# lixiny/ArtiBoost

Measured on AMD Instinct MI355X. Metric: synth samples/sec (render+fwd+bwd) 256x256 bs=64, higher is better.
Workload: dtype bf16x3; 1 GPU; train_artiboost HO3Dv2-clasbased (HybridBaseline/ResNet-34, 22x28x32x32 heat-map) + online CCV render 512->256, per-GPU batch 64, HO3D-like objects; global_batch=64, image=256, parallelism=dp1, graph=True, render_overlap=False

## Files before the change

artiboost_amd/csrc/optim.hip:

```cpp
#include "common.h"

#define OPT_THREADS 256
#define OPT_MAX_PARTS 1024

__global__ __launch_bounds__(OPT_THREADS) void sqnorm_kernel(const float* __restrict__ g, long n, float* __restrict__ part) {
    double s = 0.0;
    long nvec = n / 4;
    for (long i = (long)blockIdx.x * OPT_THREADS + threadIdx.x; i < nvec; i += (long)gridDim.x * OPT_THREADS) {
        float4 v = ((const float4*)g)[i];
        s += (double)v.x * v.x + (double)v.y * v.y + (double)v.z * v.z + (double)v.w * v.w;
    }
    __shared__ double sm[OPT_THREADS];
    sm[threadIdx.x] = s;
    __syncthreads();
    for (int o = OPT_THREADS / 2; o > 0; o >>= 1) {
        if (threadIdx.x < o) sm[threadIdx.x] += sm[threadIdx.x + o];
        __syncthreads();
    }
    if (threadIdx.x == 0) part[blockIdx.x] = (float)sm[0];
}

__global__ void norm_finalize_kernel(const float* __restrict__ part, int nparts, float* __restrict__ out) {
    double s = 0.0;
    for (int i = threadIdx.x; i < nparts; i += 64) s += part[i];
#pragma unroll
    for (int o = 32; o > 0; o >>= 1) s += __shfl_xor(s, o, 64);
    if (threadIdx.x == 0) out[0] = (float)sqrt(s);
}

__global__ __launch_bounds__(OPT_THREADS) void clip_adam_kernel(float* __restrict__ p, const float* __restrict__ g,
                                                                float* __restrict__ m, float* __restrict__ v, long n,
                                                                const float* __restrict__ total_norm, float max_norm,
                                                                float lr, float b1, float b2, float eps, float bc1,
                                                                float bc2_sqrt, const float* __restrict__ hyper,
                                                                bf16_t* __restrict__ lp, bf16_t* __restrict__ lp_lo = nullptr) {
    if (hyper) { lr = hyper[0]; bc1 = hyper[1]; bc2_sqrt = hyper[2]; }
    float coef = 1.f;
    if (max_norm > 0.f) { coef = max_norm / (total_norm[0] + 1e-6f); coef = coef > 1.f ? 1.f : coef; }
    const float step = lr / bc1;
    long nvec = n / 4;
    for (long i = (long)blockIdx.x * OPT_THREADS + threadIdx.x; i < nvec; i += (long)gridDim.x * OPT_THREADS) {
        float4 pv = ((float4*)p)[i], gv = ((const float4*)g)[i], mv = ((float4*)m)[i], vv = ((float4*)v)[i];
        float pp[4] = {pv.x, pv.y, pv.z, pv.w}, gg[4] = {gv.x, gv.y, gv.z, gv.w};
        float mm[4] = {mv.x, mv.y, mv.z, mv.w}, vvv[4] = {vv.x, vv.y, vv.z, vv.w};
#pragma unroll
        for (int k = 0; k < 4; ++k) {
            float gk = gg[k] * coef;
            mm[k] = mm[k] * b1 + (1.f - b1) * gk;
            vvv[k] = vvv[k] * b2 + (1.f - b2) * gk * gk;
            float denom = sqrtf(vvv[k]) / bc2_sqrt + eps;
            pp[k] = pp[k] - step * (mm[k] / denom);
        }
        ((float4*)p)[i] = make_float4(pp[0], pp[1], pp[2], pp[3]);
        ((float4*)m)[i] = make_float4(mm[0], mm[1], mm[2], mm[3]);
        ((float4*)v)[i] = make_float4(vvv[0], vvv[1], vvv[2], vvv[3]);
        if (lp) {
            uint2 o;
            o.x = pack_bf16x2(pp[0], pp[1]);
            o.y = pack_bf16x2(pp[2], pp[3]);
            ((uint2*)lp)[i] = o;
            if (lp_lo) {
                uint2 l;
                l.x = pack_bf16x2(pp[0] - __uint_as_float(o.x << 16), pp[1] - __uint_as_float(o.x & 0xffff0000u));
                l.y = pack_bf16x2(pp[2] - __uint_as_float(o.y << 16), pp[3] - __uint_as_float(o.y & 0xffff0000u));
                ((uint2*)lp_lo)[i] = l;
            }
        }
    }
}

extern "C" int ab_grad_norm(const float* grad, long n, float* part, float* total_norm, void* stream) {
    if (!grad || !part || !total_norm) return AB_EINVAL;
    if (n % 4) return AB_ESHAPE;
    long b = (n / 4 + OPT_THREADS - 1) / OPT_THREADS;
    int nb = (int)(b > OPT_MAX_PARTS ? OPT_MAX_PARTS : (b < 1 ? 1 : b));
    sqnorm_kernel<<<nb, OPT_THREADS, 0, as_stream(stream)>>>(grad, n, part);
    AB_LAUNCH_CHECK();
    norm_finalize_kernel<<<1, 64, 0, as_stream(stream)>>>(part, nb, total_norm);
    AB_LAUNCH_CHECK();
    return 0;
}

__global__ __launch_bounds__(OPT_THREADS) void scale_kernel(float* __restrict__ x, long n, float s, int head) {
    long nvec = (n - head) / 4;
    float4* xv = (float4*)(x + head);
    for (long i = (long)blockIdx.x * OPT_THREADS + threadIdx.x; i < nvec; i += (long)gridDim.x * OPT_THREADS) {
        float4 v = xv[i];
        v.x *= s; v.y *= s; v.z *= s; v.w *= s;
        xv[i] = v;
    }
    if (blockIdx.x == 0) {
        if ((int)threadIdx.x < head) x[threadIdx.x] *= s;
        long t = head + nvec * 4 + threadIdx.x;
        if (threadIdx.x < 4 && t < n) x[t] *= s;
    }
}

extern "C" int ab_scale_f32(float* x, long n, float s, void* stream) {
    if (!x || n < 0 || (uintptr_t)x % 4) return AB_EINVAL;
    if (n == 0) return 0;
    int head = (int)(((16 - (uintptr_t)x % 16) % 16) / 4);
    if (head > n) head = (int)n;
    long b = ((n - head) / 4 + OPT_THREADS - 1) / OPT_THREADS;
    int nb = (int)(b > 2048 ? 2048 : (b < 1 ? 1 : b));
    scale_kernel<<<nb, OPT_THREADS, 0, as_stream(stream)>>>(x, n, s, head);
    AB_LAUNCH_CHECK();
    return 0;
}

static int clip_adam_impl(float* param, const float* grad, float* m, float* v, long n, const float* total_norm, float max_norm, float lr,
                          float beta1, float beta2, float eps, int step, const float* hyper, void* lp, void* lp_lo, void* stream);

extern "C" int ab_clip_adam(float* param, const float* grad, float* m, float* v, long n, const float* total_norm,
                            float max_norm, float lr, float beta1, float beta2, float eps, int step,
                            const float* hyper, void* lp, void* stream) {
    return clip_adam_impl(param, grad, m, v, n, total_norm, max_norm, lr, beta1, beta2, eps, step, hyper, lp, nullptr, stream);
}

extern "C" int ab_clip_adam_x3(float* param, const float* grad, float* m, float* v, long n, const float* total_norm,
                               float max_norm, float lr, float beta1, float beta2, float eps, int step,
                               const float* hyper, void* lp_hi, void* lp_lo, void* stream) {
    if (!lp_hi || !lp_lo) return AB_EINVAL;
    return clip_adam_impl(param, grad, m, v, n, total_norm, max_norm, lr, beta1, beta2, eps, step, hyper, lp_hi, lp_lo, stream);
}

static int clip_adam_impl(float* param, const float* grad, float* m, float* v, long n, const float* total_norm, float max_norm, float lr,
                          float beta1, float beta2, float eps, int step, const float* hyper, void* lp, void* lp_lo, void* stream) {
    if (!param || !grad || !m || !v || (max_norm > 0.f && !total_norm)) return AB_EINVAL;
    if (n % 4 || step < 1) return AB_ESHAPE;
    double bc1 = 1.0 - pow((double)beta1, (double)step), bc2 = 1.0 - pow((double)beta2, (double)step);
    long b = (n / 4 + OPT_THREADS - 1) / OPT_THREADS;
    int nb = (int)(b > 4096 ? 4096 : (b < 1 ? 1 : b));
    clip_adam_kernel<<<nb, OPT_THREADS, 0, as_stream(stream)>>>(param, grad, m, v, n, total_norm, max_norm, lr, beta1,
                                                                beta2, eps, (float)bc1, (float)sqrt(bc2), hyper, (bf16_t*)lp, (bf16_t*)lp_lo);
    AB_LAUNCH_CHECK();
    return 0;
}


__global__ void wall_stamp_kernel(int64_t* slot) { *slot = (int64_t)wall_clock64(); }
extern "C" int ab_wall_stamp(int64_t* slot, void* stream) {
    if (!slot) return AB_EINVAL;
    wall_stamp_kernel<<<1, 1, 0, as_stream(stream)>>>(slot);
    AB_LAUNCH_CHECK();
    return 0;
}
extern "C" int ab_wall_clock_khz(void) {
    int dev = 0, khz = 0;
    if (hipGetDevice(&dev) != hipSuccess || hipDeviceGetAttribute(&khz, hipDeviceAttributeWallClockRate, dev) != hipSuccess) return 0;
    return khz;
}
```

artiboost_amd/csrc/torch_ops_gen.cpp:

```cpp
#include <ATen/ATen.h>
#include <c10/hip/HIPStream.h>
#include <torch/library.h>
#include "../../include/artiboost_hip.h"

static inline void* p(const c10::optional<at::Tensor>& t) { return (t.has_value() && t->defined()) ? t->data_ptr() : nullptr; }
static inline void* cur_stream() { return (void*)c10::hip::getCurrentHIPStream().stream(); }

#include <c10/hip/HIPFunctions.h>
typedef c10::optional<at::Tensor> OptT;
static inline bool has(const OptT& t) { return t.has_value() && t->defined(); }
static inline void ck_contig(const char* op, const char* a, const OptT& t) {
    if (has(t)) TORCH_CHECK(t->is_contiguous(), op, ": argument '", a, "' must be contiguous (the kernels take raw buffers)");
}
static inline void ck_dev(const char* op, const char* a, const OptT& t, int dt, bool contiguous) {
    if (!has(t)) return;
    TORCH_CHECK(t->is_cuda(), op, ": argument '", a, "' must be a HIP tensor, got a ", t->device().str(), " tensor");
    TORCH_CHECK(t->get_device() == c10::hip::current_device(), op, ": argument '", a, "' lives on device ", t->get_device(), ", the current device is ", (int)c10::hip::current_device());
    if (contiguous) TORCH_CHECK(t->is_contiguous(), op, ": argument '", a, "' must be contiguous (the kernel takes it as a raw buffer without a pitch)");
    if (dt >= 0) TORCH_CHECK((int)t->scalar_type() == dt, op, ": argument '", a, "' must be ", c10::toString((at::ScalarType)dt), ", got ", c10::toString(t->scalar_type()));
}
static inline void ck_host(const char* op, const char* a, const OptT& t) {
    if (!has(t)) return;
    TORCH_CHECK(t->is_cpu(), op, ": argument '", a, "' is a HOST structure / array of the C ABI and must be a CPU tensor, got a ", t->device().str(), " tensor");
    TORCH_CHECK(t->is_contiguous(), op, ": argument '", a, "' must be contiguous");
// ... 74 lines not shown
static void w_col_stats(const c10::optional<at::Tensor>& x, int64_t dtype, int64_t M, int64_t C, const c10::optional<at::Tensor>& part) { static const char* const OP = "artiboost_hip::col_stats"; ck_dev(OP, "x", x, (int)-1, true); ck_dev(OP, "part", part, (int)at::kFloat, true); ck_dtcode(OP, "x", x, dtype); ck_numel(OP, "x", x, (int64_t)(M*C)); ck_numel(OP, "part", part, (int64_t)(ab_col_stats_nparts(M)*C*2)); const long rc = (long)ab_col_stats((const void*)p(x), (int)dtype, (long)M, (int)C, (float*)p(part), cur_stream()); TORCH_CHECK(rc == 0, "ab_col_stats failed with code ", rc, rc > 0 ? " (hipError)" : " (argument error)"); }
static void w_bn_finalize(const c10::optional<at::Tensor>& part, int64_t nparts, int64_t C, int64_t count, const c10::optional<at::Tensor>& gamma, const c10::optional<at::Tensor>& beta, double eps, double momentum, const c10::optional<at::Tensor>& running_mean, const c10::optional<at::Tensor>& running_var, const c10::optional<at::Tensor>& bnp) { static const char* const OP = "artiboost_hip::bn_finalize"; ck_dev(OP, "part", part, (int)at::kFloat, true); ck_dev(OP, "gamma", gamma, (int)at::kFloat, true); ck_dev(OP, "beta", beta, (int)at::kFloat, true); ck_dev(OP, "running_mean", running_mean, (int)at::kFloat, true); ck_dev(OP, "running_var", running_var, (int)at::kFloat, true); ck_dev(OP, "bnp", bnp, (int)at::kFloat, true); ck_numel(OP, "part", part, (int64_t)(nparts*C*2)); ck_numel(OP, "gamma", gamma, (int64_t)(C)); ck_numel(OP, "beta", beta, (int64_t)(C)); ck_numel(OP, "running_mean", running_mean, (int64_t)(C)); ck_numel(OP, "running_var", running_var, (int64_t)(C)); ck_numel(OP, "bnp", bnp, (int64_t)(4*C)); const long rc = (long)ab_bn_finalize((const float*)p(part), (int)nparts, (int)C, (long)count, (const float*)p(gamma), (const float*)p(beta), (float)eps, (float)momentum, (float*)p(running_mean), (float*)p(running_var), (float*)p(bnp), cur_stream()); TORCH_CHECK(rc == 0, "ab_bn_finalize failed with code ", rc, rc > 0 ? " (hipError)" : " (argument error)"); }
static void w_bn_eval_params(int64_t C, const c10::optional<at::Tensor>& gamma, const c10::optional<at::Tensor>& beta, const c10::optional<at::Tensor>& rm, const c10::optional<at::Tensor>& rv, double eps, const c10::optional<at::Tensor>& bnp) { static const char* const OP = "artiboost_hip::bn_eval_params"; ck_dev(OP, "gamma", gamma, (int)at::kFloat, true); ck_dev(OP, "beta", beta, (int)at::kFloat, true); ck_dev(OP, "rm", rm, (int)at::kFloat, true); ck_dev(OP, "rv", rv, (int)at::kFloat, true); ck_dev(OP, "bnp", bnp, (int)at::kFloat, true); ck_numel(OP, "gamma", gamma, (int64_t)(C)); ck_numel(OP, "beta", beta, (int64_t)(C)); ck_numel(OP, "rm", rm, (int64_t)(C)); ck_numel(OP, "rv", rv, (int64_t)(C)); ck_numel(OP, "bnp", bnp, (int64_t)(4*C)); const long rc = (long)ab_bn_eval_params((int)C, (const float*)p(gamma), (const float*)p(beta), (const float*)p(rm), (const float*)p(rv), (float)eps, (float*)p(bnp), cur_stream()); TORCH_CHECK(rc == 0, "ab_bn_eval_params failed with code ", rc, rc > 0 ? " (hipError)" : " (argument error)"); }
static void w_bn_eval_params_batch(const c10::optional<at::Tensor>& flat, const c10::optional<at::Tensor>& stats, const c10::optional<at::Tensor>& desc_dev, int64_t n, int64_t max_c, double eps, const c10::optional<at::Tensor>& out) { static const char* const OP = "artiboost_hip::bn_eval_params_batch"; ck_dev(OP, "flat", flat, (int)at::kFloat, true); ck_dev(OP, "stats", stats, (int)at::kFloat, true); ck_dev(OP, "desc_dev", desc_dev, (int)at::kInt, true); ck_dev(OP, "out", out, (int)at::kFloat, true); const long rc = (long)ab_bn_eval_params_batch((const float*)p(flat), (const float*)p(stats), (const int32_t*)p(desc_dev), (int)n, (int)max_c, (float)eps, (float*)p(out), cur_stream()); TORCH_CHECK(rc == 0, "ab_bn_eval_params_batch failed with code ", rc, rc > 0 ? " (hipError)" : " (argument error)"); }
static void w_bn_apply(const c10::optional<at::Tensor>& y, const c10::optional<at::Tensor>& res, const c10::optional<at::Tensor>& bnp, int64_t dtype, int64_t M, int64_t C, int64_t relu, const c10::optional<at::Tensor>& out) { static const char* const OP = "artiboost_hip::bn_apply"; ck_dev(OP, "y", y, (int)-1, true); ck_dev(OP, "res", res, (int)-1, true); ck_dev(OP, "bnp", bnp, (int)at::kFloat, true); ck_dev(OP, "out", out, (int)-1, true); const long rc = (long)ab_bn_apply((const void*)p(y), (const void*)p(res), (const float*)p(bnp), (int)dtype, (long)M, (int)C, (int)relu, (void*)p(out), cur_stream()); TORCH_CHECK(rc == 0, "ab_bn_apply failed with code ", rc, rc > 0 ? " (hipError)" : " (argument error)"); }
static void w_bn_bwd(const c10::optional<at::Tensor>& dout, const c10::optional<at::Tensor>& out, const c10::optional<at::Tensor>& y, const c10::optional<at::Tensor>& bnp, int64_t dtype, int64_t M, int64_t C, int64_t relu, const c10::optional<at::Tensor>& part, const c10::optional<at::Tensor>& bwdp, const c10::optional<at::Tensor>& dgamma, const c10::optional<at::Tensor>& dbeta, const c10::optional<at::Tensor>& dy, const c10::optional<at::Tensor>& dz_out) { static const char* const OP = "artiboost_hip::bn_bwd"; ck_dev(OP, "dout", dout, (int)-1, true); ck_dev(OP, "out", out, (int)-1, true); ck_dev(OP, "y", y, (int)-1, true); ck_dev(OP, "bnp", bnp, (int)at::kFloat, true); ck_dev(OP, "part", part, (int)at::kFloat, true); ck_dev(OP, "bwdp", bwdp, (int)at::kFloat, true); ck_dev(OP, "dgamma", dgamma, (int)at::kFloat, true); ck_dev(OP, "dbeta", dbeta, (int)at::kFloat, true); ck_dev(OP, "dy", dy, (int)-1, true); ck_dev(OP, "dz_out", dz_out, (int)-1, true); const long rc = (long)ab_bn_bwd((const void*)p(dout), (const void*)p(out), (const void*)p(y), (const float*)p(bnp), (int)dtype, (long)M, (int)C, (int)relu, (float*)p(part), (float*)p(bwdp), (float*)p(dgamma), (float*)p(dbeta), (void*)p(dy), (void*)p(dz_out), cur_stream()); TORCH_CHECK(rc == 0, "ab_bn_bwd failed with code ", rc, rc > 0 ? " (hipError)" : " (argument error)"); }
static void w_relu_bwd(const c10::optional<at::Tensor>& dout, const c10::optional<at::Tensor>& out, int64_t dtype, int64_t n, const c10::optional<at::Tensor>& dz) { static const char* const OP = "artiboost_hip::relu_bwd"; ck_dev(OP, "dout", dout, (int)-1, true); ck_dev(OP, "out", out, (int)-1, true); ck_dev(OP, "dz", dz, (int)-1, true); const long rc = (long)ab_relu_bwd((const void*)p(dout), (const void*)p(out), (int)dtype, (long)n, (void*)p(dz), cur_stream()); TORCH_CHECK(rc == 0, "ab_relu_bwd failed with code ", rc, rc > 0 ? " (hipError)" : " (argument error)"); }
static void w_col_sum(const c10::optional<at::Tensor>& x, int64_t dtype, int64_t M, int64_t C, const c10::optional<at::Tensor>& part, const c10::optional<at::Tensor>& out) { static const char* const OP = "artiboost_hip::col_sum"; ck_dev(OP, "x", x, (int)-1, true); ck_dev(OP, "part", part, (int)at::kFloat, true); ck_dev(OP, "out", out, (int)at::kFloat, true); const long rc = (long)ab_col_sum((const void*)p(x), (int)dtype, (long)M, (int)C, (float*)p(part), (float*)p(out), cur_stream()); TORCH_CHECK(rc == 0, "ab_col_sum failed with code ", rc, rc > 0 ? " (hipError)" : " (argument error)"); }
static void w_col_sum_x3(const c10::optional<at::Tensor>& hi, const c10::optional<at::Tensor>& lo, int64_t M, int64_t C, const c10::optional<at::Tensor>& part, const c10::optional<at::Tensor>& out) { static const char* const OP = "artiboost_hip::col_sum_x3"; ck_dev(OP, "hi", hi, (int)-1, true); ck_dev(OP, "lo", lo, (int)-1, true); ck_dev(OP, "part", part, (int)at::kFloat, true); ck_dev(OP, "out", out, (int)at::kFloat, true); const long rc = (long)ab_col_sum_x3((const void*)p(hi), (const void*)p(lo), (long)M, (int)C, (float*)p(part), (float*)p(out), cur_stream()); TORCH_CHECK(rc == 0, "ab_col_sum_x3 failed with code ", rc, rc > 0 ? " (hipError)" : " (argument error)"); }
static void w_add(const c10::optional<at::Tensor>& a, const c10::optional<at::Tensor>& b, int64_t dtype, int64_t n, const c10::optional<at::Tensor>& out) { static const char* const OP = "artiboost_hip::add"; ck_dev(OP, "a", a, (int)-1, true); ck_dev(OP, "b", b, (int)-1, true); ck_dev(OP, "out", out, (int)-1, true); const long rc = (long)ab_add((const void*)p(a), (const void*)p(b), (int)dtype, (long)n, (void*)p(out), cur_stream()); TORCH_CHECK(rc == 0, "ab_add failed with code ", rc, rc > 0 ? " (hipError)" : " (argument error)"); }
static void w_maxpool3x3s2_fwd(const c10::optional<at::Tensor>& x, int64_t dtype, int64_t N, int64_t H, int64_t W, int64_t C, const c10::optional<at::Tensor>& out, const c10::optional<at::Tensor>& idx) { static const char* const OP = "artiboost_hip::maxpool3x3s2_fwd"; ck_dev(OP, "x", x, (int)-1, true); ck_dev(OP, "out", out, (int)-1, true); ck_dev(OP, "idx", idx, (int)-1, true); const long rc = (long)ab_maxpool3x3s2_fwd((const void*)p(x), (int)dtype, (int)N, (int)H, (int)W, (int)C, (void*)p(out), (void*)p(idx), cur_stream()); TORCH_CHECK(rc == 0, "ab_maxpool3x3s2_fwd failed with code ", rc, rc > 0 ? " (hipError)" : " (argument error)"); }
static int64_t w_conv2d_dgrad_bnstats_rows(int64_t dtype, int64_t N, int64_t H, int64_t W, int64_t Cin, int64_t Cout, int64_t kh, int64_t kw, int64_t stride, int64_t pad) { return (int64_t)ab_conv2d_dgrad_bnstats_rows((int)dtype, (int)N, (int)H, (int)W, (int)Cin, (int)Cout, (int)kh, (int)kw, (int)stride, (int)pad); }
static void w_conv2d_dgrad_bnstats(const c10::optional<at::Tensor>& dy, const c10::optional<at::Tensor>& wt, const c10::optional<at::Tensor>& dx, int64_t dtype, int64_t N, int64_t H, int64_t W, int64_t Cin, int64_t Cout, int64_t kh, int64_t kw, int64_t stride, int64_t pad, const c10::optional<at::Tensor>& addend, const c10::optional<at::Tensor>& bn_y, const c10::optional<at::Tensor>& bn_out, const c10::optional<at::Tensor>& bnp, const c10::optional<at::Tensor>& bn_part) { static const char* const OP = "artiboost_hip::conv2d_dgrad_bnstats"; ck_dev(OP, "dy", dy, (int)-1, true); ck_dev(OP, "wt", wt, (int)-1, true); ck_dev(OP, "dx", dx, (int)-1, true); ck_dev(OP, "addend", addend, (int)-1, true); ck_dev(OP, "bn_y", bn_y, (int)-1, true); ck_dev(OP, "bn_out", bn_out, (int)-1, true); ck_dev(OP, "bnp", bnp, (int)at::kFloat, true); ck_dev(OP, "bn_part", bn_part, (int)at::kFloat, true); const long rc = (long)ab_conv2d_dgrad_bnstats((const void*)p(dy), (const void*)p(wt), (void*)p(dx), (int)dtype, (int)N, (int)H, (int)W, (int)Cin, (int)Cout, (int)kh, (int)kw, (int)stride, (int)pad, (const void*)p(addend), (const void*)p(bn_y), (const void*)p(bn_out), (const float*)p(bnp), (float*)p(bn_part), cur_stream()); TORCH_CHECK(rc == 0, "ab_conv2d_dgrad_bnstats failed with code ", rc, rc > 0 ? " (hipError)" : " (argument error)"); }
static void w_bn_bwd_apply(const c10::optional<at::Tensor>& dout, const c10::optional<at::Tensor>& out, const c10::optional<at::Tensor>& y, const c10::optional<at::Tensor>& bnp, int64_t dtype, int64_t M, int64_t C, int64_t relu, const c10::optional<at::Tensor>& part, int64_t nparts, const c10::optional<at::Tensor>& bwdp, const c10::optional<at::Tensor>& dgamma, const c10::optional<at::Tensor>& dbeta, const c10::optional<at::Tensor>& dy, const c10::optional<at::Tensor>& dz_out) { static const char* const OP = "artiboost_hip::bn_bwd_apply"; ck_dev(OP, "dout", dout, (int)-1, true); ck_dev(OP, "out", out, (int)-1, true); ck_dev(OP, "y", y, (int)-1, true); ck_dev(OP, "bnp", bnp, (int)at::kFloat, true); ck_dev(OP, "part", part, (int)at::kFloat, true); ck_dev(OP, "bwdp", bwdp, (int)at::kFloat, true); ck_dev(OP, "dgamma", dgamma, (int)at::kFloat, true); ck_dev(OP, "dbeta", dbeta, (int)at::kFloat, true); ck_dev(OP, "dy", dy, (int)-1, true); ck_dev(OP, "dz_out", dz_out, (int)-1, true); const long rc = (long)ab_bn_bwd_apply((const void*)p(dout), (const void*)p(out), (const void*)p(y), (const float*)p(bnp), (int)dtype, (long)M, (int)C, (int)relu, (const float*)p(part), (int)nparts, (float*)p(bwdp), (float*)p(dgamma), (float*)p(dbeta), (void*)p(dy), (void*)p(dz_out), cur_stream()); TORCH_CHECK(rc == 0, "ab_bn_bwd_apply failed with code ", rc, rc > 0 ? " (hipError)" : " (argument error)"); }
static void w_bn_relu_maxpool3x3s2_fwd(const c10::optional<at::Tensor>& y, const c10::optional<at::Tensor>& bnp, int64_t dtype, int64_t N, int64_t H, int64_t W, int64_t C, const c10::optional<at::Tensor>& out, const c10::optional<at::Tensor>& idx) { static const char* const OP = "artiboost_hip::bn_relu_maxpool3x3s2_fwd"; ck_dev(OP, "y", y, (int)-1, true); ck_dev(OP, "bnp", bnp, (int)at::kFloat, true); ck_dev(OP, "out", out, (int)-1, true); ck_dev(OP, "idx", idx, (int)-1, true); const long rc = (long)ab_bn_relu_maxpool3x3s2_fwd((const void*)p(y), (const float*)p(bnp), (int)dtype, (int)N, (int)H, (int)W, (int)C, (void*)p(out), (void*)p(idx), cur_stream()); TORCH_CHECK(rc == 0, "ab_bn_relu_maxpool3x3s2_fwd failed with code ", rc, rc > 0 ? " (hipError)" : " (argument error)"); }
static void w_bn_relu_maxpool3x3s2_fwd_x3(const c10::optional<at::Tensor>& y, const c10::optional<at::Tensor>& bnp, int64_t N, int64_t H, int64_t W, int64_t C, const c10::optional<at::Tensor>& out, const c10::optional<at::Tensor>& out_hi, const c10::optional<at::Tensor>& out_lo, const c10::optional<at::Tensor>& idx) { static const char* const OP = "artiboost_hip::bn_relu_maxpool3x3s2_fwd_x3"; ck_dev(OP, "y", y, (int)at::kFloat, true); ck_dev(OP, "bnp", bnp, (int)at::kFloat, true); ck_dev(OP, "out", out, (int)at::kFloat, true); ck_dev(OP, "out_hi", out_hi, (int)-1, true); ck_dev(OP, "out_lo", out_lo, (int)-1, true); ck_dev(OP, "idx", idx, (int)-1, true); const long rc = (long)ab_bn_relu_maxpool3x3s2_fwd_x3((const float*)p(y), (const float*)p(bnp), (int)N, (int)H, (int)W, (int)C, (float*)p(out), (void*)p(out_hi), (void*)p(out_lo), (void*)p(idx), cur_stream()); TORCH_CHECK(rc == 0, "ab_bn_relu_maxpool3x3s2_fwd_x3 failed with code ", rc, rc > 0 ? " (hipError)" : " (argument error)"); }
static void w_bn_relu_maxpool_bwd(const c10::optional<at::Tensor>& dpool, const c10::optional<at::Tensor>& idx, const c10::optional<at::Tensor>& y, const c10::optional<at::Tensor>& bnp, int64_t dtype, int64_t N, int64_t H, int64_t W, int64_t C, const c10::optional<at::Tensor>& part, const c10::optional<at::Tensor>& bwdp, const c10::optional<at::Tensor>& dgamma, const c10::optional<at::Tensor>& dbeta, const c10::optional<at::Tensor>& dy) { static const char* const OP = "artiboost_hip::bn_relu_maxpool_bwd"; ck_dev(OP, "dpool", dpool, (int)-1, true); ck_dev(OP, "idx", idx, (int)-1, true); ck_dev(OP, "y", y, (int)-1, true); ck_dev(OP, "bnp", bnp, (int)at::kFloat, true); ck_dev(OP, "part", part, (int)at::kFloat, true); ck_dev(OP, "bwdp", bwdp, (int)at::kFloat, true); ck_dev(OP, "dgamma", dgamma, (int)at::kFloat, true); ck_dev(OP, "dbeta", dbeta, (int)at::kFloat, true); ck_dev(OP, "dy", dy, (int)-1, true); const long rc = (long)ab_bn_relu_maxpool_bwd((const void*)p(dpool), (const void*)p(idx), (const void*)p(y), (const float*)p(bnp), (int)dtype, (int)N, (int)H, (int)W, (int)C, (float*)p(part), (float*)p(bwdp), (float*)p(dgamma), (float*)p(dbeta), (void*)p(dy), cur_stream()); TORCH_CHECK(rc == 0, "ab_bn_relu_maxpool_bwd failed with code ", rc, rc > 0 ? " (hipError)" : " (argument error)"); }
static int64_t w_bn_relu_maxpool_bwd_x3_nparts(int64_t N, int64_t H, int64_t W, int64_t C) { return (int64_t)ab_bn_relu_maxpool_bwd_x3_nparts((int)N, (int)H, (int)W, (int)C); }
static void w_bn_relu_maxpool_bwd_x3(const c10::optional<at::Tensor>& dpool, const c10::optional<at::Tensor>& idx, const c10::optional<at::Tensor>& y, const c10::optional<at::Tensor>& bnp, int64_t N, int64_t H, int64_t W, int64_t C, const c10::optional<at::Tensor>& part, const c10::optional<at::Tensor>& bwdp, const c10::optional<at::Tensor>& dgamma, const c10::optional<at::Tensor>& dbeta, const c10::optional<at::Tensor>& dz, const c10::optional<at::Tensor>& dy_hi, const c10::optional<at::Tensor>& dy_lo) { static const char* const OP = "artiboost_hip::bn_relu_maxpool_bwd_x3"; ck_dev(OP, "dpool", dpool, (int)at::kFloat, true); ck_dev(OP, "idx", idx, (int)-1, true); ck_dev(OP, "y", y, (int)at::kFloat, true); ck_dev(OP, "bnp", bnp, (int)at::kFloat, true); ck_dev(OP, "part", part, (int)at::kFloat, true); ck_dev(OP, "bwdp", bwdp, (int)at::kFloat, true); ck_dev(OP, "dgamma", dgamma, (int)at::kFloat, true); ck_dev(OP, "dbeta", dbeta, (int)at::kFloat, true); ck_dev(OP, "dz", dz, (int)at::kFloat, true); ck_dev(OP, "dy_hi", dy_hi, (int)-1, true); ck_dev(OP, "dy_lo", dy_lo, (int)-1, true); const long rc = (long)ab_bn_relu_maxpool_bwd_x3((const float*)p(dpool), (const void*)p(idx), (const float*)p(y), (const float*)p(bnp), (int)N, (int)H, (int)W, (int)C, (float*)p(part), (float*)p(bwdp), (float*)p(dgamma), (float*)p(dbeta), (float*)p(dz), (void*)p(dy_hi), (void*)p(dy_lo), cur_stream()); TORCH_CHECK(rc == 0, "ab_bn_relu_maxpool_bwd_x3 failed with code ", rc, rc > 0 ? " (hipError)" : " (argument error)"); }
static void w_bn_relu_maxpool3x3s2_fwd_x3w(const c10::optional<at::Tensor>& y, const c10::optional<at::Tensor>& bnp, int64_t N, int64_t H, int64_t W, int64_t C, const c10::optional<at::Tensor>& out, const c10::optional<at::Tensor>& out_hi, const c10::optional<at::Tensor>& out_lo, const c10::optional<at::Tensor>& idx, const c10::optional<at::Tensor>& ywin) { static const char* const OP = "artiboost_hip::bn_relu_maxpool3x3s2_fwd_x3w"; ck_dev(OP, "y", y, (int)at::kFloat, true); ck_dev(OP, "bnp", bnp, (int)at::kFloat, true); ck_dev(OP, "out", out, (int)at::kFloat, true); ck_dev(OP, "out_hi", out_hi, (int)-1, true); ck_dev(OP, "out_lo", out_lo, (int)-1, true); ck_dev(OP, "idx", idx, (int)-1, true); ck_dev(OP, "ywin", ywin, (int)at::kFloat, true); ck_dtype(OP, "out_hi", out_hi, at::kBFloat16); ck_dtype(OP, "out_lo", out_lo, at::kBFloat16); ck_numel(OP, "y", y, (int64_t)(N*H*W*C)); ck_numel(OP, "bnp", bnp, (int64_t)(2*C)); ck_numel(OP, "out", out, (int64_t)(N*(H/2)*(W/2)*C)); ck_numel(OP, "out_hi", out_hi, (int64_t)(N*(H/2)*(W/2)*C)); ck_numel(OP, "out_lo", out_lo, (int64_t)(N*(H/2)*(W/2)*C)); ck_numel(OP, "ywin", ywin, (int64_t)(N*(H/2)*(W/2)*C)); ck_bytes(OP, "idx", idx, (int64_t)(N*(H/2)*(W/2)*C)); const long rc = (long)ab_bn_relu_maxpool3x3s2_fwd_x3w((const float*)p(y), (const float*)p(bnp), (int)N, (int)H, (int)W, (int)C, (float*)p(out), (void*)p(out_hi), (void*)p(out_lo), (void*)p(idx), (float*)p(ywin), cur_stream()); TORCH_CHECK(rc == 0, "ab_bn_relu_maxpool3x3s2_fwd_x3w failed with code ", rc, rc > 0 ? " (hipError)" : " (argument error)"); }
static void w_bn_relu_maxpool_bwd_x3w(const c10::optional<at::Tensor>& dpool, const c10::optional<at::Tensor>& idx, const c10::optional<at::Tensor>& ywin, const c10::optional<at::Tensor>& y, const c10::optional<at::Tensor>& bnp, int64_t N, int64_t H, int64_t W, int64_t C, const c10::optional<at::Tensor>& part, const c10::optional<at::Tensor>& bwdp, const c10::optional<at::Tensor>& dgamma, const c10::optional<at::Tensor>& dbeta, const c10::optional<at::Tensor>& dy_hi, const c10::optional<at::Tensor>& dy_lo) { static const char* const OP = "artiboost_hip::bn_relu_maxpool_bwd_x3w"; ck_dev(OP, "dpool", dpool, (int)at::kFloat, true); ck_dev(OP, "idx", idx, (int)-1, true); ck_dev(OP, "ywin", ywin, (int)at::kFloat, true); ck_dev(OP, "y", y, (int)at::kFloat, true); ck_dev(OP, "bnp", bnp, (int)at::kFloat, true); ck_dev(OP, "part", part, (int)at::kFloat, true); ck_dev(OP, "bwdp", bwdp, (int)at::kFloat, true); ck_dev(OP, "dgamma", dgamma, (int)at::kFloat, true); ck_dev(OP, "dbeta", dbeta, (int)at::kFloat, true); ck_dev(OP, "dy_hi", dy_hi, (int)-1, true); ck_dev(OP, "dy_lo", dy_lo, (int)-1, true); const long rc = (long)ab_bn_relu_maxpool_bwd_x3w((const float*)p(dpool), (const void*)p(idx), (const float*)p(ywin), (const float*)p(y), (const float*)p(bnp), (int)N, (int)H, (int)W, (int)C, (float*)p(part), (float*)p(bwdp), (float*)p(dgamma), (float*)p(dbeta), (void*)p(dy_hi), (void*)p(dy_lo), cur_stream()); TORCH_CHECK(rc == 0, "ab_bn_relu_maxpool_bwd_x3w failed with code ", rc, rc > 0 ? " (hipError)" : " (argument error)"); }
static void w_maxpool3x3s2_bwd(const c10::optional<at::Tensor>& idx, const c10::optional<at::Tensor>& dout, int64_t dtype, int64_t N, int64_t H, int64_t W, int64_t C, const c10::optional<at::Tensor>& dx) { static const char* const OP = "artiboost_hip::maxpool3x3s2_bwd"; ck_dev(OP, "idx", idx, (int)-1, true); ck_dev(OP, "dout", dout, (int)-1, true); ck_dev(OP, "dx", dx, (int)-1, true); const long rc = (long)ab_maxpool3x3s2_bwd((const void*)p(idx), (const void*)p(dout), (int)dtype, (int)N, (int)H, (int)W, (int)C, (void*)p(dx), cur_stream()); TORCH_CHECK(rc == 0, "ab_maxpool3x3s2_bwd failed with code ", rc, rc > 0 ? " (hipError)" : " (argument error)"); }
static void w_avgpool_fwd(const c10::optional<at::Tensor>& x, int64_t dtype, int64_t N, int64_t HW, int64_t C, const c10::optional<at::Tensor>& out) { static const char* const OP = "artiboost_hip::avgpool_fwd"; ck_dev(OP, "x", x, (int)-1, true); ck_dev(OP, "out", out, (int)at::kFloat, true); ck_dtcode(OP, "x", x, dtype); ck_numel(OP, "x", x, (int64_t)(N*HW*C)); ck_numel(OP, "out", out, (int64_t)(N*C)); const long rc = (long)ab_avgpool_fwd((const void*)p(x), (int)dtype, (int)N, (int)HW, (int)C, (float*)p(out), cur_stream()); TORCH_CHECK(rc == 0, "ab_avgpool_fwd failed with code ", rc, rc > 0 ? " (hipError)" : " (argument error)"); }
static void w_avgpool_bwd(const c10::optional<at::Tensor>& g, int64_t dtype, int64_t N, int64_t HW, int64_t C, const c10::optional<at::Tensor>& dx, int64_t accumulate) { static const char* const OP = "artiboost_hip::avgpool_bwd"; ck_dev(OP, "g", g, (int)at::kFloat, true); ck_dev(OP, "dx", dx, (int)-1, true); const long rc = (long)ab_avgpool_bwd((const float*)p(g), (int)dtype, (int)N, (int)HW, (int)C, (void*)p(dx), (int)accumulate, cur_stream()); TORCH_CHECK(rc == 0, "ab_avgpool_bwd failed with code ", rc, rc > 0 ? " (hipError)" : " (argument error)"); }
static void w_cast_f32_bf16(const c10::optional<at::Tensor>& src, int64_t n, const c10::optional<at::Tensor>& dst) { static const char* const OP = "artiboost_hip::cast_f32_bf16"; ck_dev(OP, "src", src, (int)at::kFloat, true); ck_dev(OP, "dst", dst, (int)-1, true); ck_dtype(OP, "dst", dst, at::kBFloat16); ck_numel(OP, "src", src, (int64_t)(n)); ck_numel(OP, "dst", dst, (int64_t)(n)); const long rc = (long)ab_cast_f32_bf16((const float*)p(src), (long)n, (void*)p(dst), cur_stream()); TORCH_CHECK(rc == 0, "ab_cast_f32_bf16 failed with code ", rc, rc > 0 ? " (hipError)" : " (argument error)"); }
static void w_transpose_oki(const c10::optional<at::Tensor>& src, int64_t O, int64_t K, int64_t I, int64_t dtype, const c10::optional<at::Tensor>& dst) { static const char* const OP = "artiboost_hip::transpose_oki"; ck_dev(OP, "src", src, (int)at::kFloat, true); ck_dev(OP, "dst", dst, (int)-1, true); const long rc = (long)ab_transpose_oki((const float*)p(src), (int)O, (int)K, (int)I, (int)dtype, (void*)p(dst), cur_stream()); TORCH_CHECK(rc == 0, "ab_transpose_oki failed with code ", rc, rc > 0 ? " (hipError)" : " (argument error)"); }
static void w_transpose_oki_batch(const c10::optional<at::Tensor>& desc_dev, int64_t ntensors, int64_t total_tiles, int64_t dtype) { static const char* const OP = "artiboost_hip::transpose_oki_batch"; ck_dev(OP, "desc_dev", desc_dev, (int)-1, true); const long rc = (long)ab_transpose_oki_batch((const ab_transpose_desc*)p(desc_dev), (int)ntensors, (long)total_tiles, (int)dtype, cur_stream()); TORCH_CHECK(rc == 0, "ab_transpose_oki_batch failed with code ", rc, rc > 0 ? " (hipError)" : " (argument error)"); }
static void w_transpose_oki_batch_x3(const c10::optional<at::Tensor>& desc_dev, int64_t ntensors, int64_t total_tiles, int64_t lo_offset_elems) { static const char* const OP = "artiboost_hip::transpose_oki_batch_x3"; ck_dev(OP, "desc_dev", desc_dev, (int)-1, true); const long rc = (long)ab_transpose_oki_batch_x3((const ab_transpose_desc*)p(desc_dev), (int)ntensors, (long)total_tiles, (long)lo_offset_elems, cur_stream()); TORCH_CHECK(rc == 0, "ab_transpose_oki_batch_x3 failed with code ", rc, rc > 0 ? " (hipError)" : " (argument error)"); }
static void w_image_pad_nhwc4(const c10::optional<at::Tensor>& img_nchw, int64_t dtype, int64_t N, int64_t H, int64_t W, const c10::optional<at::Tensor>& out) { static const char* const OP = "artiboost_hip::image_pad_nhwc4"; ck_dev(OP, "img_nchw", img_nchw, (int)at::kFloat, true); ck_dev(OP, "out", out, (int)-1, true); ck_dtcode(OP, "out", out, dtype); ck_numel(OP, "img_nchw", img_nchw, (int64_t)(N*3*H*W)); ck_numel(OP, "out", out, (int64_t)(N*(H+6)*(W+8)*4)); const long rc = (long)ab_image_pad_nhwc4((const float*)p(img_nchw), (int)dtype, (int)N, (int)H, (int)W, (void*)p(out), cur_stream()); TORCH_CHECK(rc == 0, "ab_image_pad_nhwc4 failed with code ", rc, rc > 0 ? " (hipError)" : " (argument error)"); }
static void w_grad_norm(const c10::optional<at::Tensor>& grad, int64_t n, const c10::optional<at::Tensor>& part, const c10::optional<at::Tensor>& total_norm) { static const char* const OP = "artiboost_hip::grad_norm"; ck_dev(OP, "grad", grad, (int)at::kFloat, true); ck_dev(OP, "part", part, (int)at::kFloat, true); ck_dev(OP, "total_norm", total_norm, (int)at::kFloat, true); ck_numel(OP, "grad", grad, (int64_t)(n)); ck_numel(OP, "total_norm", total_norm, (int64_t)(1)); const long rc = (long)ab_grad_norm((const float*)p(grad), (long)n, (float*)p(part), (float*)p(total_norm), cur_stream()); TORCH_CHECK(rc == 0, "ab_grad_norm failed with code ", rc, rc > 0 ? " (hipError)" : " (argument error)"); }
static void w_scale_f32(const c10::optional<at::Tensor>& x, int64_t n, double s) { static const char* const OP = "artiboost_hip::scale_f32"; ck_dev(OP, "x", x, (int)at::kFloat, true); ck_numel(OP, "x", x, (int64_t)(n)); const long rc = (long)ab_scale_f32((float*)p(x), (long)n, (float)s, cur_stream()); TORCH_CHECK(rc == 0, "ab_scale_f32 failed with code ", rc, rc > 0 ? " (hipError)" : " (argument error)"); }
static void w_clip_adam(const c10::optional<at::Tensor>& param, const c10::optional<at::Tensor>& grad, const c10::optional<at::Tensor>& m, const c10::optional<at::Tensor>& v, int64_t n, const c10::optional<at::Tensor>& total_norm, double max_norm, double lr, double beta1, double beta2, double eps, int64_t step, const c10::optional<at::Tensor>& hyper, const c10::optional<at::Tensor>& lp) { static const char* const OP = "artiboost_hip::clip_adam"; ck_dev(OP, "param", param, (int)at::kFloat, true); ck_dev(OP, "grad", grad, (int)at::kFloat, true); ck_dev(OP, "m", m, (int)at::kFloat, true); ck_dev(OP, "v", v, (int)at::kFloat, true); ck_dev(OP, "total_norm", total_norm, (int)at::kFloat, true); ck_dev(OP, "hyper", hyper, (int)at::kFloat, true); ck_dev(OP, "lp", lp, (int)-1, true); ck_dtype(OP, "lp", lp, at::kBFloat16); ck_numel(OP, "param", param, (int64_t)(n)); ck_numel(OP, "grad", grad, (int64_t)(n)); ck_numel(OP, "m", m, (int64_t)(n)); ck_numel(OP, "v", v, (int64_t)(n)); ck_numel(OP, "lp", lp, (int64_t)(n)); ck_numel(OP, "total_norm", total_norm, (int64_t)(1)); const long rc = (long)ab_clip_adam((float*)p(param), (const float*)p(grad), (float*)p(m), (float*)p(v), (long)n, (const float*)p(total_norm), (float)max_norm, (float)lr, (float)beta1, (float)beta2, (float)eps, (int)step, (const float*)p(hyper), (void*)p(lp), cur_stream()); TORCH_CHECK(rc == 0, "ab_clip_adam failed with code ", rc, rc > 0 ? " (hipError)" : " (argument error)"); }
static void w_clip_adam_x3(const c10::optional<at::Tensor>& param, const c10::optional<at::Tensor>& grad, const c10::optional<at::Tensor>& m, const c10::optional<at::Tensor>& v, int64_t n, const c10::optional<at::Tensor>& total_norm, double max_norm, double lr, double beta1, double beta2, double eps, int64_t step, const c10::optional<at::Tensor>& hyper, const c10::optional<at::Tensor>& lp_hi, const c10::optional<at::Tensor>& lp_lo) { static const char* const OP = "artiboost_hip::clip_adam_x3"; ck_dev(OP, "param", param, (int)at::kFloat, true); ck_dev(OP, "grad", grad, (int)at::kFloat, true); ck_dev(OP, "m", m, (int)at::kFloat, true); ck_dev(OP, "v", v, (int)at::kFloat, true); ck_dev(OP, "total_norm", total_norm, (int)at::kFloat, true); ck_dev(OP, "hyper", hyper, (int)at::kFloat, true); ck_dev(OP, "lp_hi", lp_hi, (int)-1, true); ck_dev(OP, "lp_lo", lp_lo, (int)-1, true); ck_dtype(OP, "lp_hi", lp_hi, at::kBFloat16); ck_dtype(OP, "lp_lo", lp_lo, at::kBFloat16); ck_numel(OP, "param", param, (int64_t)(n)); ck_numel(OP, "grad", grad, (int64_t)(n)); ck_numel(OP, "m", m, (int64_t)(n)); ck_numel(OP, "v", v, (int64_t)(n)); ck_numel(OP, "lp_hi", lp_hi, (int64_t)(n)); ck_numel(OP, "lp_lo", lp_lo, (int64_t)(n)); ck_numel(OP, "total_norm", total_norm, (int64_t)(1)); const long rc = (long)ab_clip_adam_x3((float*)p(param), (const float*)p(grad), (float*)p(m), (float*)p(v), (long)n, (const float*)p(total_norm), (float)max_norm, (float)lr, (float)beta1, (float)beta2, (float)eps, (int)step, (const float*)p(hyper), (void*)p(lp_hi), (void*)p(lp_lo), cur_stream()); TORCH_CHECK(rc == 0, "ab_clip_adam_x3 failed with code ", rc, rc > 0 ? " (hipError)" : " (argument error)"); }
static void w_pose_assemble(const c10::optional<at::Tensor>& kp3d, const c10::optional<at::Tensor>& box6d, int64_t box_stride, const c10::optional<at::Tensor>& root_joint, const c10::optional<at::Tensor>& cam_intr, const c10::optional<at::Tensor>& corners_can, int64_t B, int64_t center_idx, double res_w, double res_h, const c10::optional<at::Tensor>& joints_abs, const c10::optional<at::Tensor>& corners_abs, const c10::optional<at::Tensor>& rotmat, const c10::optional<at::Tensor>& uvd2d, const c10::optional<at::Tensor>& joints_rel, const c10::optional<at::Tensor>& corners_rel, const c10::optional<at::Tensor>& boxroot) { static const char* const OP = "artiboost_hip::pose_assemble"; ck_dev(OP, "kp3d", kp3d, (int)at::kFloat, true); ck_dev(OP, "box6d", box6d, (int)at::kFloat, false); ck_dev(OP, "root_joint", root_joint, (int)at::kFloat, true); ck_dev(OP, "cam_intr", cam_intr, (int)at::kFloat, true); ck_dev(OP, "corners_can", corners_can, (int)at::kFloat, true); ck_dev(OP, "joints_abs", joints_abs, (int)at::kFloat, true); ck_dev(OP, "corners_abs", corners_abs, (int)at::kFloat, true); ck_dev(OP, "rotmat", rotmat, (int)at::kFloat, true); ck_dev(OP, "uvd2d", uvd2d, (int)at::kFloat, true); ck_dev(OP, "joints_rel", joints_rel, (int)at::kFloat, true); ck_dev(OP, "corners_rel", corners_rel, (int)at::kFloat, true); ck_dev(OP, "boxroot", boxroot, (int)at::kFloat, true); ck_numel(OP, "kp3d", kp3d, (int64_t)(B*22*3)); ck_numel(OP, "root_joint", root_joint, (int64_t)(B*3)); ck_numel(OP, "cam_intr", cam_intr, (int64_t)(B*9)); ck_numel(OP, "corners_can", corners_can, (int64_t)(B*24)); ck_numel(OP, "joints_abs", joints_abs, (int64_t)(B*63)); ck_numel(OP, "joints_rel", joints_rel, (int64_t)(B*63)); ck_numel(OP, "corners_abs", corners_abs, (int64_t)(B*24)); ck_numel(OP, "corners_rel", corners_rel, (int64_t)(B*24)); ck_numel(OP, "rotmat", rotmat, (int64_t)(B*9)); ck_numel(OP, "uvd2d", uvd2d, (int64_t)(B*90)); const long rc = (long)ab_pose_assemble((const float*)p(kp3d), (const float*)p(box6d), (int)box_stride, (const float*)p(root_joint), (const float*)p(cam_intr), (const float*)p(corners_can), (int)B, (int)center_idx, (float)res_w, (float)res_h, (float*)p(joints_abs), (float*)p(corners_abs), (float*)p(rotmat), (float*)p(uvd2d), (float*)p(joints_rel), (float*)p(corners_rel), (float*)p(boxroot), cur_stream()); TORCH_CHECK(rc == 0, "ab_pose_assemble failed with code ", rc, rc > 0 ? " (hipError)" : " (argument error)"); }
static void w_pose_loss(const c10::optional<at::Tensor>& kp3d, const c10::optional<at::Tensor>& box6d, int64_t box_stride, const c10::optional<at::Tensor>& root_joint, const c10::optional<at::Tensor>& cam_intr, const c10::optional<at::Tensor>& corners_can, const c10::optional<at::Tensor>& joints_3d, const c10::optional<at::Tensor>& corners_3d, const c10::optional<at::Tensor>& joints_vis, const c10::optional<at::Tensor>& corners_vis, const c10::optional<at::Tensor>& hand_views, int64_t nvh, const c10::optional<at::Tensor>& j0, const c10::optional<at::Tensor>& j1, int64_t njp, const c10::optional<at::Tensor>& p0, const c10::optional<at::Tensor>& p1, int64_t npp, const c10::optional<at::Tensor>& scene_views, int64_t nvs, const c10::optional<at::Tensor>& s0, const c10::optional<at::Tensor>& s1, int64_t nsp, int64_t B, int64_t center_idx, double res_w, double res_h, const c10::optional<at::Tensor>& weights8_host, const c10::optional<at::Tensor>& joints_abs, const c10::optional<at::Tensor>& corners_abs, const c10::optional<at::Tensor>& rotmat, const c10::optional<at::Tensor>& uvd2d, const c10::optional<at::Tensor>& sample_part, const c10::optional<at::Tensor>& losses, const c10::optional<at::Tensor>& g_kp3d, const c10::optional<at::Tensor>& g_box6d) { static const char* const OP = "artiboost_hip::pose_loss"; ck_dev(OP, "kp3d", kp3d, (int)at::kFloat, true); ck_dev(OP, "box6d", box6d, (int)at::kFloat, false); ck_dev(OP, "root_joint", root_joint, (int)at::kFloat, true); ck_dev(OP, "cam_intr", cam_intr, (int)at::kFloat, true); ck_dev(OP, "corners_can", corners_can, (int)at::kFloat, true); ck_dev(OP, "joints_3d", joints_3d, (int)at::kFloat, true); ck_dev(OP, "corners_3d", corners_3d, (int)at::kFloat, true); ck_dev(OP, "joints_vis", joints_vis, (int)at::kFloat, true); ck_dev(OP, "corners_vis", corners_vis, (int)at::kFloat, true); ck_dev(OP, "hand_views", hand_views, (int)at::kFloat, true); ck_dev(OP, "j0", j0, (int)at::kLong, true); ck_dev(OP, "j1", j1, (int)at::kLong, true); ck_dev(OP, "p0", p0, (int)at::kLong, true); ck_dev(OP, "p1", p1, (int)at::kLong, true); ck_dev(OP, "scene_views", scene_views, (int)at::kFloat, true); ck_dev(OP, "s0", s0, (int)at::kLong, true); ck_dev(OP, "s1", s1, (int)at::kLong, true); ck_host(OP, "weights8_host", weights8_host); ck_dev(OP, "joints_abs", joints_abs, (int)at::kFloat, true); ck_dev(OP, "corners_abs", corners_abs, (int)at::kFloat, true); ck_dev(OP, "rotmat", rotmat, (int)at::kFloat, true); ck_dev(OP, "uvd2d", uvd2d, (int)at::kFloat, true); ck_dev(OP, "sample_part", sample_part, (int)at::kFloat, true); ck_dev(OP, "losses", losses, (int)at::kFloat, true); ck_dev(OP, "g_kp3d", g_kp3d, (int)at::kFloat, true); ck_dev(OP, "g_box6d", g_box6d, (int)at::kFloat, false); ck_numel(OP, "kp3d", kp3d, (int64_t)(B*22*3)); ck_numel(OP, "g_kp3d", g_kp3d, (int64_t)(B*22*3)); ck_numel(OP, "root_joint", root_joint, (int64_t)(B*3)); ck_numel(OP, "cam_intr", cam_intr, (int64_t)(B*9)); ck_numel(OP, "corners_can", corners_can, (int64_t)(B*24)); ck_numel(OP, "corners_3d", corners_3d, (int64_t)(B*24)); ck_numel(OP, "joints_3d", joints_3d, (int64_t)(B*63)); ck_numel(OP, "joints_vis", joints_vis, (int64_t)(B*21)); ck_numel(OP, "corners_vis", corners_vis, (int64_t)(B*8)); ck_numel(OP, "hand_views", hand_views, (int64_t)(nvh*3)); ck_numel(OP, "scene_views", scene_views, (int64_t)(nvs*3)); ck_numel(OP, "j0", j0, (int64_t)(njp)); ck_numel(OP, "j1", j1, (int64_t)(njp)); ck_numel(OP, "p0", p0, (int64_t)(npp)); ck_numel(OP, "p1", p1, (int64_t)(npp)); ck_numel(OP, "s0", s0, (int64_t)(nsp)); ck_numel(OP, "s1", s1, (int64_t)(nsp)); ck_numel(OP, "weights8_host", weights8_host, (int64_t)(8)); const long rc = (long)ab_pose_loss((const float*)p(kp3d), (const float*)p(box6d), (int)box_stride, (const float*)p(root_joint), (const float*)p(cam_intr), (const float*)p(corners_can), (const float*)p(joints_3d), (const float*)p(corners_3d), (const float*)p(joints_vis), (const float*)p(corners_vis), (const float*)p(hand_views), (int)nvh, (const int64_t*)p(j0), (const int64_t*)p(j1), (int)njp, (const int64_t*)p(p0), (const int64_t*)p(p1), (int)npp, (const float*)p(scene_views), (int)nvs, (const int64_t*)p(s0), (const int64_t*)p(s1), (int)nsp, (int)B, (int)center_idx, (float)res_w, (float)res_h, (const float*)p(weights8_host), (float*)p(joints_abs), (float*)p(corners_abs), (float*)p(rotmat), (float*)p(uvd2d), (float*)p(sample_part), (float*)p(losses), (float*)p(g_kp3d), (float*)p(g_box6d), cur_stream()); TORCH_CHECK(rc == 0, "ab_pose_loss failed with code ", rc, rc > 0 ? " (hipError)" : " (argument error)"); }
static void w_pose_loss_sym(const c10::optional<at::Tensor>& kp3d, const c10::optional<at::Tensor>& box6d, int64_t box_stride, const c10::optional<at::Tensor>& root_joint, const c10::optional<at::Tensor>& cam_intr, const c10::optional<at::Tensor>& corners_can, const c10::optional<at::Tensor>& joints_3d, const c10::optional<at::Tensor>& corners_3d, const c10::optional<at::Tensor>& joints_vis, const c10::optional<at::Tensor>& corners_vis, const c10::optional<at::Tensor>& hand_views, int64_t nvh, const c10::optional<at::Tensor>& j0, const c10::optional<at::Tensor>& j1, int64_t njp, const c10::optional<at::Tensor>& p0, const c10::optional<at::Tensor>& p1, int64_t npp, const c10::optional<at::Tensor>& scene_views, int64_t nvs, const c10::optional<at::Tensor>& s0, const c10::optional<at::Tensor>& s1, int64_t nsp, int64_t B, int64_t center_idx, double res_w, double res_h, const c10::optional<at::Tensor>& weights8_host, const c10::optional<at::Tensor>& sym, const c10::optional<at::Tensor>& joints_abs, const c10::optional<at::Tensor>& corners_abs, const c10::optional<at::Tensor>& rotmat, const c10::optional<at::Tensor>& uvd2d, const c10::optional<at::Tensor>& sample_part, const c10::optional<at::Tensor>& losses, const c10::optional<at::Tensor>& g_kp3d, const c10::optional<at::Tensor>& g_box6d) { static const char* const OP = "artiboost_hip::pose_loss_sym"; ck_dev(OP, "kp3d", kp3d, (int)at::kFloat, true); ck_dev(OP, "box6d", box6d, (int)at::kFloat, false); ck_dev(OP, "root_joint", root_joint, (int)at::kFloat, true); ck_dev(OP, "cam_intr", cam_intr, (int)at::kFloat, true); ck_dev(OP, "corners_can", corners_can, (int)at::kFloat, true); ck_dev(OP, "joints_3d", joints_3d, (int)at::kFloat, true); ck_dev(OP, "corners_3d", corners_3d, (int)at::kFloat, true); ck_dev(OP, "joints_vis", joints_vis, (int)at::kFloat, true); ck_dev(OP, "corners_vis", corners_vis, (int)at::kFloat, true); ck_dev(OP, "hand_views", hand_views, (int)at::kFloat, true); ck_dev(OP, "j0", j0, (int)at::kLong, true); ck_dev(OP, "j1", j1, (int)at::kLong, true); ck_dev(OP, "p0", p0, (int)at::kLong, true); ck_dev(OP, "p1", p1, (int)at::kLong, true); ck_dev(OP, "scene_views", scene_views, (int)at::kFloat, true); ck_dev(OP, "s0", s0, (int)at::kLong, true); ck_dev(OP, "s1", s1, (int)at::kLong, true); ck_host(OP, "weights8_host", weights8_host); ck_contig(OP, "sym", sym); ck_dev(OP, "joints_abs", joints_abs, (int)at::kFloat, true); ck_dev(OP, "corners_abs", corners_abs, (int)at::kFloat, true); ck_dev(OP, "rotmat", rotmat, (int)at::kFloat, true); ck_dev(OP, "uvd2d", uvd2d, (int)at::kFloat, true); ck_dev(OP, "sample_part", sample_part, (int)at::kFloat, true); ck_dev(OP, "losses", losses, (int)at::kFloat, true); ck_dev(OP, "g_kp3d", g_kp3d, (int)at::kFloat, true); ck_dev(OP, "g_box6d", g_box6d, (int)at::kFloat, false); ck_numel(OP, "kp3d", kp3d, (int64_t)(B*22*3)); ck_numel(OP, "g_kp3d", g_kp3d, (int64_t)(B*22*3)); ck_numel(OP, "root_joint", root_joint, (int64_t)(B*3)); ck_numel(OP, "cam_intr", cam_intr, (int64_t)(B*9)); const long rc = (long)ab_pose_loss_sym((const float*)p(kp3d), (const float*)p(box6d), (int)box_stride, (const float*)p(root_joint), (const float*)p(cam_intr), (const float*)p(corners_can), (const float*)p(joints_3d), (const float*)p(corners_3d), (const float*)p(joints_vis), (const float*)p(corners_vis), (const float*)p(hand_views), (int)nvh, (const int64_t*)p(j0), (const int64_t*)p(j1), (int)njp, (const int64_t*)p(p0), (const int64_t*)p(p1), (int)npp, (const float*)p(scene_views), (int)nvs, (const int64_t*)p(s0), (const int64_t*)p(s1), (int)nsp, (int)B, (int)center_idx, (float)res_w, (float)res_h, (const float*)p(weights8_host), (const ab_symcorner*)p(sym), (float*)p(joints_abs), (float*)p(corners_abs), (float*)p(rotmat), (float*)p(uvd2d), (float*)p(sample_part), (float*)p(losses), (float*)p(g_kp3d), (float*)p(g_box6d), cur_stream()); TORCH_CHECK(rc == 0, "ab_pose_loss_sym failed with code ", rc, rc > 0 ? " (hipError)" : " (argument error)"); }
static void w_reg_pose_loss(const c10::optional<at::Tensor>& joints_pred, const c10::optional<at::Tensor>& mano_pca_pose, const c10::optional<at::Tensor>& mano_shape, const c10::optional<at::Tensor>& transf, int64_t transf_stride, const c10::optional<at::Tensor>& root_joint, const c10::optional<at::Tensor>& cam_intr, const c10::optional<at::Tensor>& corners_can, const c10::optional<at::Tensor>& joints_3d, const c10::optional<at::Tensor>& corners_3d, const c10::optional<at::Tensor>& joints_vis, const c10::optional<at::Tensor>& corners_vis, const c10::optional<at::Tensor>& hand_views, int64_t nvh, const c10::optional<at::Tensor>& j0, const c10::optional<at::Tensor>& j1, int64_t njp, const c10::optional<at::Tensor>& p0, const c10::optional<at::Tensor>& p1, int64_t npp, const c10::optional<at::Tensor>& scene_views, int64_t nvs, const c10::optional<at::Tensor>& s0, const c10::optional<at::Tensor>& s1, int64_t nsp, int64_t B, int64_t ncomps, const c10::optional<at::Tensor>& weights12_host, const c10::optional<at::Tensor>& joints_abs, const c10::optional<at::Tensor>& corners_abs, const c10::optional<at::Tensor>& rotmat, const c10::optional<at::Tensor>& sample_part, const c10::optional<at::Tensor>& losses, const c10::optional<at::Tensor>& g_joints, const c10::optional<at::Tensor>& g_pose, const c10::optional<at::Tensor>& g_shape, const c10::optional<at::Tensor>& g_transf) { static const char* const OP = "artiboost_hip::reg_pose_loss"; ck_dev(OP, "joints_pred", joints_pred, (int)at::kFloat, true); ck_dev(OP, "mano_pca_pose", mano_pca_pose, (int)at::kFloat, true); ck_dev(OP, "mano_shape", mano_shape, (int)at::kFloat, true); ck_dev(OP, "transf", transf, (int)at::kFloat, false); ck_dev(OP, "root_joint", root_joint, (int)at::kFloat, true); ck_dev(OP, "cam_intr", cam_intr, (int)at::kFloat, true); ck_dev(OP, "corners_can", corners_can, (int)at::kFloat, true); ck_dev(OP, "joints_3d", joints_3d, (int)at::kFloat, true); ck_dev(OP, "corners_3d", corners_3d, (int)at::kFloat, true); ck_dev(OP, "joints_vis", joints_vis, (int)at::kFloat, true); ck_dev(OP, "corners_vis", corners_vis, (int)at::kFloat, true); ck_dev(OP, "hand_views", hand_views, (int)at::kFloat, true); ck_dev(OP, "j0", j0, (int)at::kLong, true); ck_dev(OP, "j1", j1, (int)at::kLong, true); ck_dev(OP, "p0", p0, (int)at::kLong, true); ck_dev(OP, "p1", p1, (int)at::kLong, true); ck_dev(OP, "scene_views", scene_views, (int)at::kFloat, true); ck_dev(OP, "s0", s0, (int)at::kLong, true); ck_dev(OP, "s1", s1, (int)at::kLong, true); ck_host(OP, "weights12_host", weights12_host); ck_dev(OP, "joints_abs", joints_abs, (int)at::kFloat, true); ck_dev(OP, "corners_abs", corners_abs, (int)at::kFloat, true); ck_dev(OP, "rotmat", rotmat, (int)at::kFloat, true); ck_dev(OP, "sample_part", sample_part, (int)at::kFloat, true); ck_dev(OP, "losses", losses, (int)at::kFloat, true); ck_dev(OP, "g_joints", g_joints, (int)at::kFloat, true); ck_dev(OP, "g_pose", g_pose, (int)at::kFloat, true); ck_dev(OP, "g_shape", g_shape, (int)at::kFloat, true); ck_dev(OP, "g_transf", g_transf, (int)at::kFloat, false); ck_numel(OP, "joints_pred", joints_pred, (int64_t)(B*63)); ck_numel(OP, "joints_3d", joints_3d, (int64_t)(B*63)); ck_numel(OP, "joints_abs", joints_abs, (int64_t)(B*63)); ck_numel(OP, "g_joints", g_joints, (int64_t)(B*63)); ck_numel(OP, "mano_pca_pose", mano_pca_pose, (int64_t)(B*(3+ncomps))); ck_numel(OP, "g_pose", g_pose, (int64_t)(B*(3+ncomps))); ck_numel(OP, "mano_shape", mano_shape, (int64_t)(B*10)); ck_numel(OP, "g_shape", g_shape, (int64_t)(B*10)); ck_numel(OP, "root_joint", root_joint, (int64_t)(B*3)); ck_numel(OP, "cam_intr", cam_intr, (int64_t)(B*9)); ck_numel(OP, "corners_can", corners_can, (int64_t)(B*24)); ck_numel(OP, "corners_3d", corners_3d, (int64_t)(B*24)); ck_numel(OP, "corners_abs", corners_abs, (int64_t)(B*24)); ck_numel(OP, "joints_vis", joints_vis, (int64_t)(B*21)); ck_numel(OP, "corners_vis", corners_vis, (int64_t)(B*8)); ck_numel(OP, "rotmat", rotmat, (int64_t)(B*9)); ck_numel(OP, "sample_part", sample_part, (int64_t)(B*8)); ck_numel(OP, "losses", losses, (int64_t)(16)); ck_numel(OP, "hand_views", hand_views, (int64_t)(nvh*3)); ck_numel(OP, "scene_views", scene_views, (int64_t)(nvs*3)); ck_numel(OP, "j0", j0, (int64_t)(njp)); ck_numel(OP, "j1", j1, (int64_t)(njp)); ck_numel(OP, "p0", p0, (int64_t)(npp)); ck_numel(OP, "p1", p1, (int64_t)(npp)); ck_numel(OP, "s0", s0, (int64_t)(nsp)); ck_numel(OP, "s1", s1, (int64_t)(nsp)); ck_numel(OP, "weights12_host", weights12_host, (int64_t)(12)); const long rc = (long)ab_reg_pose_loss((const float*)p(joints_pred), (const float*)p(mano_pca_pose), (const float*)p(mano_shape), (const float*)p(transf), (int)transf_stride, (const float*)p(root_joint), (const float*)p(cam_intr), (const float*)p(corners_can), (const float*)p(joints_3d), (const float*)p(corners_3d), (const float*)p(joints_vis), (const float*)p(corners_vis), (const float*)p(hand_views), (int)nvh, (const int64_t*)p(j0), (const int64_t*)p(j1), (int)njp, (const int64_t*)p(p0), (const int64_t*)p(p1), (int)npp, (const float*)p(scene_views), (int)nvs, (const int64_t*)p(s0), (const int64_t*)p(s1), (int)nsp, (int)B, (int)ncomps, (const float*)p(weights12_host), (float*)p(joints_abs), (float*)p(corners_abs), (float*)p(rotmat), (float*)p(sample_part), (float*)p(losses), (float*)p(g_joints), (float*)p(g_pose), (float*)p(g_shape), (float*)p(g_transf), cur_stream()); TORCH_CHECK(rc == 0, "ab_reg_pose_loss failed with code ", rc, rc > 0 ? " (hipError)" : " (argument error)"); }
static int64_t w_render_workspace_bytes(int64_t B, int64_t W, int64_t H, int64_t max_faces) { return (int64_t)ab_render_workspace_bytes((int)B, (int)W, (int)H, (int)max_faces); }
static void w_render_batch(const c10::optional<at::Tensor>& scene_host, const c10::optional<at::Tensor>& samples, const c10::optional<at::Tensor>& hand_verts, const c10::optional<at::Tensor>& order, const c10::optional<at::Tensor>& factor, const c10::optional<at::Tensor>& inv_affine, const c10::optional<at::Tensor>& blur_radius, int64_t B, int64_t max_faces, int64_t ow, int64_t oh, int64_t out_dtype, const c10::optional<at::Tensor>& out_pad, const c10::optional<at::Tensor>& out_chw, const c10::optional<at::Tensor>& workspace, const c10::optional<at::Tensor>& keys_out, const c10::optional<at::Tensor>& rgbx_out) { static const char* const OP = "artiboost_hip::render_batch"; ck_host(OP, "scene_host", scene_host); ck_dev(OP, "samples", samples, (int)-1, true); ck_dev(OP, "hand_verts", hand_verts, (int)at::kFloat, true); ck_dev(OP, "order", order, (int)at::kInt, true); ck_dev(OP, "factor", factor, (int)at::kFloat, true); ck_dev(OP, "inv_affine", inv_affine, (int)at::kFloat, true); ck_dev(OP, "blur_radius", blur_radius, (int)at::kFloat, true); ck_dev(OP, "out_pad", out_pad, (int)-1, true); ck_dev(OP, "out_chw", out_chw, (int)at::kFloat, true); ck_dev(OP, "workspace", workspace, (int)-1, true); ck_dev(OP, "keys_out", keys_out, (int)-1, true); ck_dev(OP, "rgbx_out", rgbx_out, (int)-1, true); ck_bytes(OP, "samples", samples, (int64_t)(B*96)); ck_numel(OP, "hand_verts", hand_verts, (int64_t)(B*778*3)); ck_numel(OP, "order", order, (int64_t)(B*4)); ck_numel(OP, "factor", factor, (int64_t)(B*4)); ck_numel(OP, "inv_affine", inv_affine, (int64_t)(B*6)); ck_numel(OP, "blur_radius", blur_radius, (int64_t)(B)); ck_dtcode(OP, "out_pad", out_pad, out_dtype); ck_numel(OP, "out_pad", out_pad, (int64_t)(B*(oh+6)*(ow+8)*4)); ck_numel(OP, "out_chw", out_chw, (int64_t)(B*3*oh*ow)); const long rc = (long)ab_render_batch((const ab_scene*)p(scene_host), (const void*)p(samples), (const float*)p(hand_verts), (const int32_t*)p(order), (const float*)p(factor), (const float*)p(inv_affine), (const float*)p(blur_radius), (int)B, (int)max_faces, (int)ow, (int)oh, (int)out_dtype, (void*)p(out_pad), (float*)p(out_chw), (void*)p(workspace), (void*)p(keys_out), (void*)p(rgbx_out), cur_stream()); TORCH_CHECK(rc == 0, "ab_render_batch failed with code ", rc, rc > 0 ? " (hipError)" : " (argument error)"); }
static void w_gaussian_blur(const c10::optional<at::Tensor>& rgbx, int64_t B, int64_t W, int64_t H, const c10::optional<at::Tensor>& radius, const c10::optional<at::Tensor>& out) { static const char* const OP = "artiboost_hip::gaussian_blur"; ck_dev(OP, "rgbx", rgbx, (int)-1, true); ck_dev(OP, "radius", radius, (int)at::kFloat, true); ck_dev(OP, "out", out, (int)-1, true); ck_dtype(OP, "rgbx", rgbx, at::kByte); ck_dtype(OP, "out", out, at::kByte); ck_numel(OP, "rgbx", rgbx, (int64_t)(B*W*H*4)); ck_numel(OP, "out", out, (int64_t)(B*W*H*4)); ck_numel(OP, "radius", radius, (int64_t)(B)); const long rc = (long)ab_gaussian_blur((const void*)p(rgbx), (int)B, (int)W, (int)H, (const float*)p(radius), (void*)p(out), cur_stream()); TORCH_CHECK(rc == 0, "ab_gaussian_blur failed with code ", rc, rc > 0 ? " (hipError)" : " (argument error)"); }
static int64_t w_augment_workspace_bytes(int64_t B, int64_t W, int64_t H) { return (int64_t)ab_augment_workspace_bytes((int)B, (int)W, (int)H); }
static void w_augment_batch(const c10::optional<at::Tensor>& rgbx, int64_t B, int64_t W, int64_t H, const c10::optional<at::Tensor>& order, const c10::optional<at::Tensor>& factor, const c10::optional<at::Tensor>& inv_affine, const c10::optional<at::Tensor>& blur_radius, const c10::optional<at::Tensor>& flip, int64_t ow, int64_t oh, int64_t out_dtype, const c10::optional<at::Tensor>& out_pad, const c10::optional<at::Tensor>& out_chw, const c10::optional<at::Tensor>& workspace) { static const char* const OP = "artiboost_hip::augment_batch"; ck_dev(OP, "rgbx", rgbx, (int)-1, true); ck_dev(OP, "order", order, (int)at::kInt, true); ck_dev(OP, "factor", factor, (int)at::kFloat, true); ck_dev(OP, "inv_affine", inv_affine, (int)at::kFloat, true); ck_dev(OP, "blur_radius", blur_radius, (int)at::kFloat, true); ck_dev(OP, "flip", flip, (int)at::kByte, true); ck_dev(OP, "out_pad", out_pad, (int)-1, true); ck_dev(OP, "out_chw", out_chw, (int)at::kFloat, true); ck_dev(OP, "workspace", workspace, (int)-1, true); ck_dtype(OP, "rgbx", rgbx, at::kByte); ck_numel(OP, "rgbx", rgbx, (int64_t)(B*W*H*4)); ck_numel(OP, "order", order, (int64_t)(B*4)); ck_numel(OP, "factor", factor, (int64_t)(B*4)); ck_numel(OP, "inv_affine", inv_affine, (int64_t)(B*6)); ck_numel(OP, "blur_radius", blur_radius, (int64_t)(B)); ck_numel(OP, "flip", flip, (int64_t)(B)); ck_dtcode(OP, "out_pad", out_pad, out_dtype); ck_numel(OP, "out_pad", out_pad, (int64_t)(B*(oh+6)*(ow+8)*4)); ck_numel(OP, "out_chw", out_chw, (int64_t)(B*3*oh*ow)); ck_bytes(OP, "workspace", workspace, (int64_t)(ab_augment_workspace_bytes(B,W,H))); const long rc = (long)ab_augment_batch((const void*)p(rgbx), (int)B, (int)W, (int)H, (const int32_t*)p(order), (const float*)p(factor), (const float*)p(inv_affine), (const float*)p(blur_radius), (const uint8_t*)p(flip), (int)ow, (int)oh, (int)out_dtype, (void*)p(out_pad), (float*)p(out_chw), (void*)p(workspace), cur_stream()); TORCH_CHECK(rc == 0, "ab_augment_batch failed with code ", rc, rc > 0 ? " (hipError)" : " (argument error)"); }
static int64_t w_jpeg_workspace_bytes(int64_t total_blocks, int64_t total_subseq, int64_t plane_bytes, int64_t data_bytes, int64_t total_segs, int64_t n, int64_t n_tables) { return (int64_t)ab_jpeg_workspace_bytes((long)total_blocks, (long)total_subseq, (long)plane_bytes, (long)data_bytes, (long)total_segs, (int)n, (int)n_tables); }
static void w_jpeg_decode_batch(const c10::optional<at::Tensor>& data, const c10::optional<at::Tensor>& desc, const c10::optional<at::Tensor>& segs, const c10::optional<at::Tensor>& qtabs, const c10::optional<at::Tensor>& htabs, int64_t n, int64_t n_tables, int64_t sub_bytes, int64_t total_blocks, int64_t total_subseq, int64_t plane_bytes, int64_t data_bytes, int64_t total_segs, int64_t max_blocks, int64_t max_width, int64_t max_height, int64_t max_subseq, int64_t out_channels, const c10::optional<at::Tensor>& out, const c10::optional<at::Tensor>& workspace) { static const char* const OP = "artiboost_hip::jpeg_decode_batch"; ck_dev(OP, "data", data, (int)-1, true); ck_dev(OP, "desc", desc, (int)at::kInt, true); ck_dev(OP, "segs", segs, (int)at::kInt, true); ck_dev(OP, "qtabs", qtabs, (int)-1, true); ck_dev(OP, "htabs", htabs, (int)-1, true); ck_dev(OP, "out", out, (int)-1, true); ck_dev(OP, "workspace", workspace, (int)-1, true); ck_dtype(OP, "data", data, at::kByte); ck_dtype(OP, "out", out, at::kByte); ck_bytes(OP, "data", data, (int64_t)(data_bytes)); ck_numel(OP, "desc", desc, (int64_t)(n*AB_JPEG_DESC_INTS)); ck_numel(OP, "segs", segs, (int64_t)(total_segs*4)); ck_bytes(OP, "qtabs", qtabs, (int64_t)(n*4*64*2)); ck_bytes(OP, "htabs", htabs, (int64_t)(n_tables*8*272)); ck_bytes(OP, "workspace", workspace, (int64_t)(ab_jpeg_workspace_bytes(total_blocks,total_subseq,plane_bytes,data_bytes,total_segs,n,n_tables))); const long rc = (long)ab_jpeg_decode_batch((const void*)p(data), (const int32_t*)p(desc), (const int32_t*)p(segs), (const void*)p(qtabs), (const void*)p(htabs), (int)n, (int)n_tables, (int)sub_bytes, (long)total_blocks, (long)total_subseq, (long)plane_bytes, (long)data_bytes, (long)total_segs, (int)max_blocks, (int)max_width, (int)max_height, (int)max_subseq, (int)out_channels, (void*)p(out), (void*)p(workspace), cur_stream()); TORCH_CHECK(rc == 0, "ab_jpeg_decode_batch failed with code ", rc, rc > 0 ? " (hipError)" : " (argument error)"); }
static void w_png_unfilter_batch(const c10::optional<at::Tensor>& raw, const c10::optional<at::Tensor>& desc, int64_t n, int64_t max_width, int64_t max_bpp, int64_t out_channels, const c10::optional<at::Tensor>& out, const c10::optional<at::Tensor>& status) { static const char* const OP = "artiboost_hip::png_unfilter_batch"; ck_dev(OP, "raw", raw, (int)-1, true); ck_dev(OP, "desc", desc, (int)at::kInt, true); ck_dev(OP, "out", out, (int)-1, true); ck_dev(OP, "status", status, (int)at::kInt, true); ck_dtype(OP, "raw", raw, at::kByte); ck_dtype(OP, "out", out, at::kByte); ck_numel(OP, "desc", desc, (int64_t)(n*AB_PNG_DESC_INTS)); ck_numel(OP, "status", status, (int64_t)(1)); const long rc = (long)ab_png_unfilter_batch((const void*)p(raw), (const int32_t*)p(desc), (int)n, (int)max_width, (int)max_bpp, (int)out_channels, (void*)p(out), (int*)p(status), cur_stream()); TORCH_CHECK(rc == 0, "ab_png_unfilter_batch failed with code ", rc, rc > 0 ? " (hipError)" : " (argument error)"); }
static void w_linear_fwd(const c10::optional<at::Tensor>& x, const c10::optional<at::Tensor>& w, const c10::optional<at::Tensor>& bias, int64_t M, int64_t N, int64_t K, int64_t relu, const c10::optional<at::Tensor>& y) { static const char* const OP = "artiboost_hip::linear_fwd"; ck_dev(OP, "x", x, (int)at::kFloat, true); ck_dev(OP, "w", w, (int)at::kFloat, true); ck_dev(OP, "bias", bias, (int)at::kFloat, true); ck_dev(OP, "y", y, (int)at::kFloat, true); ck_numel(OP, "x", x, (int64_t)(M*K)); ck_numel(OP, "w", w, (int64_t)(N*K)); ck_numel(OP, "bias", bias, (int64_t)(N)); ck_numel(OP, "y", y, (int64_t)(M*N)); const long rc = (long)ab_linear_fwd((const float*)p(x), (const float*)p(w), (const float*)p(bias), (int)M, (int)N, (int)K, (int)relu, (float*)p(y), cur_stream()); TORCH_CHECK(rc == 0, "ab_linear_fwd failed with code ", rc, rc > 0 ? " (hipError)" : " (argument error)"); }
static void w_linear_dgrad(const c10::optional<at::Tensor>& g, const c10::optional<at::Tensor>& wt, const c10::optional<at::Tensor>& act_out, int64_t M, int64_t N, int64_t K, const c10::optional<at::Tensor>& gx) { static const char* const OP = "artiboost_hip::linear_dgrad"; ck_dev(OP, "g", g, (int)at::kFloat, true); ck_dev(OP, "wt", wt, (int)at::kFloat, true); ck_dev(OP, "act_out", act_out, (int)at::kFloat, true); ck_dev(OP, "gx", gx, (int)at::kFloat, true); ck_numel(OP, "g", g, (int64_t)(M*N)); ck_numel(OP, "act_out", act_out, (int64_t)(M*N)); ck_numel(OP, "wt", wt, (int64_t)(K*N)); ck_numel(OP, "gx", gx, (int64_t)(M*K)); const long rc = (long)ab_linear_dgrad((const float*)p(g), (const float*)p(wt), (const float*)p(act_out), (int)M, (int)N, (int)K, (float*)p(gx), cur_stream()); TORCH_CHECK(rc == 0, "ab_linear_dgrad failed with code ", rc, rc > 0 ? " (hipError)" : " (argument error)"); }
static void w_linear_wgrad(const c10::optional<at::Tensor>& g, const c10::optional<at::Tensor>& x, int64_t M, int64_t N, int64_t K, const c10::optional<at::Tensor>& dw, const c10::optional<at::Tensor>& db) { static const char* const OP = "artiboost_hip::linear_wgrad"; ck_dev(OP, "g", g, (int)at::kFloat, true); ck_dev(OP, "x", x, (int)at::kFloat, true); ck_dev(OP, "dw", dw, (int)at::kFloat, true); ck_dev(OP, "db", db, (int)at::kFloat, true); ck_numel(OP, "g", g, (int64_t)(M*N)); ck_numel(OP, "x", x, (int64_t)(M*K)); ck_numel(OP, "dw", dw, (int64_t)(N*K)); ck_numel(OP, "db", db, (int64_t)(N)); const long rc = (long)ab_linear_wgrad((const float*)p(g), (const float*)p(x), (int)M, (int)N, (int)K, (float*)p(dw), (float*)p(db), cur_stream()); TORCH_CHECK(rc == 0, "ab_linear_wgrad failed with code ", rc, rc > 0 ? " (hipError)" : " (argument error)"); }
static void w_nearest_dist(const c10::optional<at::Tensor>& x, const c10::optional<at::Tensor>& ypts, const c10::optional<at::Tensor>& obj_idx, const c10::optional<at::Tensor>& rot, int64_t B, int64_t P1, int64_t P2, const c10::optional<at::Tensor>& scale, const c10::optional<at::Tensor>& shift, const c10::optional<at::Tensor>& dist, int64_t ld, const c10::optional<at::Tensor>& idx_out) { static const char* const OP = "artiboost_hip::nearest_dist"; ck_dev(OP, "x", x, (int)at::kFloat, true); ck_dev(OP, "ypts", ypts, (int)at::kFloat, true); ck_dev(OP, "obj_idx", obj_idx, (int)at::kLong, true); ck_dev(OP, "rot", rot, (int)at::kFloat, true); ck_dev(OP, "scale", scale, (int)at::kFloat, true); ck_dev(OP, "shift", shift, (int)at::kFloat, true); ck_dev(OP, "dist", dist, (int)at::kFloat, false); ck_dev(OP, "idx_out", idx_out, (int)at::kInt, true); ck_numel(OP, "x", x, (int64_t)(B*P1*3)); ck_numel(OP, "rot", rot, (int64_t)(B*9)); ck_numel(OP, "obj_idx", obj_idx, (int64_t)(B)); ck_numel(OP, "scale", scale, (int64_t)(P1)); ck_numel(OP, "shift", shift, (int64_t)(P1)); ck_numel(OP, "idx_out", idx_out, (int64_t)(B*P1)); const long rc = (long)ab_nearest_dist((const float*)p(x), (const float*)p(ypts), (const int64_t*)p(obj_idx), (const float*)p(rot), (int)B, (int)P1, (int)P2, (const float*)p(scale), (const float*)p(shift), (float*)p(dist), (int)ld, (int32_t*)p(idx_out), cur_stream()); TORCH_CHECK(rc == 0, "ab_nearest_dist failed with code ", rc, rc > 0 ? " (hipError)" : " (argument error)"); }
static void w_linear_fused(const c10::optional<at::Tensor>& x, const c10::optional<at::Tensor>& w, const c10::optional<at::Tensor>& bias, const c10::optional<at::Tensor>& scale, const c10::optional<at::Tensor>& shift, const c10::optional<at::Tensor>& residual, int64_t ldr, int64_t M, int64_t N, int64_t K, int64_t act, double slope, const c10::optional<at::Tensor>& y, int64_t ldy) { static const char* const OP = "artiboost_hip::linear_fused"; ck_dev(OP, "x", x, (int)at::kFloat, true); ck_dev(OP, "w", w, (int)at::kFloat, true); ck_dev(OP, "bias", bias, (int)at::kFloat, true); ck_dev(OP, "scale", scale, (int)at::kFloat, true); ck_dev(OP, "shift", shift, (int)at::kFloat, true); ck_dev(OP, "residual", residual, (int)at::kFloat, false); ck_dev(OP, "y", y, (int)at::kFloat, false); ck_numel(OP, "x", x, (int64_t)(M*K)); ck_numel(OP, "w", w, (int64_t)(N*K)); ck_numel(OP, "bias", bias, (int64_t)(N)); ck_numel(OP, "scale", scale, (int64_t)(N)); ck_numel(OP, "shift", shift, (int64_t)(N)); const long rc = (long)ab_linear_fused((const float*)p(x), (const float*)p(w), (const float*)p(bias), (const float*)p(scale), (const float*)p(shift), (const float*)p(residual), (int)ldr, (int)M, (int)N, (int)K, (int)act, (float)slope, (float*)p(y), (int)ldy, cur_stream()); TORCH_CHECK(rc == 0, "ab_linear_fused failed with code ", rc, rc > 0 ? " (hipError)" : " (argument error)"); }
static void w_color_jitter(const c10::optional<at::Tensor>& rgbx, int64_t B, int64_t npix, const c10::optional<at::Tensor>& order, const c10::optional<at::Tensor>& factor, const c10::optional<at::Tensor>& out, const c10::optional<at::Tensor>& lsum_ws) { static const char* const OP = "artiboost_hip::color_jitter"; ck_dev(OP, "rgbx", rgbx, (int)-1, true); ck_dev(OP, "order", order, (int)at::kInt, true); ck_dev(OP, "factor", factor, (int)at::kFloat, true); ck_dev(OP, "out", out, (int)-1, true); ck_dev(OP, "lsum_ws", lsum_ws, (int)-1, true); ck_dtype(OP, "rgbx", rgbx, at::kByte); ck_dtype(OP, "out", out, at::kByte); ck_numel(OP, "rgbx", rgbx, (int64_t)(B*npix*4)); ck_numel(OP, "out", out, (int64_t)(B*npix*4)); ck_numel(OP, "order", order, (int64_t)(B*4)); ck_numel(OP, "factor", factor, (int64_t)(B*4)); ck_bytes(OP, "lsum_ws", lsum_ws, (int64_t)(B*8)); const long rc = (long)ab_color_jitter((const void*)p(rgbx), (int)B, (int)npix, (const int32_t*)p(order), (const float*)p(factor), (void*)p(out), (void*)p(lsum_ws), cur_stream()); TORCH_CHECK(rc == 0, "ab_color_jitter failed with code ", rc, rc > 0 ? " (hipError)" : " (argument error)"); }
static void w_mano_lbs(const c10::optional<at::Tensor>& pose, const c10::optional<at::Tensor>& betas, const c10::optional<at::Tensor>& v_template, const c10::optional<at::Tensor>& shapedirs, const c10::optional<at::Tensor>& posedirs, const c10::optional<at::Tensor>& J_regressor, const c10::optional<at::Tensor>& weights, const c10::optional<at::Tensor>& hands_mean, int64_t B, const c10::optional<at::Tensor>& verts, const c10::optional<at::Tensor>& joints, const c10::optional<at::Tensor>& T_abs) { static const char* const OP = "artiboost_hip::mano_lbs"; ck_dev(OP, "pose", pose, (int)at::kFloat, true); ck_dev(OP, "betas", betas, (int)at::kFloat, true); ck_dev(OP, "v_template", v_template, (int)at::kFloat, true); ck_dev(OP, "shapedirs", shapedirs, (int)at::kFloat, true); ck_dev(OP, "posedirs", posedirs, (int)at::kFloat, true); ck_dev(OP, "J_regressor", J_regressor, (int)at::kFloat, true); ck_dev(OP, "weights", weights, (int)at::kFloat, true); ck_dev(OP, "hands_mean", hands_mean, (int)at::kFloat, true); ck_dev(OP, "verts", verts, (int)at::kFloat, true); ck_dev(OP, "joints", joints, (int)at::kFloat, true); ck_dev(OP, "T_abs", T_abs, (int)at::kFloat, true); ck_numel(OP, "pose", pose, (int64_t)(B*48)); ck_numel(OP, "betas", betas, (int64_t)(B*10)); ck_numel(OP, "v_template", v_template, (int64_t)(778*3)); ck_numel(OP, "shapedirs", shapedirs, (int64_t)(778*3*10)); ck_numel(OP, "posedirs", posedirs, (int64_t)(778*3*135)); ck_numel(OP, "J_regressor", J_regressor, (int64_t)(16*778)); ck_numel(OP, "weights", weights, (int64_t)(778*16)); ck_numel(OP, "hands_mean", hands_mean, (int64_t)(45)); ck_numel(OP, "verts", verts, (int64_t)(B*778*3)); ck_numel(OP, "joints", joints, (int64_t)(B*21*3)); ck_numel(OP, "T_abs", T_abs, (int64_t)(B*16*16)); const long rc = (long)ab_mano_lbs((const float*)p(pose), (const float*)p(betas), (const float*)p(v_template), (const float*)p(shapedirs), (const float*)p(posedirs), (const float*)p(J_regressor), (const float*)p(weights), (const float*)p(hands_mean), (int)B, (float*)p(verts), (float*)p(joints), (float*)p(T_abs), cur_stream()); TORCH_CHECK(rc == 0, "ab_mano_lbs failed with code ", rc, rc > 0 ? " (hipError)" : " (argument error)"); }
static void w_mano_pca_fwd(const c10::optional<at::Tensor>& pose_coeffs, const c10::optional<at::Tensor>& betas, const c10::optional<at::Tensor>& comps, const c10::optional<at::Tensor>& hands_mean, const c10::optional<at::Tensor>& v_template, const c10::optional<at::Tensor>& shapedirs, const c10::optional<at::Tensor>& posedirs, const c10::optional<at::Tensor>& J_regressor, const c10::optional<at::Tensor>& weights, int64_t ncomps, int64_t center_idx, int64_t B, const c10::optional<at::Tensor>& verts, const c10::optional<at::Tensor>& joints, const c10::optional<at::Tensor>& full_pose) { static const char* const OP = "artiboost_hip::mano_pca_fwd"; ck_dev(OP, "pose_coeffs", pose_coeffs, (int)at::kFloat, true); ck_dev(OP, "betas", betas, (int)at::kFloat, true); ck_dev(OP, "comps", comps, (int)at::kFloat, true); ck_dev(OP, "hands_mean", hands_mean, (int)at::kFloat, true); ck_dev(OP, "v_template", v_template, (int)at::kFloat, true); ck_dev(OP, "shapedirs", shapedirs, (int)at::kFloat, true); ck_dev(OP, "posedirs", posedirs, (int)at::kFloat, true); ck_dev(OP, "J_regressor", J_regressor, (int)at::kFloat, true); ck_dev(OP, "weights", weights, (int)at::kFloat, true); ck_dev(OP, "verts", verts, (int)at::kFloat, true); ck_dev(OP, "joints", joints, (int)at::kFloat, true); ck_dev(OP, "full_pose", full_pose, (int)at::kFloat, true); ck_numel(OP, "pose_coeffs", pose_coeffs, (int64_t)(B*(3+ncomps))); ck_numel(OP, "betas", betas, (int64_t)(B*10)); ck_numel(OP, "comps", comps, (int64_t)(ncomps*45)); ck_numel(OP, "hands_mean", hands_mean, (int64_t)(45)); ck_numel(OP, "v_template", v_template, (int64_t)(778*3)); ck_numel(OP, "shapedirs", shapedirs, (int64_t)(778*3*10)); ck_numel(OP, "posedirs", posedirs, (int64_t)(778*3*135)); ck_numel(OP, "J_regressor", J_regressor, (int64_t)(16*778)); ck_numel(OP, "weights", weights, (int64_t)(778*16)); ck_numel(OP, "verts", verts, (int64_t)(B*778*3)); ck_numel(OP, "joints", joints, (int64_t)(B*21*3)); ck_numel(OP, "full_pose", full_pose, (int64_t)(B*48)); const long rc = (long)ab_mano_pca_fwd((const float*)p(pose_coeffs), (const float*)p(betas), (const float*)p(comps), (const float*)p(hands_mean), (const float*)p(v_template), (const float*)p(shapedirs), (const float*)p(posedirs), (const float*)p(J_regressor), (const float*)p(weights), (int)ncomps, (int)center_idx, (int)B, (float*)p(verts), (float*)p(joints), (float*)p(full_pose), cur_stream()); TORCH_CHECK(rc == 0, "ab_mano_pca_fwd failed with code ", rc, rc > 0 ? " (hipError)" : " (argument error)"); }
static void w_mano_pca_bwd(const c10::optional<at::Tensor>& pose_coeffs, const c10::optional<at::Tensor>& betas, const c10::optional<at::Tensor>& comps, const c10::optional<at::Tensor>& hands_mean, const c10::optional<at::Tensor>& v_template, const c10::optional<at::Tensor>& shapedirs, const c10::optional<at::Tensor>& posedirs, const c10::optional<at::Tensor>& J_regressor, const c10::optional<at::Tensor>& weights, int64_t ncomps, int64_t center_idx, int64_t B, const c10::optional<at::Tensor>& g_verts, const c10::optional<at::Tensor>& g_joints, const c10::optional<at::Tensor>& g_full_pose, const c10::optional<at::Tensor>& g_pose_coeffs, const c10::optional<at::Tensor>& g_betas) { static const char* const OP = "artiboost_hip::mano_pca_bwd"; ck_dev(OP, "pose_coeffs", pose_coeffs, (int)at::kFloat, true); ck_dev(OP, "betas", betas, (int)at::kFloat, true); ck_dev(OP, "comps", comps, (int)at::kFloat, true); ck_dev(OP, "hands_mean", hands_mean, (int)at::kFloat, true); ck_dev(OP, "v_template", v_template, (int)at::kFloat, true); ck_dev(OP, "shapedirs", shapedirs, (int)at::kFloat, true); ck_dev(OP, "posedirs", posedirs, (int)at::kFloat, true); ck_dev(OP, "J_regressor", J_regressor, (int)at::kFloat, true); ck_dev(OP, "weights", weights, (int)at::kFloat, true); ck_dev(OP, "g_verts", g_verts, (int)at::kFloat, true); ck_dev(OP, "g_joints", g_joints, (int)at::kFloat, true); ck_dev(OP, "g_full_pose", g_full_pose, (int)at::kFloat, true); ck_dev(OP, "g_pose_coeffs", g_pose_coeffs, (int)at::kFloat, true); ck_dev(OP, "g_betas", g_betas, (int)at::kFloat, true); ck_numel(OP, "pose_coeffs", pose_coeffs, (int64_t)(B*(3+ncomps))); ck_numel(OP, "g_pose_coeffs", g_pose_coeffs, (int64_t)(B*(3+ncomps))); ck_numel(OP, "betas", betas, (int64_t)(B*10)); ck_numel(OP, "g_betas", g_betas, (int64_t)(B*10)); ck_numel(OP, "comps", comps, (int64_t)(ncomps*45)); ck_numel(OP, "hands_mean", hands_mean, (int64_t)(45)); ck_numel(OP, "v_template", v_template, (int64_t)(778*3)); ck_numel(OP, "shapedirs", shapedirs, (int64_t)(778*3*10)); ck_numel(OP, "posedirs", posedirs, (int64_t)(778*3*135)); ck_numel(OP, "J_regressor", J_regressor, (int64_t)(16*778)); ck_numel(OP, "weights", weights, (int64_t)(778*16)); ck_numel(OP, "g_verts", g_verts, (int64_t)(B*778*3)); ck_numel(OP, "g_joints", g_joints, (int64_t)(B*21*3)); ck_numel(OP, "g_full_pose", g_full_pose, (int64_t)(B*48)); const long rc = (long)ab_mano_pca_bwd((const float*)p(pose_coeffs), (const float*)p(betas), (const float*)p(comps), (const float*)p(hands_mean), (const float*)p(v_template), (const float*)p(shapedirs), (const float*)p(posedirs), (const float*)p(J_regressor), (const float*)p(weights), (int)ncomps, (int)center_idx, (int)B, (const float*)p(g_verts), (const float*)p(g_joints), (const float*)p(g_full_pose), (float*)p(g_pose_coeffs), (float*)p(g_betas), cur_stream()); TORCH_CHECK(rc == 0, "ab_mano_pca_bwd failed with code ", rc, rc > 0 ? " (hipError)" : " (argument error)"); }
static int64_t w_honet_recover_chunks(int64_t N) { return (int64_t)ab_honet_recover_chunks((int)N); }
static int64_t w_honet_recover_workspace(int64_t B, int64_t N) { return (int64_t)ab_honet_recover_workspace((int)B, (int)N); }
static void w_honet_recover_fwd(const c10::optional<at::Tensor>& hand_st, int64_t hand_pitch, const c10::optional<at::Tensor>& obj_st, int64_t obj_pitch, const c10::optional<at::Tensor>& cam_intr, const c10::optional<at::Tensor>& joints_3d, const c10::optional<at::Tensor>& hand_verts_3d, const c10::optional<at::Tensor>& obj_verts_can, const c10::optional<at::Tensor>& corners_can, int64_t B, int64_t N, double trans_factor, double scale_factor, double img_w, double img_h, double off_z, const c10::optional<at::Tensor>& root_joint, const c10::optional<at::Tensor>& joints_3d_abs, const c10::optional<at::Tensor>& hand_verts_3d_abs, const c10::optional<at::Tensor>& joints_2d, const c10::optional<at::Tensor>& hand_verts_2d, const c10::optional<at::Tensor>& obj_center, const c10::optional<at::Tensor>& rotmat, const c10::optional<at::Tensor>& obj_verts_3d_abs, const c10::optional<at::Tensor>& obj_verts_2d, const c10::optional<at::Tensor>& corners_3d_abs, const c10::optional<at::Tensor>& corners_2d, const c10::optional<at::Tensor>& corners_3d, const c10::optional<at::Tensor>& obj_verts_3d) { static const char* const OP = "artiboost_hip::honet_recover_fwd"; ck_dev(OP, "hand_st", hand_st, (int)at::kFloat, false); ck_dev(OP, "obj_st", obj_st, (int)at::kFloat, false); ck_dev(OP, "cam_intr", cam_intr, (int)at::kFloat, true); ck_dev(OP, "joints_3d", joints_3d, (int)at::kFloat, true); ck_dev(OP, "hand_verts_3d", hand_verts_3d, (int)at::kFloat, true); ck_dev(OP, "obj_verts_can", obj_verts_can, (int)at::kFloat, true); ck_dev(OP, "corners_can", corners_can, (int)at::kFloat, true); ck_dev(OP, "root_joint", root_joint, (int)at::kFloat, true); ck_dev(OP, "joints_3d_abs", joints_3d_abs, (int)at::kFloat, true); ck_dev(OP, "hand_verts_3d_abs", hand_verts_3d_abs, (int)at::kFloat, true); ck_dev(OP, "joints_2d", joints_2d, (int)at::kFloat, true); ck_dev(OP, "hand_verts_2d", hand_verts_2d, (int)at::kFloat, true); ck_dev(OP, "obj_center", obj_center, (int)at::kFloat, true); ck_dev(OP, "rotmat", rotmat, (int)at::kFloat, true); ck_dev(OP, "obj_verts_3d_abs", obj_verts_3d_abs, (int)at::kFloat, true); ck_dev(OP, "obj_verts_2d", obj_verts_2d, (int)at::kFloat, true); ck_dev(OP, "corners_3d_abs", corners_3d_abs, (int)at::kFloat, true); ck_dev(OP, "corners_2d", corners_2d, (int)at::kFloat, true); ck_dev(OP, "corners_3d", corners_3d, (int)at::kFloat, true); ck_dev(OP, "obj_verts_3d", obj_verts_3d, (int)at::kFloat, true); ck_numel(OP, "cam_intr", cam_intr, (int64_t)(B*9)); ck_numel(OP, "rotmat", rotmat, (int64_t)(B*9)); ck_numel(OP, "joints_3d", joints_3d, (int64_t)(B*63)); ck_numel(OP, "joints_3d_abs", joints_3d_abs, (int64_t)(B*63)); ck_numel(OP, "hand_verts_3d", hand_verts_3d, (int64_t)(B*778*3)); ck_numel(OP, "hand_verts_3d_abs", hand_verts_3d_abs, (int64_t)(B*778*3)); ck_numel(OP, "obj_verts_can", obj_verts_can, (int64_t)(B*N*3)); ck_numel(OP, "obj_verts_3d_abs", obj_verts_3d_abs, (int64_t)(B*N*3)); ck_numel(OP, "obj_verts_3d", obj_verts_3d, (int64_t)(B*N*3)); ck_numel(OP, "corners_can", corners_can, (int64_t)(B*24)); ck_numel(OP, "corners_3d_abs", corners_3d_abs, (int64_t)(B*24)); ck_numel(OP, "corners_3d", corners_3d, (int64_t)(B*24)); ck_numel(OP, "root_joint", root_joint, (int64_t)(B*3)); ck_numel(OP, "obj_center", obj_center, (int64_t)(B*3)); ck_numel(OP, "joints_2d", joints_2d, (int64_t)(B*42)); ck_numel(OP, "hand_verts_2d", hand_verts_2d, (int64_t)(B*778*2)); ck_numel(OP, "obj_verts_2d", obj_verts_2d, (int64_t)(B*N*2)); ck_numel(OP, "corners_2d", corners_2d, (int64_t)(B*16)); const long rc = (long)ab_honet_recover_fwd((const float*)p(hand_st), (int)hand_pitch, (const float*)p(obj_st), (int)obj_pitch, (const float*)p(cam_intr), (const float*)p(joints_3d), (const float*)p(hand_verts_3d), (const float*)p(obj_verts_can), (const float*)p(corners_can), (int)B, (int)N, (float)trans_factor, (float)scale_factor, (float)img_w, (float)img_h, (float)off_z, (float*)p(root_joint), (float*)p(joints_3d_abs), (float*)p(hand_verts_3d_abs), (float*)p(joints_2d), (float*)p(hand_verts_2d), (float*)p(obj_center), (float*)p(rotmat), (float*)p(obj_verts_3d_abs), (float*)p(obj_verts_2d), (float*)p(corners_3d_abs), (float*)p(corners_2d), (float*)p(corners_3d), (float*)p(obj_verts_3d), cur_stream()); TORCH_CHECK(rc == 0, "ab_honet_recover_fwd failed with code ", rc, rc > 0 ? " (hipError)" : " (argument error)"); }
static void w_honet_recover_bwd(const c10::optional<at::Tensor>& hand_st, int64_t hand_pitch, const c10::optional<at::Tensor>& obj_st, int64_t obj_pitch, const c10::optional<at::Tensor>& cam_intr, const c10::optional<at::Tensor>& joints_3d, const c10::optional<at::Tensor>& hand_verts_3d, const c10::optional<at::Tensor>& obj_verts_can, const c10::optional<at::Tensor>& corners_can, int64_t B, int64_t N, double trans_factor, double scale_factor, double img_w, double img_h, double off_z, const c10::optional<at::Tensor>& g_root_joint, const c10::optional<at::Tensor>& g_joints_3d_abs, const c10::optional<at::Tensor>& g_hand_verts_3d_abs, const c10::optional<at::Tensor>& g_joints_2d, const c10::optional<at::Tensor>& g_hand_verts_2d, const c10::optional<at::Tensor>& g_obj_center, const c10::optional<at::Tensor>& g_rotmat, const c10::optional<at::Tensor>& g_obj_verts_3d_abs, const c10::optional<at::Tensor>& g_obj_verts_2d, const c10::optional<at::Tensor>& g_corners_3d_abs, const c10::optional<at::Tensor>& g_corners_2d, const c10::optional<at::Tensor>& g_corners_3d, const c10::optional<at::Tensor>& g_obj_verts_3d, const c10::optional<at::Tensor>& g_hand_st, int64_t g_hand_pitch, const c10::optional<at::Tensor>& g_obj_st, int64_t g_obj_pitch, const c10::optional<at::Tensor>& g_joints_3d, const c10::optional<at::Tensor>& g_hand_verts_3d, const c10::optional<at::Tensor>& workspace) { static const char* const OP = "artiboost_hip::honet_recover_bwd"; ck_dev(OP, "hand_st", hand_st, (int)at::kFloat, false); ck_dev(OP, "obj_st", obj_st, (int)at::kFloat, false); ck_dev(OP, "cam_intr", cam_intr, (int)at::kFloat, true); ck_dev(OP, "joints_3d", joints_3d, (int)at::kFloat, true); ck_dev(OP, "hand_verts_3d", hand_verts_3d, (int)at::kFloat, true); ck_dev(OP, "obj_verts_can", obj_verts_can, (int)at::kFloat, true); ck_dev(OP, "corners_can", corners_can, (int)at::kFloat, true); ck_dev(OP, "g_root_joint", g_root_joint, (int)at::kFloat, true); ck_dev(OP, "g_joints_3d_abs", g_joints_3d_abs, (int)at::kFloat, true); ck_dev(OP, "g_hand_verts_3d_abs", g_hand_verts_3d_abs, (int)at::kFloat, true); ck_dev(OP, "g_joints_2d", g_joints_2d, (int)at::kFloat, true); ck_dev(OP, "g_hand_verts_2d", g_hand_verts_2d, (int)at::kFloat, true); ck_dev(OP, "g_obj_center", g_obj_center, (int)at::kFloat, true); ck_dev(OP, "g_rotmat", g_rotmat, (int)at::kFloat, true); ck_dev(OP, "g_obj_verts_3d_abs", g_obj_verts_3d_abs, (int)at::kFloat, true); ck_dev(OP, "g_obj_verts_2d", g_obj_verts_2d, (int)at::kFloat, true); ck_dev(OP, "g_corners_3d_abs", g_corners_3d_abs, (int)at::kFloat, true); ck_dev(OP, "g_corners_2d", g_corners_2d, (int)at::kFloat, true); ck_dev(OP, "g_corners_3d", g_corners_3d, (int)at::kFloat, true); ck_dev(OP, "g_obj_verts_3d", g_obj_verts_3d, (int)at::kFloat, true); ck_dev(OP, "g_hand_st", g_hand_st, (int)at::kFloat, false); ck_dev(OP, "g_obj_st", g_obj_st, (int)at::kFloat, false); ck_dev(OP, "g_joints_3d", g_joints_3d, (int)at::kFloat, true); ck_dev(OP, "g_hand_verts_3d", g_hand_verts_3d, (int)at::kFloat, true); ck_dev(OP, "workspace", workspace, (int)-1, true); ck_numel(OP, "cam_intr", cam_intr, (int64_t)(B*9)); ck_numel(OP, "g_rotmat", g_rotmat, (int64_t)(B*9)); ck_numel(OP, "joints_3d", joints_3d, (int64_t)(B*63)); ck_numel(OP, "g_joints_3d_abs", g_joints_3d_abs, (int64_t)(B*63)); ck_numel(OP, "g_joints_3d", g_joints_3d, (int64_t)(B*63)); ck_numel(OP, "hand_verts_3d", hand_verts_3d, (int64_t)(B*778*3)); ck_numel(OP, "g_hand_verts_3d_abs", g_hand_verts_3d_abs, (int64_t)(B*778*3)); ck_numel(OP, "g_hand_verts_3d", g_hand_verts_3d, (int64_t)(B*778*3)); ck_numel(OP, "obj_verts_can", obj_verts_can, (int64_t)(B*N*3)); ck_numel(OP, "g_obj_verts_3d_abs", g_obj_verts_3d_abs, (int64_t)(B*N*3)); ck_numel(OP, "g_obj_verts_3d", g_obj_verts_3d, (int64_t)(B*N*3)); ck_numel(OP, "corners_can", corners_can, (int64_t)(B*24)); ck_numel(OP, "g_corners_3d_abs", g_corners_3d_abs, (int64_t)(B*24)); ck_numel(OP, "g_corners_3d", g_corners_3d, (int64_t)(B*24)); ck_numel(OP, "g_root_joint", g_root_joint, (int64_t)(B*3)); ck_numel(OP, "g_obj_center", g_obj_center, (int64_t)(B*3)); ck_numel(OP, "g_joints_2d", g_joints_2d, (int64_t)(B*42)); ck_numel(OP, "g_hand_verts_2d", g_hand_verts_2d, (int64_t)(B*778*2)); ck_numel(OP, "g_obj_verts_2d", g_obj_verts_2d, (int64_t)(B*N*2)); ck_numel(OP, "g_corners_2d", g_corners_2d, (int64_t)(B*16)); ck_bytes(OP, "workspace", workspace, (int64_t)(ab_honet_recover_workspace(B,N))); const long rc = (long)ab_honet_recover_bwd((const float*)p(hand_st), (int)hand_pitch, (const float*)p(obj_st), (int)obj_pitch, (const float*)p(cam_intr), (const float*)p(joints_3d), (const float*)p(hand_verts_3d), (const float*)p(obj_verts_can), (const float*)p(corners_can), (int)B, (int)N, (float)trans_factor, (float)scale_factor, (float)img_w, (float)img_h, (float)off_z, (const float*)p(g_root_joint), (const float*)p(g_joints_3d_abs), (const float*)p(g_hand_verts_3d_abs), (const float*)p(g_joints_2d), (const float*)p(g_hand_verts_2d), (const float*)p(g_obj_center), (const float*)p(g_rotmat), (const float*)p(g_obj_verts_3d_abs), (const float*)p(g_obj_verts_2d), (const float*)p(g_corners_3d_abs), (const float*)p(g_corners_2d), (const float*)p(g_corners_3d), (const float*)p(g_obj_verts_3d), (float*)p(g_hand_st), (int)g_hand_pitch, (float*)p(g_obj_st), (int)g_obj_pitch, (float*)p(g_joints_3d), (float*)p(g_hand_verts_3d), (void*)p(workspace), cur_stream()); TORCH_CHECK(rc == 0, "ab_honet_recover_bwd failed with code ", rc, rc > 0 ? " (hipError)" : " (argument error)"); }
static void w_mesh_queries(const c10::optional<at::Tensor>& table, int64_t n_obj, int64_t n, const c10::optional<at::Tensor>& obj_id, const c10::optional<at::Tensor>& obj_transf, const c10::optional<at::Tensor>& root_joint, const c10::optional<at::Tensor>& hand_verts, const c10::optional<at::Tensor>& samples, int64_t sample_pitch, int64_t pose_offset, int64_t B, const c10::optional<at::Tensor>& obj_verts_can, const c10::optional<at::Tensor>& obj_verts_3d, const c10::optional<at::Tensor>& hand_verts_3d) { static const char* const OP = "artiboost_hip::mesh_queries"; ck_dev(OP, "table", table, (int)at::kFloat, true); ck_dev(OP, "obj_id", obj_id, (int)at::kLong, true); ck_dev(OP, "obj_transf", obj_transf, (int)at::kFloat, true); ck_dev(OP, "root_joint", root_joint, (int)at::kFloat, true); ck_dev(OP, "hand_verts", hand_verts, (int)at::kFloat, true); ck_dev(OP, "samples", samples, (int)at::kByte, true); ck_dev(OP, "obj_verts_can", obj_verts_can, (int)at::kFloat, true); ck_dev(OP, "obj_verts_3d", obj_verts_3d, (int)at::kFloat, true); ck_dev(OP, "hand_verts_3d", hand_verts_3d, (int)at::kFloat, true); ck_numel(OP, "table", table, (int64_t)(n_obj*n*3)); ck_numel(OP, "obj_id", obj_id, (int64_t)(B)); ck_numel(OP, "obj_transf", obj_transf, (int64_t)(B*16)); ck_numel(OP, "root_joint", root_joint, (int64_t)(B*3)); ck_numel(OP, "hand_verts", hand_verts, (int64_t)(B*778*3)); ck_numel(OP, "hand_verts_3d", hand_verts_3d, (int64_t)(B*778*3)); ck_bytes(OP, "samples", samples, (int64_t)((B-1)*sample_pitch+pose_offset+64)); ck_numel(OP, "obj_verts_can", obj_verts_can, (int64_t)(B*n*3)); ck_numel(OP, "obj_verts_3d", obj_verts_3d, (int64_t)(B*n*3)); const long rc = (long)ab_mesh_queries((const float*)p(table), (int)n_obj, (int)n, (const int64_t*)p(obj_id), (const float*)p(obj_transf), (const float*)p(root_joint), (const float*)p(hand_verts), (const uint8_t*)p(samples), (long)sample_pitch, (long)pose_offset, (int)B, (float*)p(obj_verts_can), (float*)p(obj_verts_3d), (float*)p(hand_verts_3d), cur_stream()); TORCH_CHECK(rc == 0, "ab_mesh_queries failed with code ", rc, rc > 0 ? " (hipError)" : " (argument error)"); }
static void w_real_mesh_queries(const c10::optional<at::Tensor>& table, int64_t n_rows, int64_t n, const c10::optional<at::Tensor>& row, const c10::optional<at::Tensor>& obj_map, const c10::optional<at::Tensor>& hand_map, const c10::optional<at::Tensor>& mano_verts, int64_t B, const c10::optional<at::Tensor>& obj_verts_can, const c10::optional<at::Tensor>& obj_verts_3d, const c10::optional<at::Tensor>& hand_verts_3d) { static const char* const OP = "artiboost_hip::real_mesh_queries"; ck_dev(OP, "table", table, (int)at::kFloat, true); ck_dev(OP, "row", row, (int)at::kLong, true); ck_dev(OP, "obj_map", obj_map, (int)at::kFloat, true); ck_dev(OP, "hand_map", hand_map, (int)at::kFloat, true); ck_dev(OP, "mano_verts", mano_verts, (int)at::kFloat, true); ck_dev(OP, "obj_verts_can", obj_verts_can, (int)at::kFloat, true); ck_dev(OP, "obj_verts_3d", obj_verts_3d, (int)at::kFloat, true); ck_dev(OP, "hand_verts_3d", hand_verts_3d, (int)at::kFloat, true); ck_numel(OP, "table", table, (int64_t)(n_rows*n*3)); ck_numel(OP, "row", row, (int64_t)(B)); ck_numel(OP, "obj_map", obj_map, (int64_t)(B*12)); ck_numel(OP, "hand_map", hand_map, (int64_t)(B*12)); ck_numel(OP, "mano_verts", mano_verts, (int64_t)(B*778*3)); ck_numel(OP, "hand_verts_3d", hand_verts_3d, (int64_t)(B*778*3)); ck_numel(OP, "obj_verts_can", obj_verts_can, (int64_t)(B*n*3)); ck_numel(OP, "obj_verts_3d", obj_verts_3d, (int64_t)(B*n*3)); const long rc = (long)ab_real_mesh_queries((const float*)p(table), (int)n_rows, (int)n, (const int64_t*)p(row), (const float*)p(obj_map), (const float*)p(hand_map), (const float*)p(mano_verts), (int)B, (float*)p(obj_verts_can), (float*)p(obj_verts_3d), (float*)p(hand_verts_3d), cur_stream()); TORCH_CHECK(rc == 0, "ab_real_mesh_queries failed with code ", rc, rc > 0 ? " (hipError)" : " (argument error)"); }
static int64_t w_honet_loss_chunks(int64_t N) { return (int64_t)ab_honet_loss_chunks((int)N); }
static int64_t w_honet_loss_workspace(int64_t B, int64_t N) { return (int64_t)ab_honet_loss_workspace((int)B, (int)N); }
static void w_honet_loss(const c10::optional<at::Tensor>& joints_3d_abs, const c10::optional<at::Tensor>& hand_verts_3d_abs, const c10::optional<at::Tensor>& obj_verts_3d_abs, const c10::optional<at::Tensor>& corners_3d_abs, const c10::optional<at::Tensor>& mano_pca_pose, const c10::optional<at::Tensor>& mano_shape, const c10::optional<at::Tensor>& root_joint, const c10::optional<at::Tensor>& joints_3d, const c10::optional<at::Tensor>& hand_verts_3d, const c10::optional<at::Tensor>& obj_verts_3d, const c10::optional<at::Tensor>& corners_3d, int64_t B, int64_t N, int64_t ncomps, const c10::optional<at::Tensor>& weights7_host, const c10::optional<at::Tensor>& sample_part, const c10::optional<at::Tensor>& losses, const c10::optional<at::Tensor>& g_joints_3d_abs, const c10::optional<at::Tensor>& g_hand_verts_3d_abs, const c10::optional<at::Tensor>& g_obj_verts_3d_abs, const c10::optional<at::Tensor>& g_mano_pca_pose, const c10::optional<at::Tensor>& g_mano_shape, const c10::optional<at::Tensor>& workspace) { static const char* const OP = "artiboost_hip::honet_loss"; ck_dev(OP, "joints_3d_abs", joints_3d_abs, (int)at::kFloat, true); ck_dev(OP, "hand_verts_3d_abs", hand_verts_3d_abs, (int)at::kFloat, true); ck_dev(OP, "obj_verts_3d_abs", obj_verts_3d_abs, (int)at::kFloat, true); ck_dev(OP, "corners_3d_abs", corners_3d_abs, (int)at::kFloat, true); ck_dev(OP, "mano_pca_pose", mano_pca_pose, (int)at::kFloat, true); ck_dev(OP, "mano_shape", mano_shape, (int)at::kFloat, true); ck_dev(OP, "root_joint", root_joint, (int)at::kFloat, true); ck_dev(OP, "joints_3d", joints_3d, (int)at::kFloat, true); ck_dev(OP, "hand_verts_3d", hand_verts_3d, (int)at::kFloat, true); ck_dev(OP, "obj_verts_3d", obj_verts_3d, (int)at::kFloat, true); ck_dev(OP, "corners_3d", corners_3d, (int)at::kFloat, true); ck_host(OP, "weights7_host", weights7_host); ck_dev(OP, "sample_part", sample_part, (int)at::kFloat, true); ck_dev(OP, "losses", losses, (int)at::kFloat, true); ck_dev(OP, "g_joints_3d_abs", g_joints_3d_abs, (int)at::kFloat, true); ck_dev(OP, "g_hand_verts_3d_abs", g_hand_verts_3d_abs, (int)at::kFloat, true); ck_dev(OP, "g_obj_verts_3d_abs", g_obj_verts_3d_abs, (int)at::kFloat, true); ck_dev(OP, "g_mano_pca_pose", g_mano_pca_pose, (int)at::kFloat, true); ck_dev(OP, "g_mano_shape", g_mano_shape, (int)at::kFloat, true); ck_dev(OP, "workspace", workspace, (int)-1, true); ck_numel(OP, "joints_3d_abs", joints_3d_abs, (int64_t)(B*63)); ck_numel(OP, "joints_3d", joints_3d, (int64_t)(B*63)); ck_numel(OP, "g_joints_3d_abs", g_joints_3d_abs, (int64_t)(B*63)); ck_numel(OP, "hand_verts_3d_abs", hand_verts_3d_abs, (int64_t)(B*778*3)); ck_numel(OP, "hand_verts_3d", hand_verts_3d, (int64_t)(B*778*3)); ck_numel(OP, "g_hand_verts_3d_abs", g_hand_verts_3d_abs, (int64_t)(B*778*3)); ck_numel(OP, "obj_verts_3d_abs", obj_verts_3d_abs, (int64_t)(B*N*3)); ck_numel(OP, "obj_verts_3d", obj_verts_3d, (int64_t)(B*N*3)); ck_numel(OP, "g_obj_verts_3d_abs", g_obj_verts_3d_abs, (int64_t)(B*N*3)); ck_numel(OP, "corners_3d_abs", corners_3d_abs, (int64_t)(B*24)); ck_numel(OP, "corners_3d", corners_3d, (int64_t)(B*24)); ck_numel(OP, "mano_pca_pose", mano_pca_pose, (int64_t)(B*(3+ncomps))); ck_numel(OP, "g_mano_pca_pose", g_mano_pca_pose, (int64_t)(B*(3+ncomps))); ck_numel(OP, "mano_shape", mano_shape, (int64_t)(B*10)); ck_numel(OP, "g_mano_shape", g_mano_shape, (int64_t)(B*10)); ck_numel(OP, "root_joint", root_joint, (int64_t)(B*3)); ck_numel(OP, "weights7_host", weights7_host, (int64_t)(7)); ck_numel(OP, "sample_part", sample_part, (int64_t)(B*8)); ck_numel(OP, "losses", losses, (int64_t)(8)); ck_bytes(OP, "workspace", workspace, (int64_t)(ab_honet_loss_workspace(B,N))); const long rc = (long)ab_honet_loss((const float*)p(joints_3d_abs), (const float*)p(hand_verts_3d_abs), (const float*)p(obj_verts_3d_abs), (const float*)p(corners_3d_abs), (const float*)p(mano_pca_pose), (const float*)p(mano_shape), (const float*)p(root_joint), (const float*)p(joints_3d), (const float*)p(hand_verts_3d), (const float*)p(obj_verts_3d), (const float*)p(corners_3d), (int)B, (int)N, (int)ncomps, (const float*)p(weights7_host), (float*)p(sample_part), (float*)p(losses), (float*)p(g_joints_3d_abs), (float*)p(g_hand_verts_3d_abs), (float*)p(g_obj_verts_3d_abs), (float*)p(g_mano_pca_pose), (float*)p(g_mano_shape), (void*)p(workspace), cur_stream()); TORCH_CHECK(rc == 0, "ab_honet_loss failed with code ", rc, rc > 0 ? " (hipError)" : " (argument error)"); }
static void w_mano_fit(const c10::optional<at::Tensor>& quat, const c10::optional<at::Tensor>& pred_joints, const c10::optional<at::Tensor>& v_template, const c10::optional<at::Tensor>& shapedirs, const c10::optional<at::Tensor>& posedirs, const c10::optional<at::Tensor>& J_regressor, const c10::optional<at::Tensor>& weights, const c10::optional<at::Tensor>& J_template, const c10::optional<at::Tensor>& J_shapedirs, int64_t B, int64_t n_iter, int64_t step0, int64_t init, const c10::optional<at::Tensor>& params, const c10::optional<at::Tensor>& adam_m, const c10::optional<at::Tensor>& adam_v, const c10::optional<at::Tensor>& verts, const c10::optional<at::Tensor>& joints, const c10::optional<at::Tensor>& loss, const c10::optional<at::Tensor>& grad) { static const char* const OP = "artiboost_hip::mano_fit"; ck_dev(OP, "quat", quat, (int)at::kFloat, true); ck_dev(OP, "pred_joints", pred_joints, (int)at::kFloat, true); ck_dev(OP, "v_template", v_template, (int)at::kFloat, true); ck_dev(OP, "shapedirs", shapedirs, (int)at::kFloat, true); ck_dev(OP, "posedirs", posedirs, (int)at::kFloat, true); ck_dev(OP, "J_regressor", J_regressor, (int)at::kFloat, true); ck_dev(OP, "weights", weights, (int)at::kFloat, true); ck_dev(OP, "J_template", J_template, (int)at::kFloat, true); ck_dev(OP, "J_shapedirs", J_shapedirs, (int)at::kFloat, true); ck_dev(OP, "params", params, (int)at::kFloat, true); ck_dev(OP, "adam_m", adam_m, (int)at::kFloat, true); ck_dev(OP, "adam_v", adam_v, (int)at::kFloat, true); ck_dev(OP, "verts", verts, (int)at::kFloat, true); ck_dev(OP, "joints", joints, (int)at::kFloat, true); ck_dev(OP, "loss", loss, (int)at::kFloat, true); ck_dev(OP, "grad", grad, (int)at::kFloat, true); ck_numel(OP, "quat", quat, (int64_t)(B*64)); ck_numel(OP, "pred_joints", pred_joints, (int64_t)(B*63)); ck_numel(OP, "v_template", v_template, (int64_t)(778*3)); ck_numel(OP, "shapedirs", shapedirs, (int64_t)(778*3*10)); ck_numel(OP, "posedirs", posedirs, (int64_t)(778*3*135)); ck_numel(OP, "J_regressor", J_regressor, (int64_t)(16*778)); ck_numel(OP, "weights", weights, (int64_t)(778*16)); ck_numel(OP, "J_template", J_template, (int64_t)(48)); ck_numel(OP, "J_shapedirs", J_shapedirs, (int64_t)(480)); ck_numel(OP, "params", params, (int64_t)(B*59)); ck_numel(OP, "adam_m", adam_m, (int64_t)(B*59)); ck_numel(OP, "adam_v", adam_v, (int64_t)(B*59)); ck_numel(OP, "grad", grad, (int64_t)(B*59)); ck_numel(OP, "verts", verts, (int64_t)(B*778*3)); ck_numel(OP, "joints", joints, (int64_t)(B*63)); ck_numel(OP, "loss", loss, (int64_t)(B*n_iter)); const long rc = (long)ab_mano_fit((const float*)p(quat), (const float*)p(pred_joints), (const float*)p(v_template), (const float*)p(shapedirs), (const float*)p(posedirs), (const float*)p(J_regressor), (const float*)p(weights), (const float*)p(J_template), (const float*)p(J_shapedirs), (int)B, (int)n_iter, (int)step0, (int)init, (float*)p(params), (float*)p(adam_m), (float*)p(adam_v), (float*)p(verts), (float*)p(joints), (float*)p(loss), (float*)p(grad), cur_stream()); TORCH_CHECK(rc == 0, "ab_mano_fit failed with code ", rc, rc > 0 ? " (hipError)" : " (argument error)"); }
static int64_t w_draw_workspace_bytes(int64_t B, int64_t W, int64_t H, int64_t max_obj_verts) { return (int64_t)ab_draw_workspace_bytes((int)B, (int)W, (int)H, (int)max_obj_verts); }
static int64_t w_draw_workspace_keys_offset(int64_t B, int64_t max_obj_verts) { return (int64_t)ab_draw_workspace_keys_offset((int)B, (int)max_obj_verts); }
// ... 111 lines not shown
    m.def("col_stats(Tensor? x, int dtype, int M, int C, Tensor(a!)? part) -> ()");
    m.def("bn_finalize(Tensor? part, int nparts, int C, int count, Tensor? gamma, Tensor? beta, float eps, float momentum, Tensor(a!)? running_mean, Tensor(b!)? running_var, Tensor(c!)? bnp) -> ()");
    m.def("bn_eval_params(int C, Tensor? gamma, Tensor? beta, Tensor? rm, Tensor? rv, float eps, Tensor(a!)? bnp) -> ()");
    m.def("bn_eval_params_batch(Tensor? flat, Tensor? stats, Tensor? desc_dev, int n, int max_c, float eps, Tensor(a!)? out) -> ()");
    m.def("bn_apply(Tensor? y, Tensor? res, Tensor? bnp, int dtype, int M, int C, int relu, Tensor(a!)? out) -> ()");
    m.def("bn_bwd(Tensor? dout, Tensor? out, Tensor? y, Tensor? bnp, int dtype, int M, int C, int relu, Tensor(a!)? part, Tensor(b!)? bwdp, Tensor(c!)? dgamma, Tensor(d!)? dbeta, Tensor(e!)? dy, Tensor(f!)? dz_out) -> ()");
    m.def("relu_bwd(Tensor? dout, Tensor? out, int dtype, int n, Tensor(a!)? dz) -> ()");
    m.def("col_sum(Tensor? x, int dtype, int M, int C, Tensor(a!)? part, Tensor(b!)? out) -> ()");
    m.def("col_sum_x3(Tensor? hi, Tensor? lo, int M, int C, Tensor(a!)? part, Tensor(b!)? out) -> ()");
    m.def("add(Tensor? a, Tensor? b, int dtype, int n, Tensor(a!)? out) -> ()");
    m.def("maxpool3x3s2_fwd(Tensor? x, int dtype, int N, int H, int W, int C, Tensor(a!)? out, Tensor(b!)? idx) -> ()");
    m.def("conv2d_dgrad_bnstats_rows(int dtype, int N, int H, int W, int Cin, int Cout, int kh, int kw, int stride, int pad) -> int");
    m.def("conv2d_dgrad_bnstats(Tensor? dy, Tensor? wt, Tensor(a!)? dx, int dtype, int N, int H, int W, int Cin, int Cout, int kh, int kw, int stride, int pad, Tensor? addend, Tensor? bn_y, Tensor? bn_out, Tensor? bnp, Tensor(b!)? bn_part) -> ()");
    m.def("bn_bwd_apply(Tensor? dout, Tensor? out, Tensor? y, Tensor? bnp, int dtype, int M, int C, int relu, Tensor? part, int nparts, Tensor(a!)? bwdp, Tensor(b!)? dgamma, Tensor(c!)? dbeta, Tensor(d!)? dy, Tensor(e!)? dz_out) -> ()");
    m.def("bn_relu_maxpool3x3s2_fwd(Tensor? y, Tensor? bnp, int dtype, int N, int H, int W, int C, Tensor(a!)? out, Tensor(b!)? idx) -> ()");
    m.def("bn_relu_maxpool3x3s2_fwd_x3(Tensor? y, Tensor? bnp, int N, int H, int W, int C, Tensor(a!)? out, Tensor(b!)? out_hi, Tensor(c!)? out_lo, Tensor(d!)? idx) -> ()");
    m.def("bn_relu_maxpool_bwd(Tensor? dpool, Tensor? idx, Tensor? y, Tensor? bnp, int dtype, int N, int H, int W, int C, Tensor(a!)? part, Tensor(b!)? bwdp, Tensor(c!)? dgamma, Tensor(d!)? dbeta, Tensor(e!)? dy) -> ()");
    m.def("bn_relu_maxpool_bwd_x3_nparts(int N, int H, int W, int C) -> int");
    m.def("bn_relu_maxpool_bwd_x3(Tensor? dpool, Tensor? idx, Tensor? y, Tensor? bnp, int N, int H, int W, int C, Tensor(a!)? part, Tensor(b!)? bwdp, Tensor(c!)? dgamma, Tensor(d!)? dbeta, Tensor(e!)? dz, Tensor(f!)? dy_hi, Tensor(g!)? dy_lo) -> ()");
    m.def("bn_relu_maxpool3x3s2_fwd_x3w(Tensor? y, Tensor? bnp, int N, int H, int W, int C, Tensor(a!)? out, Tensor(b!)? out_hi, Tensor(c!)? out_lo, Tensor(d!)? idx, Tensor(e!)? ywin) -> ()");
    m.def("bn_relu_maxpool_bwd_x3w(Tensor? dpool, Tensor? idx, Tensor? ywin, Tensor? y, Tensor? bnp, int N, int H, int W, int C, Tensor(a!)? part, Tensor(b!)? bwdp, Tensor(c!)? dgamma, Tensor(d!)? dbeta, Tensor(e!)? dy_hi, Tensor(f!)? dy_lo) -> ()");
    m.def("maxpool3x3s2_bwd(Tensor? idx, Tensor? dout, int dtype, int N, int H, int W, int C, Tensor(a!)? dx) -> ()");
    m.def("avgpool_fwd(Tensor? x, int dtype, int N, int HW, int C, Tensor(a!)? out) -> ()");
    m.def("avgpool_bwd(Tensor? g, int dtype, int N, int HW, int C, Tensor(a!)? dx, int accumulate) -> ()");
    m.def("cast_f32_bf16(Tensor? src, int n, Tensor(a!)? dst) -> ()");
    m.def("transpose_oki(Tensor? src, int O, int K, int I, int dtype, Tensor(a!)? dst) -> ()");
    m.def("transpose_oki_batch(Tensor? desc_dev, int ntensors, int total_tiles, int dtype) -> ()");
    m.def("transpose_oki_batch_x3(Tensor? desc_dev, int ntensors, int total_tiles, int lo_offset_elems) -> ()");
    m.def("image_pad_nhwc4(Tensor? img_nchw, int dtype, int N, int H, int W, Tensor(a!)? out) -> ()");
    m.def("grad_norm(Tensor? grad, int n, Tensor(a!)? part, Tensor(b!)? total_norm) -> ()");
    m.def("scale_f32(Tensor(a!)? x, int n, float s) -> ()");
    m.def("clip_adam(Tensor(a!)? param, Tensor? grad, Tensor(b!)? m, Tensor(c!)? v, int n, Tensor? total_norm, float max_norm, float lr, float beta1, float beta2, float eps, int step, Tensor? hyper, Tensor(d!)? lp) -> ()");
    m.def("clip_adam_x3(Tensor(a!)? param, Tensor? grad, Tensor(b!)? m, Tensor(c!)? v, int n, Tensor? total_norm, float max_norm, float lr, float beta1, float beta2, float eps, int step, Tensor? hyper, Tensor(d!)? lp_hi, Tensor(e!)? lp_lo) -> ()");
    m.def("pose_assemble(Tensor? kp3d, Tensor? box6d, int box_stride, Tensor? root_joint, Tensor? cam_intr, Tensor? corners_can, int B, int center_idx, float res_w, float res_h, Tensor(a!)? joints_abs, Tensor(b!)? corners_abs, Tensor(c!)? rotmat, Tensor(d!)? uvd2d, Tensor(e!)? joints_rel, Tensor(f!)? corners_rel, Tensor(g!)? boxroot) -> ()");
    m.def("pose_loss(Tensor? kp3d, Tensor? box6d, int box_stride, Tensor? root_joint, Tensor? cam_intr, Tensor? corners_can, Tensor? joints_3d, Tensor? corners_3d, Tensor? joints_vis, Tensor? corners_vis, Tensor? hand_views, int nvh, Tensor? j0, Tensor? j1, int njp, Tensor? p0, Tensor? p1, int npp, Tensor? scene_views, int nvs, Tensor? s0, Tensor? s1, int nsp, int B, int center_idx, float res_w, float res_h, Tensor? weights8_host, Tensor(a!)? joints_abs, Tensor(b!)? corners_abs, Tensor(c!)? rotmat, Tensor(d!)? uvd2d, Tensor(e!)? sample_part, Tensor(f!)? losses, Tensor(g!)? g_kp3d, Tensor(h!)? g_box6d) -> ()");
    m.def("pose_loss_sym(Tensor? kp3d, Tensor? box6d, int box_stride, Tensor? root_joint, Tensor? cam_intr, Tensor? corners_can, Tensor? joints_3d, Tensor? corners_3d, Tensor? joints_vis, Tensor? corners_vis, Tensor? hand_views, int nvh, Tensor? j0, Tensor? j1, int njp, Tensor? p0, Tensor? p1, int npp, Tensor? scene_views, int nvs, Tensor? s0, Tensor? s1, int nsp, int B, int center_idx, float res_w, float res_h, Tensor? weights8_host, Tensor? sym, Tensor(a!)? joints_abs, Tensor(b!)? corners_abs, Tensor(c!)? rotmat, Tensor(d!)? uvd2d, Tensor(e!)? sample_part, Tensor(f!)? losses, Tensor(g!)? g_kp3d, Tensor(h!)? g_box6d) -> ()");
    m.def("reg_pose_loss(Tensor? joints_pred, Tensor? mano_pca_pose, Tensor? mano_shape, Tensor? transf, int transf_stride, Tensor? root_joint, Tensor? cam_intr, Tensor? corners_can, Tensor? joints_3d, Tensor? corners_3d, Tensor? joints_vis, Tensor? corners_vis, Tensor? hand_views, int nvh, Tensor? j0, Tensor? j1, int njp, Tensor? p0, Tensor? p1, int npp, Tensor? scene_views, int nvs, Tensor? s0, Tensor? s1, int nsp, int B, int ncomps, Tensor? weights12_host, Tensor(a!)? joints_abs, Tensor(b!)? corners_abs, Tensor(c!)? rotmat, Tensor(d!)? sample_part, Tensor(e!)? losses, Tensor(f!)? g_joints, Tensor(g!)? g_pose, Tensor(h!)? g_shape, Tensor(i!)? g_transf) -> ()");
    m.def("render_workspace_bytes(int B, int W, int H, int max_faces) -> int");
    m.def("render_batch(Tensor? scene_host, Tensor? samples, Tensor? hand_verts, Tensor? order, Tensor? factor, Tensor? inv_affine, Tensor? blur_radius, int B, int max_faces, int ow, int oh, int out_dtype, Tensor(a!)? out_pad, Tensor(b!)? out_chw, Tensor(c!)? workspace, Tensor(d!)? keys_out, Tensor(e!)? rgbx_out) -> ()");
    m.def("gaussian_blur(Tensor? rgbx, int B, int W, int H, Tensor? radius, Tensor(a!)? out) -> ()");
    m.def("augment_workspace_bytes(int B, int W, int H) -> int");
    m.def("augment_batch(Tensor? rgbx, int B, int W, int H, Tensor? order, Tensor? factor, Tensor? inv_affine, Tensor? blur_radius, Tensor? flip, int ow, int oh, int out_dtype, Tensor(a!)? out_pad, Tensor(b!)? out_chw, Tensor(c!)? workspace) -> ()");
    m.def("jpeg_workspace_bytes(int total_blocks, int total_subseq, int plane_bytes, int data_bytes, int total_segs, int n, int n_tables) -> int");
    m.def("jpeg_decode_batch(Tensor? data, Tensor? desc, Tensor? segs, Tensor? qtabs, Tensor? htabs, int n, int n_tables, int sub_bytes, int total_blocks, int total_subseq, int plane_bytes, int data_bytes, int total_segs, int max_blocks, int max_width, int max_height, int max_subseq, int out_channels, Tensor(a!)? out, Tensor(b!)? workspace) -> ()");
    m.def("png_unfilter_batch(Tensor? raw, Tensor? desc, int n, int max_width, int max_bpp, int out_channels, Tensor(a!)? out, Tensor(b!)? status) -> ()");
    m.def("linear_fwd(Tensor? x, Tensor? w, Tensor? bias, int M, int N, int K, int relu, Tensor(a!)? y) -> ()");
    m.def("linear_dgrad(Tensor? g, Tensor? wt, Tensor? act_out, int M, int N, int K, Tensor(a!)? gx) -> ()");
    m.def("linear_wgrad(Tensor? g, Tensor? x, int M, int N, int K, Tensor(a!)? dw, Tensor(b!)? db) -> ()");
    m.def("nearest_dist(Tensor? x, Tensor? ypts, Tensor? obj_idx, Tensor? rot, int B, int P1, int P2, Tensor? scale, Tensor? shift, Tensor(a!)? dist, int ld, Tensor(b!)? idx_out) -> ()");
    m.def("linear_fused(Tensor? x, Tensor? w, Tensor? bias, Tensor? scale, Tensor? shift, Tensor? residual, int ldr, int M, int N, int K, int act, float slope, Tensor(a!)? y, int ldy) -> ()");
    m.def("color_jitter(Tensor? rgbx, int B, int npix, Tensor? order, Tensor? factor, Tensor(a!)? out, Tensor(b!)? lsum_ws) -> ()");
    m.def("mano_lbs(Tensor? pose, Tensor? betas, Tensor? v_template, Tensor? shapedirs, Tensor? posedirs, Tensor? J_regressor, Tensor? weights, Tensor? hands_mean, int B, Tensor(a!)? verts, Tensor(b!)? joints, Tensor(c!)? T_abs) -> ()");
    m.def("mano_pca_fwd(Tensor? pose_coeffs, Tensor? betas, Tensor? comps, Tensor? hands_mean, Tensor? v_template, Tensor? shapedirs, Tensor? posedirs, Tensor? J_regressor, Tensor? weights, int ncomps, int center_idx, int B, Tensor(a!)? verts, Tensor(b!)? joints, Tensor(c!)? full_pose) -> ()");
    m.def("mano_pca_bwd(Tensor? pose_coeffs, Tensor? betas, Tensor? comps, Tensor? hands_mean, Tensor? v_template, Tensor? shapedirs, Tensor? posedirs, Tensor? J_regressor, Tensor? weights, int ncomps, int center_idx, int B, Tensor? g_verts, Tensor? g_joints, Tensor? g_full_pose, Tensor(a!)? g_pose_coeffs, Tensor(b!)? g_betas) -> ()");
    m.def("honet_recover_chunks(int N) -> int");
    m.def("honet_recover_workspace(int B, int N) -> int");
    m.def("honet_recover_fwd(Tensor? hand_st, int hand_pitch, Tensor? obj_st, int obj_pitch, Tensor? cam_intr, Tensor? joints_3d, Tensor? hand_verts_3d, Tensor? obj_verts_can, Tensor? corners_can, int B, int N, float trans_factor, float scale_factor, float img_w, float img_h, float off_z, Tensor(a!)? root_joint, Tensor(b!)? joints_3d_abs, Tensor(c!)? hand_verts_3d_abs, Tensor(d!)? joints_2d, Tensor(e!)? hand_verts_2d, Tensor(f!)? obj_center, Tensor(g!)? rotmat, Tensor(h!)? obj_verts_3d_abs, Tensor(i!)? obj_verts_2d, Tensor(j!)? corners_3d_abs, Tensor(k!)? corners_2d, Tensor(l!)? corners_3d, Tensor(m!)? obj_verts_3d) -> ()");
    m.def("honet_recover_bwd(Tensor? hand_st, int hand_pitch, Tensor? obj_st, int obj_pitch, Tensor? cam_intr, Tensor? joints_3d, Tensor? hand_verts_3d, Tensor? obj_verts_can, Tensor? corners_can, int B, int N, float trans_factor, float scale_factor, float img_w, float img_h, float off_z, Tensor? g_root_joint, Tensor? g_joints_3d_abs, Tensor? g_hand_verts_3d_abs, Tensor? g_joints_2d, Tensor? g_hand_verts_2d, Tensor? g_obj_center, Tensor? g_rotmat, Tensor? g_obj_verts_3d_abs, Tensor? g_obj_verts_2d, Tensor? g_corners_3d_abs, Tensor? g_corners_2d, Tensor? g_corners_3d, Tensor? g_obj_verts_3d, Tensor(a!)? g_hand_st, int g_hand_pitch, Tensor(b!)? g_obj_st, int g_obj_pitch, Tensor(c!)? g_joints_3d, Tensor(d!)? g_hand_verts_3d, Tensor(e!)? workspace) -> ()");
    m.def("mesh_queries(Tensor? table, int n_obj, int n, Tensor? obj_id, Tensor? obj_transf, Tensor? root_joint, Tensor? hand_verts, Tensor? samples, int sample_pitch, int pose_offset, int B, Tensor(a!)? obj_verts_can, Tensor(b!)? obj_verts_3d, Tensor(c!)? hand_verts_3d) -> ()");
    m.def("real_mesh_queries(Tensor? table, int n_rows, int n, Tensor? row, Tensor? obj_map, Tensor? hand_map, Tensor? mano_verts, int B, Tensor(a!)? obj_verts_can, Tensor(b!)? obj_verts_3d, Tensor(c!)? hand_verts_3d) -> ()");
    m.def("honet_loss_chunks(int N) -> int");
    m.def("honet_loss_workspace(int B, int N) -> int");
    m.def("honet_loss(Tensor? joints_3d_abs, Tensor? hand_verts_3d_abs, Tensor? obj_verts_3d_abs, Tensor? corners_3d_abs, Tensor? mano_pca_pose, Tensor? mano_shape, Tensor? root_joint, Tensor? joints_3d, Tensor? hand_verts_3d, Tensor? obj_verts_3d, Tensor? corners_3d, int B, int N, int ncomps, Tensor? weights7_host, Tensor(a!)? sample_part, Tensor(b!)? losses, Tensor(c!)? g_joints_3d_abs, Tensor(d!)? g_hand_verts_3d_abs, Tensor(e!)? g_obj_verts_3d_abs, Tensor(f!)? g_mano_pca_pose, Tensor(g!)? g_mano_shape, Tensor(h!)? workspace) -> ()");
    m.def("mano_fit(Tensor? quat, Tensor? pred_joints, Tensor? v_template, Tensor? shapedirs, Tensor? posedirs, Tensor? J_regressor, Tensor? weights, Tensor? J_template, Tensor? J_shapedirs, int B, int n_iter, int step0, int init, Tensor(a!)? params, Tensor(b!)? adam_m, Tensor(c!)? adam_v, Tensor(d!)? verts, Tensor(e!)? joints, Tensor(f!)? loss, Tensor(g!)? grad) -> ()");
    m.def("draw_workspace_bytes(int B, int W, int H, int max_obj_verts) -> int");
    m.def("draw_workspace_keys_offset(int B, int max_obj_verts) -> int");
// ... 66 lines not shown
    m.impl("col_stats", &w_col_stats);
    m.impl("bn_finalize", &w_bn_finalize);
    m.impl("bn_eval_params", &w_bn_eval_params);
    m.impl("bn_eval_params_batch", &w_bn_eval_params_batch);
    m.impl("bn_apply", &w_bn_apply);
    m.impl("bn_bwd", &w_bn_bwd);
    m.impl("relu_bwd", &w_relu_bwd);
    m.impl("col_sum", &w_col_sum);
    m.impl("col_sum_x3", &w_col_sum_x3);
    m.impl("add", &w_add);
    m.impl("maxpool3x3s2_fwd", &w_maxpool3x3s2_fwd);
    m.impl("conv2d_dgrad_bnstats_rows", &w_conv2d_dgrad_bnstats_rows);
    m.impl("conv2d_dgrad_bnstats", &w_conv2d_dgrad_bnstats);
    m.impl("bn_bwd_apply", &w_bn_bwd_apply);
    m.impl("bn_relu_maxpool3x3s2_fwd", &w_bn_relu_maxpool3x3s2_fwd);
    m.impl("bn_relu_maxpool3x3s2_fwd_x3", &w_bn_relu_maxpool3x3s2_fwd_x3);
    m.impl("bn_relu_maxpool_bwd", &w_bn_relu_maxpool_bwd);
    m.impl("bn_relu_maxpool_bwd_x3_nparts", &w_bn_relu_maxpool_bwd_x3_nparts);
    m.impl("bn_relu_maxpool_bwd_x3", &w_bn_relu_maxpool_bwd_x3);
    m.impl("bn_relu_maxpool3x3s2_fwd_x3w", &w_bn_relu_maxpool3x3s2_fwd_x3w);
    m.impl("bn_relu_maxpool_bwd_x3w", &w_bn_relu_maxpool_bwd_x3w);
    m.impl("maxpool3x3s2_bwd", &w_maxpool3x3s2_bwd);
    m.impl("avgpool_fwd", &w_avgpool_fwd);
    m.impl("avgpool_bwd", &w_avgpool_bwd);
    m.impl("cast_f32_bf16", &w_cast_f32_bf16);
    m.impl("transpose_oki", &w_transpose_oki);
    m.impl("transpose_oki_batch", &w_transpose_oki_batch);
    m.impl("transpose_oki_batch_x3", &w_transpose_oki_batch_x3);
    m.impl("image_pad_nhwc4", &w_image_pad_nhwc4);
    m.impl("grad_norm", &w_grad_norm);
    m.impl("scale_f32", &w_scale_f32);
    m.impl("clip_adam", &w_clip_adam);
    m.impl("clip_adam_x3", &w_clip_adam_x3);
    m.impl("pose_assemble", &w_pose_assemble);
    m.impl("pose_loss", &w_pose_loss);
    m.impl("pose_loss_sym", &w_pose_loss_sym);
    m.impl("reg_pose_loss", &w_reg_pose_loss);
    m.impl("render_workspace_bytes", &w_render_workspace_bytes);
    m.impl("render_batch", &w_render_batch);
    m.impl("gaussian_blur", &w_gaussian_blur);
    m.impl("augment_workspace_bytes", &w_augment_workspace_bytes);
    m.impl("augment_batch", &w_augment_batch);
    m.impl("jpeg_workspace_bytes", &w_jpeg_workspace_bytes);
    m.impl("jpeg_decode_batch", &w_jpeg_decode_batch);
    m.impl("png_unfilter_batch", &w_png_unfilter_batch);
    m.impl("linear_fwd", &w_linear_fwd);
    m.impl("linear_dgrad", &w_linear_dgrad);
    m.impl("linear_wgrad", &w_linear_wgrad);
    m.impl("nearest_dist", &w_nearest_dist);
    m.impl("linear_fused", &w_linear_fused);
    m.impl("color_jitter", &w_color_jitter);
    m.impl("mano_lbs", &w_mano_lbs);
    m.impl("mano_pca_fwd", &w_mano_pca_fwd);
    m.impl("mano_pca_bwd", &w_mano_pca_bwd);
    m.impl("honet_recover_chunks", &w_honet_recover_chunks);
    m.impl("honet_recover_workspace", &w_honet_recover_workspace);
    m.impl("honet_recover_fwd", &w_honet_recover_fwd);
    m.impl("honet_recover_bwd", &w_honet_recover_bwd);
    m.impl("mesh_queries", &w_mesh_queries);
    m.impl("real_mesh_queries", &w_real_mesh_queries);
    m.impl("honet_loss_chunks", &w_honet_loss_chunks);
    m.impl("honet_loss_workspace", &w_honet_loss_workspace);
    m.impl("honet_loss", &w_honet_loss);
    m.impl("mano_fit", &w_mano_fit);
    m.impl("draw_workspace_bytes", &w_draw_workspace_bytes);
    m.impl("draw_workspace_keys_offset", &w_draw_workspace_keys_offset);
// ... 8 lines not shown
```

artiboost_amd/hybridnet.py:

```python
from collections import OrderedDict

import os

import torch

from . import kernels as K
from .head import softargmax3d_fwd, softargmax3d_bwd, softargmax3d_bwd_x3, softargmax3d_stage2

RESNET34_LAYERS = [3, 4, 6, 3]
DEPTH_PITCH = 32
BOX_OUT_PAD = 64


class _Entry:
    __slots__ = ("name", "kind", "ref_shape", "kshape", "offset", "numel", "bn")

    def __init__(self, name, kind, ref_shape, kshape):
        self.name, self.kind, self.ref_shape, self.kshape = name, kind, tuple(ref_shape), tuple(kshape)
        self.numel = 1
        for d in kshape:
            self.numel *= d
        self.offset = 0


# ... 241 lines not shown
            elif e.kind in ("linear", "linear_pad", "frozen") and len(shp) == 2:
                bound = 1.0 / math.sqrt(shp[1])
                sd[name] = (torch.rand(shp, generator=g) * 2 - 1) * bound
            elif name.endswith(".weight") and e.kind == "vec":
                sd[name] = torch.ones(shp)
            elif "box_head" in name or "fc.bias" in name or name.startswith(("mano_branch.", "obj_transfhead.", "mano_transhead.", "obj_transhead.")):
                fan_in = self.entries[name.replace(".bias", ".weight")].ref_shape[1]
                sd[name] = (torch.rand(shp, generator=g) * 2 - 1) / math.sqrt(fan_in)
            else:
                sd[name] = torch.zeros(shp)
        for name, (_, c) in self.buffers.items():
            sd[name] = torch.ones(c) if name.endswith("running_var") else torch.zeros(c)
        self.load_reference_state_dict(sd)


class HybridNet:

    def __init__(self, store: ParamStore, image_size=(256, 256), compute_dtype=torch.bfloat16):
        self.p = store
        self.W, self.H = int(image_size[0]), int(image_size[1])
        self.x3 = compute_dtype in ("bf16x3", "x3")
        self.dtype = torch.float32 if self.x3 else compute_dtype
        self.training = True
        self.image_plane = "f32"
        self.norm = 0
        self.frozen_bn = False
        self.lp = None
        self.tr = {}
        self._packed = False
        self.saved = None
        self.last = None
        self.eval_fold = True
        self._tr_plan = None
        self._eval_desc = None
        self._eval_bnp = None
        self._zparts = {}
        self._g3 = None
        self._head_full = None
        self._wgrp = []
        self._wgrp_key = None
        self._wgrp_max = {}

    def _dgrad_names(self):
        names = []
        for name, e in self.p.entries.items():
            if e.kind in ("conv", "deconv", "final_w"):
                names.append(name)
        return names

    def refresh_after_update(self, lp_fresh=False):
        self.pack_weights(skip_cast=lp_fresh)

    def pack_weights(self, skip_cast=False):
        p = self.p
        if self.x3:
            if self.lp is None or tuple(self.lp.shape) != (2, p.total):
                self.lp = torch.empty((2, p.total), dtype=torch.bfloat16, device=p.device)
                skip_cast = False
            if not skip_cast:
                K.split(p.flat, out=self.lp)
        elif self.dtype == torch.bfloat16:
            if self.lp is None or self.lp.dtype != torch.bfloat16:
                self.lp = torch.empty(p.total, dtype=torch.bfloat16, device=p.device)
                skip_cast = False
            if not skip_cast:
                K.cast_bf16(p.flat, self.lp)
        else:
            self.lp = p.flat
        if self._tr_plan is None:
            pairs = []
            if self.x3:
                tot = sum(_round_up(p.entries[n].numel, 64) for n in self._dgrad_names())
                self._tr_planes = torch.zeros((2, tot), dtype=torch.bfloat16, device=p.device)
                self._tr_lo_off = tot
                off = 0
            for name in self._dgrad_names():
                O, kh, kw, I = p.entries[name].kshape
                if self.x3:
                    n = p.entries[name].numel
                    dst = self._tr_planes[0, off:off + n].view(I, kh, kw, O)
                    self.tr[name] = self._tr_planes[:, off:off + n].view(2, I, kh, kw, O)
                    off += _round_up(n, 64)
                else:
                    dst = self.tr[name] = torch.empty((I, kh, kw, O), dtype=self.dtype, device=p.device)
                pairs.append((p.view(name).reshape(O, kh * kw, I), dst))
            self._tr_pairs = pairs
            self._tr_plan = K.transpose_plan(pairs) or False
            self.box_t, bpairs = {}, []
            lin = (("box_head.layers.0.weight", "box_head.layers.2.weight", "box_head.layers.4.weight") if p.box_head else
                   tuple(n for n, e in p.entries.items() if e.kind in ("linear", "linear_pad")) if p.trunk_only else ())
            for name in lin:
                O, _, _, I = p.entries[name].kshape
                dst = self.box_t[name] = torch.empty((I, O), dtype=torch.float32, device=p.device)
                bpairs.append((p.view(name).reshape(O, 1, I), dst.view(I, 1, O)))
            self._box_pairs = bpairs
            self._box_plan = (K.transpose_plan(bpairs) or False) if bpairs else False
        if self._box_plan:
            K.transpose_oki_batch(self._box_plan)
        else:
            for src, dst in self._box_pairs:
                dst.copy_(src.permute(2, 1, 0))
        if self.x3:
            if not self._tr_plan:
                raise RuntimeError("bf16x3 needs the batched transpose plan (channel counts multiples of 8 / 4)")
            K.transpose_oki_batch_x3(self._tr_plan, self._tr_lo_off)
        elif self._tr_plan:
            K.transpose_oki_batch(self._tr_plan)
        else:
            for src, dst in self._tr_pairs:
                K.transpose_oki(src, dst)
        self._packed = True

    def w(self, name):
        e = self.p.entries[name]
        if self.x3:
            return self.lp[:, e.offset:e.offset + e.numel].view((2,) + e.kshape)
        return self.lp[e.offset:e.offset + e.numel].view(e.kshape)

    def _conv_fwd(self, x, name, stride, pad, **kw):
        if kw.get("want_stats") and not self.training:
            kw = dict(kw, want_stats=False)
            fn = K.conv2d_fwd_x3 if self.x3 else K.conv2d_fwd
            return fn(x, self.w(name), stride, pad, **kw), None
        if self.x3:
            return K.conv2d_fwd_x3(x, self.w(name), stride, pad, **kw)
        return K.conv2d_fwd(x, self.w(name), stride, pad, **kw)

    def _conv_dgrad(self, dy, name, in_hw, stride, pad, addend=None, bn=None, want_stats=False):
        if self.x3:
# ... 439 lines not shown
```

artiboost_amd/kernels.py:

```python
import ctypes

import torch

from . import _lib as L


def _empty(shape, like, dtype=None):
    return torch.empty(shape, dtype=dtype or like.dtype, device=like.device)


def conv_out(h, k, s, p):
    return (h + 2 * p - k) // s + 1


def conv2d_fwd(x, w_ohwi, stride, pad, bias=None, want_stats=False, relu=False):
    N, H, W, Cin = x.shape
    Cout, kh, kw, _ = w_ohwi.shape
    Ho, Wo = conv_out(H, kh, stride, pad), conv_out(W, kw, stride, pad)
    y = _empty((N, Ho, Wo, Cout), x)
    lib = L.lib()
    stats = None
    if want_stats:
        nt = lib.ab_conv2d_stat_rows(L.i(L.dt(x)), L.i(N), L.i(H), L.i(W), L.i(Cin), L.i(Cout), L.i(kh), L.i(kw), L.i(stride), L.i(pad), L.i(0))
        stats = torch.empty((nt, Cout, 2), dtype=torch.float32, device=x.device)
# ... 318 lines not shown
def linear_wgrad(g, x, dw, db=None):
    M, N = g.shape
    Kd = x.shape[1]
    L.check(L.lib().ab_linear_wgrad(L.ptr(g), L.ptr(x), L.i(M), L.i(N), L.i(Kd), L.ptr(dw), L.ptr(db), L.stream()),
            "ab_linear_wgrad")


def transpose_plan(pairs):
    import numpy as np
    rec = np.zeros(len(pairs), dtype=np.dtype([("src", "<u8"), ("dst", "<u8"), ("O", "<i4"), ("K", "<i4"), ("I", "<i4"),
                                               ("tile_begin", "<i4")]))
    tiles = 0
    for n, (src, dst) in enumerate(pairs):
        O, Kk, I = src.shape
        if I % 4 or O % 8 or not src.is_contiguous() or not dst.is_contiguous() or dst.dtype != pairs[0][1].dtype:
            return None
        rec[n] = (src.data_ptr(), dst.data_ptr(), O, Kk, I, tiles)
        tiles += ((O + 63) // 64) * Kk * ((I + 63) // 64)
    dev = torch.from_numpy(rec.view(np.uint8).copy()).to(pairs[0][0].device)
    return dev, len(pairs), tiles, L.dt(pairs[0][1])


def transpose_oki_batch(plan):
    dev, n, tiles, dt = plan
    L.check(L.lib().ab_transpose_oki_batch(L.ptr(dev), L.i(n), L.l(tiles), L.i(dt), L.stream()), "ab_transpose_oki_batch")


def transpose_oki_batch_x3(plan, lo_offset_elems):
    dev, n, tiles, dt = plan
    assert dt == L.DT_BF16
    L.check(L.lib().ab_transpose_oki_batch_x3(L.ptr(dev), L.i(n), L.l(tiles), L.l(lo_offset_elems), L.stream()), "ab_transpose_oki_batch_x3")


def image_pad_nhwc4(img_nchw_f32, dtype):
    N, C, H, W = img_nchw_f32.shape
    assert C == 3
    out = torch.empty((N, H + 6, W + 8, 4), dtype=dtype, device=img_nchw_f32.device)
    L.check(L.lib().ab_image_pad_nhwc4(L.ptr(img_nchw_f32), L.i(L.dt(out)), L.i(N), L.i(H), L.i(W), L.ptr(out),
                                       L.stream()), "ab_image_pad_nhwc4")
    return out


def relu_bwd(dout, out):
    dz = torch.empty_like(dout)
    L.check(L.lib().ab_relu_bwd(L.ptr(dout), L.ptr(out), L.i(L.dt(dout)), L.l(dout.numel()), L.ptr(dz), L.stream()),
            "ab_relu_bwd")
    return dz


def col_sum(x, out):
    C = x.shape[-1]
    M = x.numel() // C
    lib = L.lib()
    part = torch.empty((lib.ab_col_stats_nparts(L.l(M)), C, 2), dtype=torch.float32, device=x.device)
    L.check(lib.ab_col_sum(L.ptr(x), L.i(L.dt(x)), L.l(M), L.i(C), L.ptr(part), L.ptr(out), L.stream()), "ab_col_sum")
    return out



def split(x_f32, out=None):
    if x_f32.dtype != torch.float32:
        raise TypeError("split() takes a float32 tensor")
    sp = out if out is not None else torch.empty((2,) + tuple(x_f32.shape), dtype=torch.bfloat16, device=x_f32.device)
    L.check(L.lib().ab_split_f32(L.ptr(x_f32), L.l(x_f32.numel()), L.ptr(sp[0]), L.ptr(sp[1]), L.stream()), "ab_split_f32")
    return sp

# ... 564 lines not shown
```

artiboost_amd/optim.py:

```python
import torch

from . import _lib as L


class FusedClipAdam(torch.optim.Optimizer):

    def __init__(self, params, lr=5e-5, betas=(0.9, 0.999), eps=1e-8, weight_decay=0.0, max_norm=None, model=None):
        if weight_decay:
            raise NotImplementedError("weight_decay (the reference trains with WEIGHT_DECAY: 0)")
        super().__init__(params, dict(lr=lr, betas=betas, eps=eps))
        self.max_norm = max_norm
        self.model = model
        self._part = None
        self.total_norm = None
        self.hyper = None
        self._hyper_host = None
        self.graph_steps = 0
        self._eager_hyper = None

    HYPER_SLOTS = 32

    def use_device_hyper(self, device):
        self.hyper = torch.zeros(3, dtype=torch.float32, device=device)
        self._hyper_host = torch.zeros((self.HYPER_SLOTS, 3), dtype=torch.float32).pin_memory()
        self._hyper_events = [None] * self.HYPER_SLOTS
        self._hyper_next = 0

    def advance_hyper(self):
        self.graph_steps += 1
        for st in self.state.values():
            st["step"] = self.graph_steps
        g = self.param_groups[0]
        b1, b2 = g["betas"]
        k = self._hyper_next
        self._hyper_next = (k + 1) % self.HYPER_SLOTS
        if self._hyper_events[k] is not None:
            self._hyper_events[k].synchronize()
        slot = self._hyper_host[k]
        slot[0] = g["lr"]
        slot[1] = 1.0 - b1 ** self.graph_steps
        slot[2] = (1.0 - b2 ** self.graph_steps) ** 0.5
        self.hyper.copy_(slot, non_blocking=True)
        ev = self._hyper_events[k] or torch.cuda.Event()
        ev.record()
        self._hyper_events[k] = ev

    def state_dict(self):
        sd = super().state_dict()
        sd["graph_steps"] = self.graph_steps
        return sd

    def load_state_dict(self, state_dict):
        state_dict = dict(state_dict)
        self.graph_steps = int(state_dict.pop("graph_steps", 0))
        super().load_state_dict(state_dict)
        for st in self.state.values():
            self.graph_steps = max(self.graph_steps, int(st.get("step", 0)))

    def grad_norm(self, grad):
        if self._part is None:
            self._part = torch.empty(1024, dtype=torch.float32, device=grad.device)
            self.total_norm = torch.empty(1, dtype=torch.float32, device=grad.device)
        L.check(L.lib().ab_grad_norm(L.ptr(grad), L.l(grad.numel()), L.ptr(self._part), L.ptr(self.total_norm),
                                     L.stream()), "ab_grad_norm")
        return self.total_norm

    @torch.no_grad()
    def step(self, closure=None):
        for group in self.param_groups:
            for p in group["params"]:
                if p.grad is None:
                    continue
                st = self.state[p]
                if not st:
                    st["step"] = 0
                    st["exp_avg"] = torch.zeros_like(p)
                    st["exp_avg_sq"] = torch.zeros_like(p)
                st["step"] += 1
                g = p.grad
                tn = self.grad_norm(g) if self.max_norm else None
                lp = lp_planes = None
                net = self.model.net if (self.model is not None and p is self.model.flat_param) else None
                if net is not None and getattr(net, "x3", False):
                    if net.lp is None or tuple(net.lp.shape) != (2, p.numel()):
                        net.lp = torch.empty((2, p.numel()), dtype=torch.bfloat16, device=p.device)
                    lp_planes = net.lp
                elif net is not None and net.dtype == torch.bfloat16:
                    if net.lp is None or net.lp.dtype != torch.bfloat16:
                        net.lp = torch.empty(p.numel(), dtype=torch.bfloat16, device=p.device)
                    lp = net.lp
                b1, b2 = group["betas"]
                hyper = self.hyper
                if hyper is None:
                    if self._eager_hyper is None or self._eager_hyper.device != p.device:
                        self._eager_hyper = torch.zeros(3, dtype=torch.float32, device=p.device)
                    hyper = self._eager_hyper
                    hyper.copy_(torch.tensor([group["lr"], 1.0 - b1 ** st["step"], (1.0 - b2 ** st["step"]) ** 0.5], dtype=torch.float32))
                if lp_planes is not None:
                    L.check(L.lib().ab_clip_adam_x3(L.ptr(p), L.ptr(g), L.ptr(st["exp_avg"]), L.ptr(st["exp_avg_sq"]),
                                                    L.l(p.numel()), L.ptr(tn), L.f(self.max_norm or 0.0), L.f(group["lr"]),
                                                    L.f(b1), L.f(b2), L.f(group["eps"]), L.i(st["step"]), L.ptr(hyper),
                                                    L.ptr(lp_planes[0]), L.ptr(lp_planes[1]), L.stream()), "ab_clip_adam_x3")
                else:
                    L.check(L.lib().ab_clip_adam(L.ptr(p), L.ptr(g), L.ptr(st["exp_avg"]), L.ptr(st["exp_avg_sq"]),
                                                 L.l(p.numel()), L.ptr(tn), L.f(self.max_norm or 0.0), L.f(group["lr"]),
                                                 L.f(b1), L.f(b2), L.f(group["eps"]), L.i(st["step"]), L.ptr(hyper),
                                                 L.ptr(lp), L.stream()), "ab_clip_adam")
                if net is not None:
                    net.refresh_after_update(lp_fresh=lp is not None or lp_planes is not None)
        return None
```

include/artiboost_hip.h:

```cpp
#ifndef ARTIBOOST_HIP_H
#define ARTIBOOST_HIP_H
#include <stdint.h>
#ifdef __cplusplus
extern "C" {
#endif

#define AB_DT_F32 0
#define AB_DT_BF16 1
#define AB_DT_U8N 2
#define AB_EINVAL (-1)
#define AB_ESHAPE (-2)
#define AB_EALIGN (-3)

int ab_abi_version(void);

int ab_wall_stamp(int64_t* slot, void* stream);
int ab_wall_clock_khz(void);

int ab_softargmax3d_ntiles(int H, int W);
int ab_softargmax3d_fwd(const void* logits, int dtype, int B, int C, int D, int DP, int H, int W,
                        float* part, float* uvd, float* conf, float* stat, void* stream);
int ab_softargmax3d_bwd(const void* logits, int dtype, int B, int C, int D, int DP, int H, int W,
                        const float* uvd, const float* conf, const float* stat,
                        const float* g_uvd, const float* g_conf, void* dlogits, void* stream);
// ... 148 lines not shown
                           int W, int C, float* part, float* bwdp, float* dgamma, float* dbeta, void* dy, void* stream);
int ab_bn_relu_maxpool_bwd_x3_nparts(int N, int H, int W, int C);
int ab_bn_relu_maxpool_bwd_x3(const float* dpool, const void* idx, const float* y, const float* bnp, int N, int H, int W,
                              int C, float* part, float* bwdp, float* dgamma, float* dbeta, float* dz, void* dy_hi,
                              void* dy_lo, void* stream);
int ab_bn_relu_maxpool3x3s2_fwd_x3w(const float* y, const float* bnp, int N, int H, int W, int C, float* out, void* out_hi,
                                    void* out_lo, void* idx, float* ywin, void* stream);
int ab_bn_relu_maxpool_bwd_x3w(const float* dpool, const void* idx, const float* ywin, const float* y, const float* bnp, int N, int H,
                               int W, int C, float* part, float* bwdp, float* dgamma, float* dbeta, void* dy_hi, void* dy_lo,
                               void* stream);
int ab_maxpool3x3s2_bwd(const void* idx, const void* dout, int dtype, int N, int H, int W, int C, void* dx, void* stream);
int ab_avgpool_fwd(const void* x, int dtype, int N, int HW, int C, float* out, void* stream);
int ab_avgpool_bwd(const float* g, int dtype, int N, int HW, int C, void* dx, int accumulate, void* stream);
int ab_cast_f32_bf16(const float* src, long n, void* dst, void* stream);
int ab_transpose_oki(const float* src, int O, int K, int I, int dtype, void* dst, void* stream);
typedef struct ab_transpose_desc {
    const void* src;
    void* dst;
    int32_t O, K, I;
    int32_t tile_begin;
} ab_transpose_desc;
int ab_transpose_oki_batch(const ab_transpose_desc* desc_dev, int ntensors, long total_tiles, int dtype, void* stream);
int ab_transpose_oki_batch_x3(const ab_transpose_desc* desc_dev, int ntensors, long total_tiles, long lo_offset_elems, void* stream);
int ab_image_pad_nhwc4(const float* img_nchw, int dtype, int N, int H, int W, void* out, void* stream);

int ab_grad_norm(const float* grad, long n, float* part, float* total_norm, void* stream);
int ab_scale_f32(float* x, long n, float s, void* stream);
int ab_clip_adam(float* param, const float* grad, float* m, float* v, long n, const float* total_norm,
                 float max_norm, float lr, float beta1, float beta2, float eps, int step, const float* hyper,
                 void* lp, void* stream);
int ab_clip_adam_x3(float* param, const float* grad, float* m, float* v, long n, const float* total_norm,
                    float max_norm, float lr, float beta1, float beta2, float eps, int step,
                    const float* hyper, void* lp_hi, void* lp_lo, void* stream);

int ab_pose_assemble(const float* kp3d, const float* box6d, int box_stride, const float* root_joint, const float* cam_intr,
                     const float* corners_can, int B, int center_idx, float res_w, float res_h, float* joints_abs,
                     float* corners_abs, float* rotmat, float* uvd2d, float* joints_rel, float* corners_rel, float* boxroot,
                     void* stream);
int ab_pose_loss(const float* kp3d, const float* box6d, int box_stride, const float* root_joint,
                 const float* cam_intr, const float* corners_can, const float* joints_3d, const float* corners_3d,
                 const float* joints_vis, const float* corners_vis, const float* hand_views, int nvh,
                 const int64_t* j0, const int64_t* j1, int njp, const int64_t* p0, const int64_t* p1, int npp,
                 const float* scene_views, int nvs, const int64_t* s0, const int64_t* s1, int nsp, int B,
                 int center_idx, float res_w, float res_h, const float* weights8_host, float* joints_abs,
                 float* corners_abs, float* rotmat, float* uvd2d, float* sample_part, float* losses, float* g_kp3d,
                 float* g_box6d, void* stream);
typedef struct ab_symcorner {
    const float* R;
    const float* t;
    int32_t K;
    const int64_t* obj_idx;
    const float* obj_transf;
    float lambda;
    float weight;
    float* loss_out;
} ab_symcorner;
int ab_pose_loss_sym(const float* kp3d, const float* box6d, int box_stride, const float* root_joint,
                     const float* cam_intr, const float* corners_can, const float* joints_3d, const float* corners_3d,
                     const float* joints_vis, const float* corners_vis, const float* hand_views, int nvh,
                     const int64_t* j0, const int64_t* j1, int njp, const int64_t* p0, const int64_t* p1, int npp,
                     const float* scene_views, int nvs, const int64_t* s0, const int64_t* s1, int nsp, int B,
                     int center_idx, float res_w, float res_h, const float* weights8_host, const ab_symcorner* sym,
                     float* joints_abs, float* corners_abs, float* rotmat, float* uvd2d, float* sample_part, float* losses,
                     float* g_kp3d, float* g_box6d, void* stream);
int ab_reg_pose_loss(const float* joints_pred, const float* mano_pca_pose, const float* mano_shape, const float* transf,
                     int transf_stride, const float* root_joint, const float* cam_intr, const float* corners_can,
// ... 113 lines not shown
```

Measured before the change: 7415 samples/s.

## Fuse Adam update with weight-layout transposes and grad-norm finalize

```diff
diff --git a/artiboost_amd/csrc/optim.hip b/artiboost_amd/csrc/optim.hip
--- a/artiboost_amd/csrc/optim.hip
+++ b/artiboost_amd/csrc/optim.hip
@@ -26,6 +26,27 @@
 #pragma unroll
     for (int o = 32; o > 0; o >>= 1) s += __shfl_xor(s, o, 64);
     if (threadIdx.x == 0) out[0] = (float)sqrt(s);
+}
+
+__device__ __forceinline__ void adam4(float4& pv, const float4& gv, float4& mv, float4& vv, float coef, float step, float b1, float b2, float eps,
+                                      float bc2_sqrt, uint2& hi, uint2& lo) {
+    float pp[4] = {pv.x, pv.y, pv.z, pv.w}, gg[4] = {gv.x, gv.y, gv.z, gv.w};
+    float mm[4] = {mv.x, mv.y, mv.z, mv.w}, vvv[4] = {vv.x, vv.y, vv.z, vv.w};
+#pragma unroll
+    for (int k = 0; k < 4; ++k) {
+        float gk = gg[k] * coef;
+        mm[k] = mm[k] * b1 + (1.f - b1) * gk;
+        vvv[k] = vvv[k] * b2 + (1.f - b2) * gk * gk;
+        float denom = sqrtf(vvv[k]) / bc2_sqrt + eps;
+        pp[k] = pp[k] - step * (mm[k] / denom);
+    }
+    pv = make_float4(pp[0], pp[1], pp[2], pp[3]);
+    mv = make_float4(mm[0], mm[1], mm[2], mm[3]);
+    vv = make_float4(vvv[0], vvv[1], vvv[2], vvv[3]);
+    hi.x = pack_bf16x2(pp[0], pp[1]);
+    hi.y = pack_bf16x2(pp[2], pp[3]);
+    lo.x = pack_bf16x2(pp[0] - __uint_as_float(hi.x << 16), pp[1] - __uint_as_float(hi.x & 0xffff0000u));
+    lo.y = pack_bf16x2(pp[2] - __uint_as_float(hi.y << 16), pp[3] - __uint_as_float(hi.y & 0xffff0000u));
 }
 
 __global__ __launch_bounds__(OPT_THREADS) void clip_adam_kernel(float* __restrict__ p, const float* __restrict__ g,
@@ -41,39 +62,26 @@
     long nvec = n / 4;
     for (long i = (long)blockIdx.x * OPT_THREADS + threadIdx.x; i < nvec; i += (long)gridDim.x * OPT_THREADS) {
         float4 pv = ((float4*)p)[i], gv = ((const float4*)g)[i], mv = ((float4*)m)[i], vv = ((float4*)v)[i];
-        float pp[4] = {pv.x, pv.y, pv.z, pv.w}, gg[4] = {gv.x, gv.y, gv.z, gv.w};
-        float mm[4] = {mv.x, mv.y, mv.z, mv.w}, vvv[4] = {vv.x, vv.y, vv.z, vv.w};
-#pragma unroll
-        for (int k = 0; k < 4; ++k) {
-            float gk = gg[k] * coef;
-            mm[k] = mm[k] * b1 + (1.f - b1) * gk;
-            vvv[k] = vvv[k] * b2 + (1.f - b2) * gk * gk;
-            float denom = sqrtf(vvv[k]) / bc2_sqrt + eps;
-            pp[k] = pp[k] - step * (mm[k] / denom);
-        }
-        ((float4*)p)[i] = make_float4(pp[0], pp[1], pp[2], pp[3]);
-        ((float4*)m)[i] = make_float4(mm[0], mm[1], mm[2], mm[3]);
-        ((float4*)v)[i] = make_float4(vvv[0], vvv[1], vvv[2], vvv[3]);
+        uint2 hi, lo;
+        adam4(pv, gv, mv, vv, coef, step, b1, b2, eps, bc2_sqrt, hi, lo);
+        ((float4*)p)[i] = pv;
+        ((float4*)m)[i] = mv;
+        ((float4*)v)[i] = vv;
         if (lp) {
-            uint2 o;
-            o.x = pack_bf16x2(pp[0], pp[1]);
-            o.y = pack_bf16x2(pp[2], pp[3]);
-            ((uint2*)lp)[i] = o;
-            if (lp_lo) {
-                uint2 l;
-                l.x = pack_bf16x2(pp[0] - __uint_as_float(o.x << 16), pp[1] - __uint_as_float(o.x & 0xffff0000u));
-                l.y = pack_bf16x2(pp[2] - __uint_as_float(o.y << 16), pp[3] - __uint_as_float(o.y & 0xffff0000u));
-                ((uint2*)lp_lo)[i] = l;
-            }
-        }
-    }
-}
-
+            ((uint2*)lp)[i] = hi;
+            if (lp_lo) ((uint2*)lp_lo)[i] = lo;
+        }
+    }
+}
+
+static int norm_parts(long n) {
+    long b = (n / 4 + OPT_THREADS - 1) / OPT_THREADS;
+    return (int)(b > OPT_MAX_PARTS ? OPT_MAX_PARTS : (b < 1 ? 1 : b));
+}
 extern "C" int ab_grad_norm(const float* grad, long n, float* part, float* total_norm, void* stream) {
     if (!grad || !part || !total_norm) return AB_EINVAL;
     if (n % 4) return AB_ESHAPE;
-    long b = (n / 4 + OPT_THREADS - 1) / OPT_THREADS;
-    int nb = (int)(b > OPT_MAX_PARTS ? OPT_MAX_PARTS : (b < 1 ? 1 : b));
+    const int nb = norm_parts(n);
     sqnorm_kernel<<<nb, OPT_THREADS, 0, as_stream(stream)>>>(grad, n, part);
     AB_LAUNCH_CHECK();
     norm_finalize_kernel<<<1, 64, 0, as_stream(stream)>>>(part, nb, total_norm);
@@ -137,6 +145,144 @@
     return 0;
 }
 
+__device__ __forceinline__ void store_bf16x8(bf16_t* p, const float* f) {
+    *(uint4*)p = make_uint4(pack_bf16x2(f[0], f[1]), pack_bf16x2(f[2], f[3]), pack_bf16x2(f[4], f[5]), pack_bf16x2(f[6], f[7]));
+}
+
+__global__ __launch_bounds__(OPT_THREADS) void clip_adam_layouts_kernel(float* __restrict__ p, const float* __restrict__ g, float* __restrict__ m,
+                                                                        float* __restrict__ v, float* __restrict__ total_norm,
+                                                                        const float* __restrict__ part, int nparts, float max_norm, float lr,
+                                                                        float b1, float b2, float eps, float bc1, float bc2_sqrt,
+                                                                        const float* __restrict__ hyper, bf16_t* __restrict__ lp,
+                                                                        bf16_t* __restrict__ lp_lo, const ab_adam_tile_desc* __restrict__ tiles,
+                                                                        int ntensors, unsigned ntiles, const ab_adam_range* __restrict__ ranges) {
+    __shared__ float sm[64][65];
+    if (hyper) { lr = hyper[0]; bc1 = hyper[1]; bc2_sqrt = hyper[2]; }
+    const float step = lr / bc1;
+    float coef = 1.f;
+    if (max_norm > 0.f) {
+        double s = 0.0;
+        for (int i = threadIdx.x & 63; i < nparts; i += 64) s += part[i];
+#pragma unroll
+        for (int o = 32; o > 0; o >>= 1) s += __shfl_xor(s, o, 64);
+        const float tn = (float)sqrt(s);
+        if (blockIdx.x == 0 && threadIdx.x == 0) total_norm[0] = tn;
+        coef = max_norm / (tn + 1e-6f);
+        coef = coef > 1.f ? 1.f : coef;
+    }
+    if (blockIdx.x >= ntiles) {
+        const ab_adam_range rg = ranges[blockIdx.x - ntiles];
+        for (long i = rg.begin / 4 + threadIdx.x; i < rg.end / 4; i += OPT_THREADS) {
+            float4 pv = ((float4*)p)[i], gv = ((const float4*)g)[i], mv = ((float4*)m)[i], vv = ((float4*)v)[i];
+            uint2 hi, lo;
+            adam4(pv, gv, mv, vv, coef, step, b1, b2, eps, bc2_sqrt, hi, lo);
+            ((float4*)p)[i] = pv;
+            ((float4*)m)[i] = mv;
+            ((float4*)v)[i] = vv;
+            ((uint2*)lp)[i] = hi;
+            ((uint2*)lp_lo)[i] = lo;
+        }
+        return;
+    }
+    int t = 0;
+    for (int hi_t = ntensors; hi_t - t > 1;) {
+        const int mid = (t + hi_t) >> 1;
+        if (blockIdx.x >= (unsigned)tiles[mid].tile_begin) t = mid; else hi_t = mid;
+    }
+    const ab_adam_tile_desc d = tiles[t];
+    const int O = d.O, K = d.K, I = d.I;
+    const int ti = (I + 63) / 64;
+    long tile = (long)blockIdx.x - d.tile_begin;
+    const int it = (int)(tile % ti); tile /= ti;
+    const int k = (int)(tile % K); const int ot = (int)(tile / K);
+    const int o0 = ot * 64, i0 = it * 64;
+    {
+        const int c4 = (threadIdx.x & 15) * 4, r = threadIdx.x >> 4;
+        float4 pv[4], gv[4], mv[4], vv[4];
+        long e[4];
+#pragma unroll
+        for (int pass = 0; pass < 4; ++pass) {
+            const int o = o0 + r + pass * 16, i = i0 + c4;
+            e[pass] = (o < O && i < I) ? (d.flat_off + ((long)o * K + k) * I + i) / 4 : -1;
+            pv[pass] = gv[pass] = mv[pass] = vv[pass] = make_float4(0.f, 0.f, 0.f, 0.f);
+            if (e[pass] >= 0) {
+                pv[pass] = ((float4*)p)[e[pass]]; gv[pass] = ((const float4*)g)[e[pass]];
+                mv[pass] = ((float4*)m)[e[pass]]; vv[pass] = ((float4*)v)[e[pass]];
+            }
+        }
+#pragma unroll
+        for (int pass = 0; pass < 4; ++pass) {
+            if (e[pass] >= 0) {
+                uint2 hi, lo;
+                adam4(pv[pass], gv[pass], mv[pass], vv[pass], coef, step, b1, b2, eps, bc2_sqrt, hi, lo);
+                ((float4*)p)[e[pass]] = pv[pass];
+                ((float4*)m)[e[pass]] = mv[pass];
+                ((float4*)v)[e[pass]] = vv[pass];
+                ((uint2*)lp)[e[pass]] = hi;
+                ((uint2*)lp_lo)[e[pass]] = lo;
+            }
+            float* row = &sm[r + pass * 16][c4];
+            row[0] = pv[pass].x; row[1] = pv[pass].y; row[2] = pv[pass].z; row[3] = pv[pass].w;
+        }
+    }
+    __syncthreads();
+    if (d.kind == 0) {
+        bf16_t* __restrict__ dst = (bf16_t*)d.dst;
+        const int cv = (threadIdx.x & 7) * 8, r = threadIdx.x >> 3;
+#pragma unroll
+        for (int pass = 0; pass < 2; ++pass) {
+            const int il = r + pass * 32;
+            const int i = i0 + il, o = o0 + cv;
+            if (i < I && o < O) {
+                float f[8];
+#pragma unroll
+                for (int q = 0; q < 8; ++q) f[q] = sm[cv + q][il];
+                store_bf16x8(dst + ((long)i * K + k) * O + o, f);
+#pragma unroll
+                for (int q = 0; q < 8; ++q) f[q] -= bf16_to_f32(f32_to_bf16(f[q]));
+                store_bf16x8(dst + d.lo_off + ((long)i * K + k) * O + o, f);
+            }
+        }
+    } else {
+        float* __restrict__ dst = (float*)d.dst;
+        const int cv = (threadIdx.x & 15) * 4, r = threadIdx.x >> 4;
+#pragma unroll
+        for (int pass = 0; pass < 4; ++pass) {
+            const int il = r + pass * 16;
+            const int i = i0 + il, o = o0 + cv;
+            if (i < I && o < O)
+                *(float4*)(dst + ((long)i * K + k) * O + o) = make_float4(sm[cv][il], sm[cv + 1][il], sm[cv + 2][il], sm[cv + 3][il]);
+        }
+    }
+}
+
+extern "C" int ab_grad_norm_parts(long n) { return norm_parts(n); }
+
+extern "C" int ab_grad_sqnorm(const float* grad, long n, float* part, void* stream) {
+    if (!grad || !part) return AB_EINVAL;
+    if (n % 4) return AB_ESHAPE;
+    sqnorm_kernel<<<norm_parts(n), OPT_THREADS, 0, as_stream(stream)>>>(grad, n, part);
+    AB_LAUNCH_CHECK();
+    return 0;
+}
+
+extern "C" int ab_clip_adam_layouts(float* param, const float* grad, float* m, float* v, long n, float* total_norm, float max_norm, float lr,
+                                    float beta1, float beta2, float eps, int step, const float* hyper, void* lp_hi, void* lp_lo,
+                                    const ab_adam_tile_desc* tiles_dev, int ntensors, long total_tiles, const ab_adam_range* ranges_dev,
+                                    long nranges, const float* part, int nparts, void* stream) {
+    if (!param || !grad || !m || !v || !lp_hi || !lp_lo) return AB_EINVAL;
+    if (max_norm > 0.f && (!total_norm || !part || nparts < 1 || nparts > OPT_MAX_PARTS)) return AB_EINVAL;
+    if (ntensors < 0 || total_tiles < 0 || nranges < 0 || (total_tiles > 0) != (ntensors > 0)) return AB_EINVAL;
+    if ((total_tiles && !tiles_dev) || (nranges && !ranges_dev)) return AB_EINVAL;
+    if (n % 4 || step < 1 || total_tiles + nranges < 1 || total_tiles + nranges > 0x7fffffffL) return AB_ESHAPE;
+    double bc1 = 1.0 - pow((double)beta1, (double)step), bc2 = 1.0 - pow((double)beta2, (double)step);
+    clip_adam_layouts_kernel<<<(unsigned)(total_tiles + nranges), OPT_THREADS, 0, as_stream(stream)>>>(
+        param, grad, m, v, total_norm, part, nparts, max_norm, lr, beta1, beta2, eps, (float)bc1, (float)sqrt(bc2), hyper, (bf16_t*)lp_hi,
+        (bf16_t*)lp_lo, tiles_dev, ntensors, (unsigned)total_tiles, ranges_dev);
+    AB_LAUNCH_CHECK();
+    return 0;
+}
+
 
 __global__ void wall_stamp_kernel(int64_t* slot) { *slot = (int64_t)wall_clock64(); }
 extern "C" int ab_wall_stamp(int64_t* slot, void* stream) {
diff --git a/artiboost_amd/csrc/torch_ops_gen.cpp b/artiboost_amd/csrc/torch_ops_gen.cpp
--- a/artiboost_amd/csrc/torch_ops_gen.cpp
+++ b/artiboost_amd/csrc/torch_ops_gen.cpp
@@ -130,6 +130,9 @@
 static void w_scale_f32(const c10::optional<at::Tensor>& x, int64_t n, double s) { static const char* const OP = "artiboost_hip::scale_f32"; ck_dev(OP, "x", x, (int)at::kFloat, true); ck_numel(OP, "x", x, (int64_t)(n)); const long rc = (long)ab_scale_f32((float*)p(x), (long)n, (float)s, cur_stream()); TORCH_CHECK(rc == 0, "ab_scale_f32 failed with code ", rc, rc > 0 ? " (hipError)" : " (argument error)"); }
 static void w_clip_adam(const c10::optional<at::Tensor>& param, const c10::optional<at::Tensor>& grad, const c10::optional<at::Tensor>& m, const c10::optional<at::Tensor>& v, int64_t n, const c10::optional<at::Tensor>& total_norm, double max_norm, double lr, double beta1, double beta2, double eps, int64_t step, const c10::optional<at::Tensor>& hyper, const c10::optional<at::Tensor>& lp) { static const char* const OP = "artiboost_hip::clip_adam"; ck_dev(OP, "param", param, (int)at::kFloat, true); ck_dev(OP, "grad", grad, (int)at::kFloat, true); ck_dev(OP, "m", m, (int)at::kFloat, true); ck_dev(OP, "v", v, (int)at::kFloat, true); ck_dev(OP, "total_norm", total_norm, (int)at::kFloat, true); ck_dev(OP, "hyper", hyper, (int)at::kFloat, true); ck_dev(OP, "lp", lp, (int)-1, true); ck_dtype(OP, "lp", lp, at::kBFloat16); ck_numel(OP, "param", param, (int64_t)(n)); ck_numel(OP, "grad", grad, (int64_t)(n)); ck_numel(OP, "m", m, (int64_t)(n)); ck_numel(OP, "v", v, (int64_t)(n)); ck_numel(OP, "lp", lp, (int64_t)(n)); ck_numel(OP, "total_norm", total_norm, (int64_t)(1)); const long rc = (long)ab_clip_adam((float*)p(param), (const float*)p(grad), (float*)p(m), (float*)p(v), (long)n, (const float*)p(total_norm), (float)max_norm, (float)lr, (float)beta1, (float)beta2, (float)eps, (int)step, (const float*)p(hyper), (void*)p(lp), cur_stream()); TORCH_CHECK(rc == 0, "ab_clip_adam failed with code ", rc, rc > 0 ? " (hipError)" : " (argument error)"); }
 static void w_clip_adam_x3(const c10::optional<at::Tensor>& param, const c10::optional<at::Tensor>& grad, const c10::optional<at::Tensor>& m, const c10::optional<at::Tensor>& v, int64_t n, const c10::optional<at::Tensor>& total_norm, double max_norm, double lr, double beta1, double beta2, double eps, int64_t step, const c10::optional<at::Tensor>& hyper, const c10::optional<at::Tensor>& lp_hi, const c10::optional<at::Tensor>& lp_lo) { static const char* const OP = "artiboost_hip::clip_adam_x3"; ck_dev(OP, "param", param, (int)at::kFloat, true); ck_dev(OP, "grad", grad, (int)at::kFloat, true); ck_dev(OP, "m", m, (int)at::kFloat, true); ck_dev(OP, "v", v, (int)at::kFloat, true); ck_dev(OP, "total_norm", total_norm, (int)at::kFloat, true); ck_dev(OP, "hyper", hyper, (int)at::kFloat, true); ck_dev(OP, "lp_hi", lp_hi, (int)-1, true); ck_dev(OP, "lp_lo", lp_lo, (int)-1, true); ck_dtype(OP, "lp_hi", lp_hi, at::kBFloat16); ck_dtype(OP, "lp_lo", lp_lo, at::kBFloat16); ck_numel(OP, "param", param, (int64_t)(n)); ck_numel(OP, "grad", grad, (int64_t)(n)); ck_numel(OP, "m", m, (int64_t)(n)); ck_numel(OP, "v", v, (int64_t)(n)); ck_numel(OP, "lp_hi", lp_hi, (int64_t)(n)); ck_numel(OP, "lp_lo", lp_lo, (int64_t)(n)); ck_numel(OP, "total_norm", total_norm, (int64_t)(1)); const long rc = (long)ab_clip_adam_x3((float*)p(param), (const float*)p(grad), (float*)p(m), (float*)p(v), (long)n, (const float*)p(total_norm), (float)max_norm, (float)lr, (float)beta1, (float)beta2, (float)eps, (int)step, (const float*)p(hyper), (void*)p(lp_hi), (void*)p(lp_lo), cur_stream()); TORCH_CHECK(rc == 0, "ab_clip_adam_x3 failed with code ", rc, rc > 0 ? " (hipError)" : " (argument error)"); }
+static int64_t w_grad_norm_parts(int64_t n) { return (int64_t)ab_grad_norm_parts((long)n); }
+static void w_grad_sqnorm(const c10::optional<at::Tensor>& grad, int64_t n, const c10::optional<at::Tensor>& part) { static const char* const OP = "artiboost_hip::grad_sqnorm"; ck_dev(OP, "grad", grad, (int)at::kFloat, true); ck_dev(OP, "part", part, (int)at::kFloat, true); ck_numel(OP, "grad", grad, (int64_t)(n)); ck_numel(OP, "part", part, (int64_t)(ab_grad_norm_parts(n))); const long rc = (long)ab_grad_sqnorm((const float*)p(grad), (long)n, (float*)p(part), cur_stream()); TORCH_CHECK(rc == 0, "ab_grad_sqnorm failed with code ", rc, rc > 0 ? " (hipError)" : " (argument error)"); }
+static void w_clip_adam_layouts(const c10::optional<at::Tensor>& param, const c10::optional<at::Tensor>& grad, const c10::optional<at::Tensor>& m, const c10::optional<at::Tensor>& v, int64_t n, const c10::optional<at::Tensor>& total_norm, double max_norm, double lr, double beta1, double beta2, double eps, int64_t step, const c10::optional<at::Tensor>& hyper, const c10::optional<at::Tensor>& lp_hi, const c10::optional<at::Tensor>& lp_lo, const c10::optional<at::Tensor>& tiles_dev, int64_t ntensors, int64_t total_tiles, const c10::optional<at::Tensor>& ranges_dev, int64_t nranges, const c10::optional<at::Tensor>& part, int64_t nparts) { static const char* const OP = "artiboost_hip::clip_adam_layouts"; ck_dev(OP, "param", param, (int)at::kFloat, true); ck_dev(OP, "grad", grad, (int)at::kFloat, true); ck_dev(OP, "m", m, (int)at::kFloat, true); ck_dev(OP, "v", v, (int)at::kFloat, true); ck_dev(OP, "total_norm", total_norm, (int)at::kFloat, true); ck_dev(OP, "hyper", hyper, (int)at::kFloat, true); ck_dev(OP, "lp_hi", lp_hi, (int)-1, true); ck_dev(OP, "lp_lo", lp_lo, (int)-1, true); ck_dev(OP, "tiles_dev", tiles_dev, (int)-1, true); ck_dev(OP, "ranges_dev", ranges_dev, (int)-1, true); ck_dev(OP, "part", part, (int)at::kFloat, true); ck_dtype(OP, "lp_hi", lp_hi, at::kBFloat16); ck_dtype(OP, "lp_lo", lp_lo, at::kBFloat16); ck_numel(OP, "param", param, (int64_t)(n)); ck_numel(OP, "grad", grad, (int64_t)(n)); ck_numel(OP, "m", m, (int64_t)(n)); ck_numel(OP, "v", v, (int64_t)(n)); ck_numel(OP, "lp_hi", lp_hi, (int64_t)(n)); ck_numel(OP, "lp_lo", lp_lo, (int64_t)(n)); ck_numel(OP, "total_norm", total_norm, (int64_t)(1)); ck_numel(OP, "part", part, (int64_t)(nparts)); ck_bytes(OP, "tiles_dev", tiles_dev, (int64_t)(ntensors*48)); ck_bytes(OP, "ranges_dev", ranges_dev, (int64_t)(nranges*16)); const long rc = (long)ab_clip_adam_layouts((float*)p(param), (const float*)p(grad), (float*)p(m), (float*)p(v), (long)n, (float*)p(total_norm), (float)max_norm, (float)lr, (float)beta1, (float)beta2, (float)eps, (int)step, (const float*)p(hyper), (void*)p(lp_hi), (void*)p(lp_lo), (const ab_adam_tile_desc*)p(tiles_dev), (int)ntensors, (long)total_tiles, (const ab_adam_range*)p(ranges_dev), (long)nranges, (const float*)p(part), (int)nparts, cur_stream()); TORCH_CHECK(rc == 0, "ab_clip_adam_layouts failed with code ", rc, rc > 0 ? " (hipError)" : " (argument error)"); }
 static void w_pose_assemble(const c10::optional<at::Tensor>& kp3d, const c10::optional<at::Tensor>& box6d, int64_t box_stride, const c10::optional<at::Tensor>& root_joint, const c10::optional<at::Tensor>& cam_intr, const c10::optional<at::Tensor>& corners_can, int64_t B, int64_t center_idx, double res_w, double res_h, const c10::optional<at::Tensor>& joints_abs, const c10::optional<at::Tensor>& corners_abs, const c10::optional<at::Tensor>& rotmat, const c10::optional<at::Tensor>& uvd2d, const c10::optional<at::Tensor>& joints_rel, const c10::optional<at::Tensor>& corners_rel, const c10::optional<at::Tensor>& boxroot) { static const char* const OP = "artiboost_hip::pose_assemble"; ck_dev(OP, "kp3d", kp3d, (int)at::kFloat, true); ck_dev(OP, "box6d", box6d, (int)at::kFloat, false); ck_dev(OP, "root_joint", root_joint, (int)at::kFloat, true); ck_dev(OP, "cam_intr", cam_intr, (int)at::kFloat, true); ck_dev(OP, "corners_can", corners_can, (int)at::kFloat, true); ck_dev(OP, "joints_abs", joints_abs, (int)at::kFloat, true); ck_dev(OP, "corners_abs", corners_abs, (int)at::kFloat, true); ck_dev(OP, "rotmat", rotmat, (int)at::kFloat, true); ck_dev(OP, "uvd2d", uvd2d, (int)at::kFloat, true); ck_dev(OP, "joints_rel", joints_rel, (int)at::kFloat, true); ck_dev(OP, "corners_rel", corners_rel, (int)at::kFloat, true); ck_dev(OP, "boxroot", boxroot, (int)at::kFloat, true); ck_numel(OP, "kp3d", kp3d, (int64_t)(B*22*3)); ck_numel(OP, "root_joint", root_joint, (int64_t)(B*3)); ck_numel(OP, "cam_intr", cam_intr, (int64_t)(B*9)); ck_numel(OP, "corners_can", corners_can, (int64_t)(B*24)); ck_numel(OP, "joints_abs", joints_abs, (int64_t)(B*63)); ck_numel(OP, "joints_rel", joints_rel, (int64_t)(B*63)); ck_numel(OP, "corners_abs", corners_abs, (int64_t)(B*24)); ck_numel(OP, "corners_rel", corners_rel, (int64_t)(B*24)); ck_numel(OP, "rotmat", rotmat, (int64_t)(B*9)); ck_numel(OP, "uvd2d", uvd2d, (int64_t)(B*90)); const long rc = (long)ab_pose_assemble((const float*)p(kp3d), (const float*)p(box6d), (int)box_stride, (const float*)p(root_joint), (const float*)p(cam_intr), (const float*)p(corners_can), (int)B, (int)center_idx, (float)res_w, (float)res_h, (float*)p(joints_abs), (float*)p(corners_abs), (float*)p(rotmat), (float*)p(uvd2d), (float*)p(joints_rel), (float*)p(corners_rel), (float*)p(boxroot), cur_stream()); TORCH_CHECK(rc == 0, "ab_pose_assemble failed with code ", rc, rc > 0 ? " (hipError)" : " (argument error)"); }
 static void w_pose_loss(const c10::optional<at::Tensor>& kp3d, const c10::optional<at::Tensor>& box6d, int64_t box_stride, const c10::optional<at::Tensor>& root_joint, const c10::optional<at::Tensor>& cam_intr, const c10::optional<at::Tensor>& corners_can, const c10::optional<at::Tensor>& joints_3d, const c10::optional<at::Tensor>& corners_3d, const c10::optional<at::Tensor>& joints_vis, const c10::optional<at::Tensor>& corners_vis, const c10::optional<at::Tensor>& hand_views, int64_t nvh, const c10::optional<at::Tensor>& j0, const c10::optional<at::Tensor>& j1, int64_t njp, const c10::optional<at::Tensor>& p0, const c10::optional<at::Tensor>& p1, int64_t npp, const c10::optional<at::Tensor>& scene_views, int64_t nvs, const c10::optional<at::Tensor>& s0, const c10::optional<at::Tensor>& s1, int64_t nsp, int64_t B, int64_t center_idx, double res_w, double res_h, const c10::optional<at::Tensor>& weights8_host, const c10::optional<at::Tensor>& joints_abs, const c10::optional<at::Tensor>& corners_abs, const c10::optional<at::Tensor>& rotmat, const c10::optional<at::Tensor>& uvd2d, const c10::optional<at::Tensor>& sample_part, const c10::optional<at::Tensor>& losses, const c10::optional<at::Tensor>& g_kp3d, const c10::optional<at::Tensor>& g_box6d) { static const char* const OP = "artiboost_hip::pose_loss"; ck_dev(OP, "kp3d", kp3d, (int)at::kFloat, true); ck_dev(OP, "box6d", box6d, (int)at::kFloat, false); ck_dev(OP, "root_joint", root_joint, (int)at::kFloat, true); ck_dev(OP, "cam_intr", cam_intr, (int)at::kFloat, true); ck_dev(OP, "corners_can", corners_can, (int)at::kFloat, true); ck_dev(OP, "joints_3d", joints_3d, (int)at::kFloat, true); ck_dev(OP, "corners_3d", corners_3d, (int)at::kFloat, true); ck_dev(OP, "joints_vis", joints_vis, (int)at::kFloat, true); ck_dev(OP, "corners_vis", corners_vis, (int)at::kFloat, true); ck_dev(OP, "hand_views", hand_views, (int)at::kFloat, true); ck_dev(OP, "j0", j0, (int)at::kLong, true); ck_dev(OP, "j1", j1, (int)at::kLong, true); ck_dev(OP, "p0", p0, (int)at::kLong, true); ck_dev(OP, "p1", p1, (int)at::kLong, true); ck_dev(OP, "scene_views", scene_views, (int)at::kFloat, true); ck_dev(OP, "s0", s0, (int)at::kLong, true); ck_dev(OP, "s1", s1, (int)at::kLong, true); ck_host(OP, "weights8_host", weights8_host); ck_dev(OP, "joints_abs", joints_abs, (int)at::kFloat, true); ck_dev(OP, "corners_abs", corners_abs, (int)at::kFloat, true); ck_dev(OP, "rotmat", rotmat, (int)at::kFloat, true); ck_dev(OP, "uvd2d", uvd2d, (int)at::kFloat, true); ck_dev(OP, "sample_part", sample_part, (int)at::kFloat, true); ck_dev(OP, "losses", losses, (int)at::kFloat, true); ck_dev(OP, "g_kp3d", g_kp3d, (int)at::kFloat, true); ck_dev(OP, "g_box6d", g_box6d, (int)at::kFloat, false); ck_numel(OP, "kp3d", kp3d, (int64_t)(B*22*3)); ck_numel(OP, "g_kp3d", g_kp3d, (int64_t)(B*22*3)); ck_numel(OP, "root_joint", root_joint, (int64_t)(B*3)); ck_numel(OP, "cam_intr", cam_intr, (int64_t)(B*9)); ck_numel(OP, "corners_can", corners_can, (int64_t)(B*24)); ck_numel(OP, "corners_3d", corners_3d, (int64_t)(B*24)); ck_numel(OP, "joints_3d", joints_3d, (int64_t)(B*63)); ck_numel(OP, "joints_vis", joints_vis, (int64_t)(B*21)); ck_numel(OP, "corners_vis", corners_vis, (int64_t)(B*8)); ck_numel(OP, "hand_views", hand_views, (int64_t)(nvh*3)); ck_numel(OP, "scene_views", scene_views, (int64_t)(nvs*3)); ck_numel(OP, "j0", j0, (int64_t)(njp)); ck_numel(OP, "j1", j1, (int64_t)(njp)); ck_numel(OP, "p0", p0, (int64_t)(npp)); ck_numel(OP, "p1", p1, (int64_t)(npp)); ck_numel(OP, "s0", s0, (int64_t)(nsp)); ck_numel(OP, "s1", s1, (int64_t)(nsp)); ck_numel(OP, "weights8_host", weights8_host, (int64_t)(8)); const long rc = (long)ab_pose_loss((const float*)p(kp3d), (const float*)p(box6d), (int)box_stride, (const float*)p(root_joint), (const float*)p(cam_intr), (const float*)p(corners_can), (const float*)p(joints_3d), (const float*)p(corners_3d), (const float*)p(joints_vis), (const float*)p(corners_vis), (const float*)p(hand_views), (int)nvh, (const int64_t*)p(j0), (const int64_t*)p(j1), (int)njp, (const int64_t*)p(p0), (const int64_t*)p(p1), (int)npp, (const float*)p(scene_views), (int)nvs, (const int64_t*)p(s0), (const int64_t*)p(s1), (int)nsp, (int)B, (int)center_idx, (float)res_w, (float)res_h, (const float*)p(weights8_host), (float*)p(joints_abs), (float*)p(corners_abs), (float*)p(rotmat), (float*)p(uvd2d), (float*)p(sample_part), (float*)p(losses), (float*)p(g_kp3d), (float*)p(g_box6d), cur_stream()); TORCH_CHECK(rc == 0, "ab_pose_loss failed with code ", rc, rc > 0 ? " (hipError)" : " (argument error)"); }
 static void w_pose_loss_sym(const c10::optional<at::Tensor>& kp3d, const c10::optional<at::Tensor>& box6d, int64_t box_stride, const c10::optional<at::Tensor>& root_joint, const c10::optional<at::Tensor>& cam_intr, const c10::optional<at::Tensor>& corners_can, const c10::optional<at::Tensor>& joints_3d, const c10::optional<at::Tensor>& corners_3d, const c10::optional<at::Tensor>& joints_vis, const c10::optional<at::Tensor>& corners_vis, const c10::optional<at::Tensor>& hand_views, int64_t nvh, const c10::optional<at::Tensor>& j0, const c10::optional<at::Tensor>& j1, int64_t njp, const c10::optional<at::Tensor>& p0, const c10::optional<at::Tensor>& p1, int64_t npp, const c10::optional<at::Tensor>& scene_views, int64_t nvs, const c10::optional<at::Tensor>& s0, const c10::optional<at::Tensor>& s1, int64_t nsp, int64_t B, int64_t center_idx, double res_w, double res_h, const c10::optional<at::Tensor>& weights8_host, const c10::optional<at::Tensor>& sym, const c10::optional<at::Tensor>& joints_abs, const c10::optional<at::Tensor>& corners_abs, const c10::optional<at::Tensor>& rotmat, const c10::optional<at::Tensor>& uvd2d, const c10::optional<at::Tensor>& sample_part, const c10::optional<at::Tensor>& losses, const c10::optional<at::Tensor>& g_kp3d, const c10::optional<at::Tensor>& g_box6d) { static const char* const OP = "artiboost_hip::pose_loss_sym"; ck_dev(OP, "kp3d", kp3d, (int)at::kFloat, true); ck_dev(OP, "box6d", box6d, (int)at::kFloat, false); ck_dev(OP, "root_joint", root_joint, (int)at::kFloat, true); ck_dev(OP, "cam_intr", cam_intr, (int)at::kFloat, true); ck_dev(OP, "corners_can", corners_can, (int)at::kFloat, true); ck_dev(OP, "joints_3d", joints_3d, (int)at::kFloat, true); ck_dev(OP, "corners_3d", corners_3d, (int)at::kFloat, true); ck_dev(OP, "joints_vis", joints_vis, (int)at::kFloat, true); ck_dev(OP, "corners_vis", corners_vis, (int)at::kFloat, true); ck_dev(OP, "hand_views", hand_views, (int)at::kFloat, true); ck_dev(OP, "j0", j0, (int)at::kLong, true); ck_dev(OP, "j1", j1, (int)at::kLong, true); ck_dev(OP, "p0", p0, (int)at::kLong, true); ck_dev(OP, "p1", p1, (int)at::kLong, true); ck_dev(OP, "scene_views", scene_views, (int)at::kFloat, true); ck_dev(OP, "s0", s0, (int)at::kLong, true); ck_dev(OP, "s1", s1, (int)at::kLong, true); ck_host(OP, "weights8_host", weights8_host); ck_contig(OP, "sym", sym); ck_dev(OP, "joints_abs", joints_abs, (int)at::kFloat, true); ck_dev(OP, "corners_abs", corners_abs, (int)at::kFloat, true); ck_dev(OP, "rotmat", rotmat, (int)at::kFloat, true); ck_dev(OP, "uvd2d", uvd2d, (int)at::kFloat, true); ck_dev(OP, "sample_part", sample_part, (int)at::kFloat, true); ck_dev(OP, "losses", losses, (int)at::kFloat, true); ck_dev(OP, "g_kp3d", g_kp3d, (int)at::kFloat, true); ck_dev(OP, "g_box6d", g_box6d, (int)at::kFloat, false); ck_numel(OP, "kp3d", kp3d, (int64_t)(B*22*3)); ck_numel(OP, "g_kp3d", g_kp3d, (int64_t)(B*22*3)); ck_numel(OP, "root_joint", root_joint, (int64_t)(B*3)); ck_numel(OP, "cam_intr", cam_intr, (int64_t)(B*9)); const long rc = (long)ab_pose_loss_sym((const float*)p(kp3d), (const float*)p(box6d), (int)box_stride, (const float*)p(root_joint), (const float*)p(cam_intr), (const float*)p(corners_can), (const float*)p(joints_3d), (const float*)p(corners_3d), (const float*)p(joints_vis), (const float*)p(corners_vis), (const float*)p(hand_views), (int)nvh, (const int64_t*)p(j0), (const int64_t*)p(j1), (int)njp, (const int64_t*)p(p0), (const int64_t*)p(p1), (int)npp, (const float*)p(scene_views), (int)nvs, (const int64_t*)p(s0), (const int64_t*)p(s1), (int)nsp, (int)B, (int)center_idx, (float)res_w, (float)res_h, (const float*)p(weights8_host), (const ab_symcorner*)p(sym), (float*)p(joints_abs), (float*)p(corners_abs), (float*)p(rotmat), (float*)p(uvd2d), (float*)p(sample_part), (float*)p(losses), (float*)p(g_kp3d), (float*)p(g_box6d), cur_stream()); TORCH_CHECK(rc == 0, "ab_pose_loss_sym failed with code ", rc, rc > 0 ? " (hipError)" : " (argument error)"); }
@@ -307,6 +310,9 @@
     m.def("scale_f32(Tensor(a!)? x, int n, float s) -> ()");
     m.def("clip_adam(Tensor(a!)? param, Tensor? grad, Tensor(b!)? m, Tensor(c!)? v, int n, Tensor? total_norm, float max_norm, float lr, float beta1, float beta2, float eps, int step, Tensor? hyper, Tensor(d!)? lp) -> ()");
     m.def("clip_adam_x3(Tensor(a!)? param, Tensor? grad, Tensor(b!)? m, Tensor(c!)? v, int n, Tensor? total_norm, float max_norm, float lr, float beta1, float beta2, float eps, int step, Tensor? hyper, Tensor(d!)? lp_hi, Tensor(e!)? lp_lo) -> ()");
+    m.def("grad_norm_parts(int n) -> int");
+    m.def("grad_sqnorm(Tensor? grad, int n, Tensor(a!)? part) -> ()");
+    m.def("clip_adam_layouts(Tensor(a!)? param, Tensor? grad, Tensor(b!)? m, Tensor(c!)? v, int n, Tensor(d!)? total_norm, float max_norm, float lr, float beta1, float beta2, float eps, int step, Tensor? hyper, Tensor(e!)? lp_hi, Tensor(f!)? lp_lo, Tensor? tiles_dev, int ntensors, int total_tiles, Tensor? ranges_dev, int nranges, Tensor? part, int nparts) -> ()");
     m.def("pose_assemble(Tensor? kp3d, Tensor? box6d, int box_stride, Tensor? root_joint, Tensor? cam_intr, Tensor? corners_can, int B, int center_idx, float res_w, float res_h, Tensor(a!)? joints_abs, Tensor(b!)? corners_abs, Tensor(c!)? rotmat, Tensor(d!)? uvd2d, Tensor(e!)? joints_rel, Tensor(f!)? corners_rel, Tensor(g!)? boxroot) -> ()");
     m.def("pose_loss(Tensor? kp3d, Tensor? box6d, int box_stride, Tensor? root_joint, Tensor? cam_intr, Tensor? corners_can, Tensor? joints_3d, Tensor? corners_3d, Tensor? joints_vis, Tensor? corners_vis, Tensor? hand_views, int nvh, Tensor? j0, Tensor? j1, int njp, Tensor? p0, Tensor? p1, int npp, Tensor? scene_views, int nvs, Tensor? s0, Tensor? s1, int nsp, int B, int center_idx, float res_w, float res_h, Tensor? weights8_host, Tensor(a!)? joints_abs, Tensor(b!)? corners_abs, Tensor(c!)? rotmat, Tensor(d!)? uvd2d, Tensor(e!)? sample_part, Tensor(f!)? losses, Tensor(g!)? g_kp3d, Tensor(h!)? g_box6d) -> ()");
     m.def("pose_loss_sym(Tensor? kp3d, Tensor? box6d, int box_stride, Tensor? root_joint, Tensor? cam_intr, Tensor? corners_can, Tensor? joints_3d, Tensor? corners_3d, Tensor? joints_vis, Tensor? corners_vis, Tensor? hand_views, int nvh, Tensor? j0, Tensor? j1, int njp, Tensor? p0, Tensor? p1, int npp, Tensor? scene_views, int nvs, Tensor? s0, Tensor? s1, int nsp, int B, int center_idx, float res_w, float res_h, Tensor? weights8_host, Tensor? sym, Tensor(a!)? joints_abs, Tensor(b!)? corners_abs, Tensor(c!)? rotmat, Tensor(d!)? uvd2d, Tensor(e!)? sample_part, Tensor(f!)? losses, Tensor(g!)? g_kp3d, Tensor(h!)? g_box6d) -> ()");
@@ -439,6 +445,9 @@
     m.impl("scale_f32", &w_scale_f32);
     m.impl("clip_adam", &w_clip_adam);
     m.impl("clip_adam_x3", &w_clip_adam_x3);
+    m.impl("grad_norm_parts", &w_grad_norm_parts);
+    m.impl("grad_sqnorm", &w_grad_sqnorm);
+    m.impl("clip_adam_layouts", &w_clip_adam_layouts);
     m.impl("pose_assemble", &w_pose_assemble);
     m.impl("pose_loss", &w_pose_loss);
     m.impl("pose_loss_sym", &w_pose_loss_sym);
diff --git a/artiboost_amd/hybridnet.py b/artiboost_amd/hybridnet.py
--- a/artiboost_amd/hybridnet.py
+++ b/artiboost_amd/hybridnet.py
@@ -297,6 +297,7 @@
         self.last = None
         self.eval_fold = True
         self._tr_plan = None
+        self._adam_plan = None
         self._eval_desc = None
         self._eval_bnp = None
         self._zparts = {}
@@ -313,7 +314,9 @@
                 names.append(name)
         return names
 
-    def refresh_after_update(self, lp_fresh=False):
+    def refresh_after_update(self, lp_fresh=False, tr_fresh=False):
+        if lp_fresh and tr_fresh and self._packed:
+            return
         self.pack_weights(skip_cast=lp_fresh)
 
     def pack_weights(self, skip_cast=False):
@@ -360,6 +363,8 @@
                 bpairs.append((p.view(name).reshape(O, 1, I), dst.view(I, 1, O)))
             self._box_pairs = bpairs
             self._box_plan = (K.transpose_plan(bpairs) or False) if bpairs else False
+            if self.x3 and self._tr_plan and (self._box_plan or not bpairs):
+                self._adam_plan = K.adam_layout_plan(p.flat, [(pairs, K.ADAM_KIND_X3, self._tr_lo_off), (bpairs, K.ADAM_KIND_F32, 0)])
         if self._box_plan:
             K.transpose_oki_batch(self._box_plan)
         else:
diff --git a/artiboost_amd/kernels.py b/artiboost_amd/kernels.py
--- a/artiboost_amd/kernels.py
+++ b/artiboost_amd/kernels.py
@@ -374,6 +374,78 @@
     L.check(L.lib().ab_transpose_oki_batch_x3(L.ptr(dev), L.i(n), L.l(tiles), L.l(lo_offset_elems), L.stream()), "ab_transpose_oki_batch_x3")
 
 
+ADAM_TILE_DESC = [("dst", "<u8"), ("flat_off", "<i8"), ("lo_off", "<i8"), ("O", "<i4"), ("K", "<i4"), ("I", "<i4"), ("tile_begin", "<i4"),
+                  ("kind", "<i4"), ("reserved", "<i4")]
+ADAM_RANGE = [("begin", "<i8"), ("end", "<i8")]
+ADAM_KIND_X3, ADAM_KIND_F32 = 0, 1
+ADAM_RANGE_CHUNK = 4096
+
+
+def adam_layout_tables(entries, total, chunk=ADAM_RANGE_CHUNK):
+    import numpy as np
+    if total % 4 or chunk % 4 or chunk < 4:
+        return None
+    tiles = np.zeros(len(entries), dtype=np.dtype(ADAM_TILE_DESC))
+    nt = 0
+    for n, (off, O, Kk, I, dst, kind, lo_off) in enumerate(entries):
+        if I % 4 or O % 8 or off % 4 or off < 0 or min(O, Kk, I) < 1 or kind not in (ADAM_KIND_X3, ADAM_KIND_F32):
+            return None
+        if dst % 16 or (kind == ADAM_KIND_X3 and (lo_off <= 0 or lo_off % 8)):
+            return None
+        tiles[n] = (dst, off, lo_off if kind == ADAM_KIND_X3 else 0, O, Kk, I, nt, kind, 0)
+        nt += ((O + 63) // 64) * Kk * ((I + 63) // 64)
+    spans = sorted((int(off), int(off) + O * Kk * I) for off, O, Kk, I, _, _, _ in entries)
+    gaps, at = [], 0
+    for b, e in spans:
+        if b < at or e > total:
+            return None
+        if b > at:
+            gaps.append((at, b))
+        at = e
+    if at < total:
+        gaps.append((at, total))
+    pieces = [(b, min(b + chunk, e)) for g0, e in gaps for b in range(g0, e, chunk)]
+    ranges = np.zeros(len(pieces), dtype=np.dtype(ADAM_RANGE))
+    for n, pc in enumerate(pieces):
+        ranges[n] = pc
+    if nt + len(pieces) > 0x7fffffff:
+        return None
+    return tiles, ranges, nt
+
+
+def adam_layout_plan(flat, groups):
+    entries = []
+    for pairs, kind, lo_off in groups:
+        want = torch.bfloat16 if kind == ADAM_KIND_X3 else torch.float32
+        for src, dst in pairs:
+            O, Kk, I = src.shape
+            rel = src.data_ptr() - flat.data_ptr()
+            if not src.is_contiguous() or not dst.is_contiguous() or dst.dtype != want or src.dtype != torch.float32 or rel % 4:
+                return None
+            entries.append((rel // 4, O, Kk, I, dst.data_ptr(), kind, lo_off))
+    tabs = adam_layout_tables(entries, flat.numel())
+    if tabs is None:
+        return None
+    tiles, ranges, nt = tabs
+    import numpy as np
+    up = lambda a: torch.from_numpy(a.view(np.uint8).reshape(-1).copy()).to(flat.device) if len(a) else None
+    return dict(tiles=up(tiles), ntensors=len(tiles), total_tiles=nt, ranges=up(ranges), nranges=len(ranges), flat_ptr=flat.data_ptr(),
+                n=flat.numel())
+
+
+def grad_sqnorm(grad, part):
+    L.check(L.lib().ab_grad_sqnorm(L.ptr(grad), L.l(grad.numel()), L.ptr(part), L.stream()), "ab_grad_sqnorm")
+    return int(L.lib().ab_grad_norm_parts(L.l(grad.numel())))
+
+
+def clip_adam_layouts(plan, p, g, m, v, total_norm, max_norm, lr, b1, b2, eps, step, hyper, lp_planes, part, nparts):
+    assert plan["flat_ptr"] == p.data_ptr() and plan["n"] == p.numel()
+    L.check(L.lib().ab_clip_adam_layouts(L.ptr(p), L.ptr(g), L.ptr(m), L.ptr(v), L.l(p.numel()), L.ptr(total_norm), L.f(max_norm), L.f(lr),
+                                         L.f(b1), L.f(b2), L.f(eps), L.i(step), L.ptr(hyper), L.ptr(lp_planes[0]), L.ptr(lp_planes[1]),
+                                         L.ptr(plan["tiles"]), L.i(plan["ntensors"]), L.l(plan["total_tiles"]), L.ptr(plan["ranges"]),
+                                         L.l(plan["nranges"]), L.ptr(part), L.i(nparts), L.stream()), "ab_clip_adam_layouts")
+
+
 def image_pad_nhwc4(img_nchw_f32, dtype):
     N, C, H, W = img_nchw_f32.shape
     assert C == 3
diff --git a/artiboost_amd/optim.py b/artiboost_amd/optim.py
--- a/artiboost_amd/optim.py
+++ b/artiboost_amd/optim.py
@@ -1,6 +1,7 @@
 import torch
 
 from . import _lib as L
+from . import kernels as K
 
 
 class FusedClipAdam(torch.optim.Optimizer):
@@ -17,6 +18,7 @@
         self._hyper_host = None
         self.graph_steps = 0
         self._eager_hyper = None
+        self.separate_layouts = False
 
     HYPER_SLOTS = 32
 
@@ -57,10 +59,13 @@
         for st in self.state.values():
             self.graph_steps = max(self.graph_steps, int(st.get("step", 0)))
 
-    def grad_norm(self, grad):
+    def _norm_buffers(self, grad):
         if self._part is None:
             self._part = torch.empty(1024, dtype=torch.float32, device=grad.device)
             self.total_norm = torch.empty(1, dtype=torch.float32, device=grad.device)
+
+    def grad_norm(self, grad):
+        self._norm_buffers(grad)
         L.check(L.lib().ab_grad_norm(L.ptr(grad), L.l(grad.numel()), L.ptr(self._part), L.ptr(self.total_norm),
                                      L.stream()), "ab_grad_norm")
         return self.total_norm
@@ -78,9 +83,19 @@
                     st["exp_avg_sq"] = torch.zeros_like(p)
                 st["step"] += 1
                 g = p.grad
-                tn = self.grad_norm(g) if self.max_norm else None
                 lp = lp_planes = None
                 net = self.model.net if (self.model is not None and p is self.model.flat_param) else None
+                plan = getattr(net, "_adam_plan", None) if (net is not None and getattr(net, "x3", False) and net._packed) else None
+                if self.separate_layouts or (plan is not None and (plan["flat_ptr"] != p.data_ptr() or plan["n"] != p.numel())):
+                    plan = None
+                nparts = 0
+                if plan is not None:
+                    self._norm_buffers(g)
+                    tn = self.total_norm
+                    if self.max_norm:
+                        nparts = K.grad_sqnorm(g, self._part)
+                else:
+                    tn = self.grad_norm(g) if self.max_norm else None
                 if net is not None and getattr(net, "x3", False):
                     if net.lp is None or tuple(net.lp.shape) != (2, p.numel()):
                         net.lp = torch.empty((2, p.numel()), dtype=torch.bfloat16, device=p.device)
@@ -96,7 +111,10 @@
                         self._eager_hyper = torch.zeros(3, dtype=torch.float32, device=p.device)
                     hyper = self._eager_hyper
                     hyper.copy_(torch.tensor([group["lr"], 1.0 - b1 ** st["step"], (1.0 - b2 ** st["step"]) ** 0.5], dtype=torch.float32))
-                if lp_planes is not None:
+                if plan is not None:
+                    K.clip_adam_layouts(plan, p, g, st["exp_avg"], st["exp_avg_sq"], tn, self.max_norm or 0.0, group["lr"], b1, b2,
+                                        group["eps"], st["step"], hyper, lp_planes, self._part, nparts)
+                elif lp_planes is not None:
                     L.check(L.lib().ab_clip_adam_x3(L.ptr(p), L.ptr(g), L.ptr(st["exp_avg"]), L.ptr(st["exp_avg_sq"]),
                                                     L.l(p.numel()), L.ptr(tn), L.f(self.max_norm or 0.0), L.f(group["lr"]),
                                                     L.f(b1), L.f(b2), L.f(group["eps"]), L.i(st["step"]), L.ptr(hyper),
@@ -107,5 +125,5 @@
                                                  L.f(b1), L.f(b2), L.f(group["eps"]), L.i(st["step"]), L.ptr(hyper),
                                                  L.ptr(lp), L.stream()), "ab_clip_adam")
                 if net is not None:
-                    net.refresh_after_update(lp_fresh=lp is not None or lp_planes is not None)
+                    net.refresh_after_update(lp_fresh=lp is not None or lp_planes is not None, tr_fresh=plan is not None)
         return None
diff --git a/include/artiboost_hip.h b/include/artiboost_hip.h
--- a/include/artiboost_hip.h
+++ b/include/artiboost_hip.h
@@ -204,6 +204,24 @@
 int ab_clip_adam_x3(float* param, const float* grad, float* m, float* v, long n, const float* total_norm,
                     float max_norm, float lr, float beta1, float beta2, float eps, int step,
                     const float* hyper, void* lp_hi, void* lp_lo, void* stream);
+typedef struct ab_adam_tile_desc {
+    void* dst;
+    int64_t flat_off;
+    int64_t lo_off;
+    int32_t O, K, I;
+    int32_t tile_begin;
+    int32_t kind;
+    int32_t reserved;
+} ab_adam_tile_desc;
+typedef struct ab_adam_range {
+    int64_t begin, end;
+} ab_adam_range;
+int ab_grad_norm_parts(long n);
+int ab_grad_sqnorm(const float* grad, long n, float* part, void* stream);
+int ab_clip_adam_layouts(float* param, const float* grad, float* m, float* v, long n, float* total_norm, float max_norm, float lr,
+                         float beta1, float beta2, float eps, int step, const float* hyper, void* lp_hi, void* lp_lo,
+                         const ab_adam_tile_desc* tiles_dev, int ntensors, long total_tiles, const ab_adam_range* ranges_dev,
+                         long nranges, const float* part, int nparts, void* stream);
 
 int ab_pose_assemble(const float* kp3d, const float* box6d, int box_stride, const float* root_joint, const float* cam_intr,
                      const float* corners_can, int B, int center_idx, float res_w, float res_h, float* joints_abs,
```

Measured after the change: 7422 samples/s (median of 4 runs). Within noise of the previous version (+0.1%).
